# facebookresearch/PoseDiffusion

Measured on AMD Instinct MI355X. Metric: sequences/sec (20-frame, GGS on), higher is better.
Workload: dtype f32 (GGS, attention, LayerNorm, DDPM update, every accumulation); the encoder GEMMs multiply fp16 hi + lo operand pairs (22 bits, static power-of-two scales) with fp32 accumulation -- `exact_mode` is the same pipe with them on the exact-fp32 matrix instruction

## Files before the change

include/pd_engine.h:

```cpp
#ifndef PD_ENGINE_H
#define PD_ENGINE_H

#include <stdint.h>

#ifdef __cplusplus
extern "C" {
#endif

#define PD_OK 0
#define PD_ERR_INVALID_ARG (-1)
#define PD_ERR_UNSUPPORTED (-2)
#define PD_ERR_HIP (-3)
#define PD_ERR_STATE (-4)

#define PD_MAX_LAYERS 16
#define PD_POSE_DIM 9

typedef struct pd_engine pd_engine;

typedef struct pd_layer_weights {
    const float *norm1_w, *norm1_b;
    const float *in_proj_w, *in_proj_b;
    const float *out_proj_w, *out_proj_b;
    const float *norm2_w, *norm2_b;
    const float *linear1_w, *linear1_b;
    const float *linear2_w, *linear2_b;
} pd_layer_weights;

typedef struct pd_weights {
    int32_t d_model;
    int32_t nhead;
    int32_t dim_ff;
    int32_t num_layers;
    int32_t z_dim;
    int32_t n_harmonic;
    int32_t t_emb_dim;
    int32_t mlp_hidden;
    int32_t timesteps;
    int32_t reserved;
    const float *time_w0, *time_b0;
    const float *time_w2, *time_b2;
    const float *first_w, *first_b;
    pd_layer_weights layers[PD_MAX_LAYERS];
    const float *last0_w, *last0_b;
    const float *last_ln_w, *last_ln_b;
    const float *last3_w, *last3_b;
    const float *sqrt_recip_alphas_cumprod;
    const float *sqrt_recipm1_alphas_cumprod;
    const float *posterior_mean_coef1;
    const float *posterior_mean_coef2;
    const float *posterior_log_variance_clipped;
} pd_weights;

#define PD_WEIGHTS_PRED_X0 1
#define PD_WEIGHTS_POST_NORM 2
#define PD_WEIGHTS_NO_PIVOT 4
#define PD_WEIGHTS_GENERIC 8

typedef struct pd_ggs_cfg {
    float alpha;
    float learning_rate;
    int32_t iter_num;
    float sampson_max;
    int32_t min_matches;
    float momentum;
    int32_t wgs_per_seq;
    int32_t reserved;
} pd_ggs_cfg;
#define PD_GGS_CFG_FORCE_ONE_HOP 1
#define PD_GGS_CFG_NO_LDS_STAGING 2
#define PD_GGS_CFG_WAVES8 4
#define PD_GGS_CFG_LANE_ITEMS 8
#define PD_GGS_CFG_NO_LANE_ITEMS 16
#define PD_GGS_CFG_XCHG_SPREAD 32
#define PD_GGS_CFG_LONG_FRAMES 64


int pd_engine_create(const pd_weights *w, int max_B, int max_N, pd_engine **out);
void pd_engine_destroy(pd_engine *eng);
const char *pd_last_error(void);
const char *pd_version(void);


int pd_denoise_step(pd_engine *eng, const float *x, const float *z, int t, int B, int N,
                    float *eps_out, void *stream);

int pd_p_mean(pd_engine *eng, const float *x, const float *z, int t, int B, int N,
              float *mean_out, float *x0_out, void *stream);

int pd_p_finish(pd_engine *eng, const float *mean, const float *noise, int t, int B, int N,
                float *x_out, void *stream);


int pd_engine_set_q_tables(pd_engine *eng, const float *sqrt_alphas_cumprod, const float *sqrt_one_minus_alphas_cumprod);

int pd_denoise_step_t(pd_engine *eng, const float *x, const float *z, const int64_t *t_seq, int B, int N, float *out, void *stream);

int pd_p_losses(pd_engine *eng, const float *x_start, const float *z, const int64_t *t_seq, const float *noise, int B, int N,
                int loss_type, float *loss_out, float *x0_pred_out, float *xt_out, float *model_out, void *stream);

int pd_engine_set_frame_counts(pd_engine *eng, int B, const int32_t *n_frames, void *stream);


int pd_ggs_set_matches(pd_engine *eng, int seq, const double *kp1, const double *kp2,
                       const int64_t *i12, int64_t M, int n_frames, int height, int width);

#define PD_MATCH_HINT_ONE_ORDER (1 << 30)
typedef struct pd_match_hints {
    int32_t max_pairs;
    int32_t max_matches_per_pair;
} pd_match_hints;
int pd_ggs_set_matches_csr_async(pd_engine *eng, int seq_first, int n_seqs, const int64_t *seq_offsets, const double *kp1,
                                 const double *kp2, const int64_t *i12, int n_frames, int height, int width,
                                 const pd_match_hints *hints, void *stream);


int pd_ggs_guide(pd_engine *eng, float *model_mean, int B, int N, int t, const pd_ggs_cfg *cfg,
                 float *stats_out, void *stream);

int pd_ggs_stage_iters(const pd_ggs_cfg *cfg, int *iters_out5);

int pd_ggs_optimize(pd_engine *eng, float *model_mean, int B, int N, int update_R, int update_T,
                    int update_FL, const pd_ggs_cfg *cfg, float *stats_out, float *trace_out,
                    void *stream);

int pd_ggs_loss_grad(pd_engine *eng, const float *x, int B, int N, int update_R, int update_T,
                     int update_FL, const pd_ggs_cfg *cfg, float *loss_out, float *grad_out,
                     void *stream);


#define PD_OPT_DENOISER_SPLIT 2
#define PD_OPT_DENOISER_FUSED_ATTN 5
#define PD_OPT_DENOISER_LONG_ATTN 6
#define PD_OPT_GGS_MAX_FRAMES 7
#define PD_OPT_GGS_LONG_PAIR_ITEMS 8
int pd_engine_set_option(pd_engine *eng, int option, int value);
#define PD_OPT_WEIGHTS_NON_FINITE 4
int pd_engine_get_option(pd_engine *eng, int option, int *value_out);

int pd_sample(pd_engine *eng, const float *z, const float *noise, int B, int N, int cond_start_step,
              const pd_ggs_cfg *ggs, float *pose_out, float *process_out, float *stats_out,
              int use_graph, void *stream);

#define PD_PHASE_ALL 0
#define PD_PHASE_UNGUIDED 1
#define PD_PHASE_GUIDED 2
int pd_sample_phase(pd_engine *eng, const float *z, const float *noise, int B, int N, int cond_start_step,
                    const pd_ggs_cfg *ggs, int phase, float *pose_out, float *process_out, float *stats_out,
                    int use_graph, void *stream);

int pd_pose_to_camera(pd_engine *eng, const float *enc, int n_cameras, float *R_out, float *T_out,
                      float *focal_out, void *stream);
int pd_pose_to_camera_ex(pd_engine *eng, const float *enc, int n_cameras, float *R_out, float *T_out,
                         float *focal_out, float log_focal_length_bias, float min_focal_length, float max_focal_length,
                         void *stream);

int pd_camera_to_pose(const float *R, const float *T, const float *focal, int n, float log_focal_length_bias,
                      float min_focal_length, float max_focal_length, float *enc_out, void *stream);


int pd_time_embedding(const float *w0, const float *b0, const float *w2, const float *b2, const float *timesteps, int n,
                      float *out, void *stream);

int pd_pose_embedding(const float *x, long long rows, int dim, float *out, void *stream);


int pd_metrics_rel_pose_errors(const float *R_pred, const float *T_pred, const float *R_gt, const float *T_gt, int B, int N,
                               float *rel_r_deg, float *rel_t_deg, void *stream);

int pd_metrics_summary(const float *rel_r_deg, const float *rel_t_deg, int n, int max_threshold, float *out7, void *stream);

int pd_metrics_are(const float *R_a, const float *R_b, int n, float *err_deg, void *stream);

int pd_align_cameras(const float *R_src, const float *T_src, const float *R_tgt, const float *T_tgt, int n, int estimate_scale,
                     float eps, float *R_out, float *T_out, float *s_R_T_out, void *stream);


int pd_preprocess_image(const unsigned char *rgb_hwc, int height, int width, int image_size, float *out_chw, void *stream);


typedef struct pd_vit_layer_weights {
    const float *norm1_w, *norm1_b, *qkv_w, *qkv_b, *proj_w, *proj_b, *norm2_w, *norm2_b, *fc1_w, *fc1_b, *fc2_w, *fc2_b;
} pd_vit_layer_weights;
typedef struct pd_vit_weights {
    int32_t dim, depth, num_heads, mlp_hidden, patch_size, pos_grid, reserved0, reserved1;
    const float *patch_w, *patch_b, *cls_token, *pos_embed, *norm_w, *norm_b;
    pd_vit_layer_weights layers[16];
} pd_vit_weights;
typedef struct pd_vit pd_vit;
int pd_vit_create(const pd_vit_weights *w, pd_vit **out);
void pd_vit_destroy(pd_vit *v);
#define PD_VIT_OPT_EXACT_FP32 1
int pd_vit_set_option(pd_vit *v, int option, int value);

int pd_vit_forward_scale(pd_vit *v, const float *images, int n_img, int H, int W, double scale_factor, const float *pos_scaled,
                         float weight, int accumulate, float *z_out, void *stream);


int pd_ggs_launch_stamps(pd_engine *eng, long long *dst, int n, int *clock_khz_out, void *stream);

int pd_time_kernel(pd_engine *eng, int what, int B, int N, const pd_ggs_cfg *cfg, int reps,
                   float *ms_out, void *stream);

int pd_check_async_error(pd_engine *eng);

int pd_debug_ggs_prof(pd_engine *eng, int enable, long long *out6);
int pd_debug_ggs_plan(pd_engine *eng, int B, int N, const pd_ggs_cfg *cfg, int *out8);
int pd_debug_lane_tables(pd_engine *eng, int seq, int *out, int n_out);
int pd_debug_mfma_f16_subnormal(float *out4_host, void *stream);
int pd_debug_vit_tokens(pd_vit *v, float *dst, long long n_floats, void *stream);

#ifdef __cplusplus
}
#endif
#endif
```

posediffusion_amd/_lib.py:

```python
from __future__ import annotations

import ctypes as C
import os
import subprocess

_HERE = os.path.dirname(os.path.abspath(__file__))
LIB_PATH = os.environ.get("PD_ENGINE_LIB") or os.path.join(_HERE, "lib", "libpd_engine.so")
CSRC_DIR = os.path.join(_HERE, "csrc")
HEADER_PATH = os.path.normpath(os.path.join(_HERE, "..", "include", "pd_engine.h"))

PD_MAX_LAYERS = 16

c_float_p = C.POINTER(C.c_float)


class pd_layer_weights(C.Structure):
    _fields_ = [(n, C.c_void_p) for n in (
        "norm1_w", "norm1_b", "in_proj_w", "in_proj_b", "out_proj_w", "out_proj_b",
        "norm2_w", "norm2_b", "linear1_w", "linear1_b", "linear2_w", "linear2_b")]


class pd_weights(C.Structure):
    _fields_ = (
        [(n, C.c_int32) for n in ("d_model", "nhead", "dim_ff", "num_layers", "z_dim", "n_harmonic",
                                  "t_emb_dim", "mlp_hidden", "timesteps", "reserved")]
        + [(n, C.c_void_p) for n in ("time_w0", "time_b0", "time_w2", "time_b2", "first_w", "first_b")]
        + [("layers", pd_layer_weights * PD_MAX_LAYERS)]
        + [(n, C.c_void_p) for n in ("last0_w", "last0_b", "last_ln_w", "last_ln_b", "last3_w", "last3_b",
                                     "sqrt_recip_alphas_cumprod", "sqrt_recipm1_alphas_cumprod",
                                     "posterior_mean_coef1", "posterior_mean_coef2",
                                     "posterior_log_variance_clipped")]
    )


class pd_layer_grads(C.Structure):
    _fields_ = list(pd_layer_weights._fields_)


class pd_weight_grads(C.Structure):
    _fields_ = (
        [(n, C.c_void_p) for n in ("time_w0", "time_b0", "time_w2", "time_b2", "first_w", "first_b")]
        + [("layers", pd_layer_grads * PD_MAX_LAYERS)]
        + [(n, C.c_void_p) for n in ("last0_w", "last0_b", "last_ln_w", "last_ln_b", "last3_w", "last3_b")]
    )


class pd_vit_layer_weights(C.Structure):
    _fields_ = [(n, C.c_void_p) for n in ("norm1_w", "norm1_b", "qkv_w", "qkv_b", "proj_w", "proj_b", "norm2_w", "norm2_b",
                                          "fc1_w", "fc1_b", "fc2_w", "fc2_b")]


class pd_vit_weights(C.Structure):
    _fields_ = ([(n, C.c_int32) for n in ("dim", "depth", "num_heads", "mlp_hidden", "patch_size", "pos_grid", "reserved0", "reserved1")]
                + [(n, C.c_void_p) for n in ("patch_w", "patch_b", "cls_token", "pos_embed", "norm_w", "norm_b")]
                + [("layers", pd_vit_layer_weights * 16)])


class pd_vit_layer_grads(C.Structure):
    _fields_ = list(pd_vit_layer_weights._fields_)


class pd_vit_weight_grads(C.Structure):
    _fields_ = ([(n, C.c_void_p) for n in ("patch_w", "patch_b", "cls_token", "pos_embed", "norm_w", "norm_b")]
                + [("layers", pd_vit_layer_grads * 16)])


PD_VIT_TRAIN_MAX_TOKENS, PD_VIT_TRAIN_MAX_SCALES = 256, 8

PD_GGS_CFG_FORCE_ONE_HOP = 1
PD_GGS_CFG_NO_LDS_STAGING = 2
PD_GGS_CFG_WAVES8 = 4
PD_WEIGHTS_PRED_X0 = 1
PD_WEIGHTS_POST_NORM = 2
PD_WEIGHTS_NO_PIVOT = 4
PD_WEIGHTS_GENERIC = 8
PD_GGS_CFG_LANE_ITEMS = 8
PD_GGS_CFG_NO_LANE_ITEMS = 16
PD_GGS_CFG_XCHG_SPREAD = 32
PD_GGS_CFG_LONG_FRAMES = 64
PD_OPT_DENOISER_SPLIT = 2
PD_OPT_WEIGHTS_NON_FINITE = 4
PD_OPT_DENOISER_FUSED_ATTN = 5
PD_OPT_DENOISER_LONG_ATTN = 6
PD_OPT_GGS_MAX_FRAMES = 7
PD_OPT_GGS_LONG_PAIR_ITEMS = 8
PD_DROP_ATTN, PD_DROP_RESID1, PD_DROP_FF, PD_DROP_RESID2, PD_DROP_ALL = 1, 2, 4, 8, 15
PD_TR_OPT_MAX_FRAMES, PD_TR_OPT_LONG_ATTN = 1, 2
PD_MATCH_HINT_ONE_ORDER = 1 << 30


class pd_ggs_cfg(C.Structure):
    _fields_ = [("alpha", C.c_float), ("learning_rate", C.c_float), ("iter_num", C.c_int32),
                ("sampson_max", C.c_float), ("min_matches", C.c_int32), ("momentum", C.c_float),
                ("wgs_per_seq", C.c_int32), ("reserved", C.c_int32)]


class pd_match_hints(C.Structure):
    _fields_ = [("max_pairs", C.c_int32), ("max_matches_per_pair", C.c_int32)]


_vp, _i, _i64 = C.c_void_p, C.c_int, C.c_int64
SIGNATURES = {
    "pd_engine_create": (_i, [C.POINTER(pd_weights), _i, _i, C.POINTER(_vp)]),
    "pd_engine_destroy": (None, [_vp]),
    "pd_last_error": (C.c_char_p, []),
    "pd_version": (C.c_char_p, []),
    "pd_denoise_step": (_i, [_vp, _vp, _vp, _i, _i, _i, _vp, _vp]),
    "pd_engine_set_q_tables": (_i, [_vp, _vp, _vp]),
    "pd_engine_set_frame_counts": (_i, [_vp, _i, C.POINTER(C.c_int32), _vp]),
    "pd_denoise_step_t": (_i, [_vp, _vp, _vp, _vp, _i, _i, _vp, _vp]),
    "pd_p_losses": (_i, [_vp, _vp, _vp, _vp, _vp, _i, _i, _i, _vp, _vp, _vp, _vp, _vp]),
    "pd_camera_to_pose": (_i, [_vp, _vp, _vp, _i, C.c_float, C.c_float, C.c_float, _vp, _vp]),
    "pd_p_mean": (_i, [_vp, _vp, _vp, _i, _i, _i, _vp, _vp, _vp]),
    "pd_p_finish": (_i, [_vp, _vp, _vp, _i, _i, _i, _vp, _vp]),
    "pd_ggs_set_matches": (_i, [_vp, _i, _vp, _vp, _vp, _i64, _i, _i, _i]),
    "pd_ggs_set_matches_csr_async": (_i, [_vp, _i, _i, C.POINTER(_i64), _vp, _vp, _vp, _i, _i, _i, C.POINTER(pd_match_hints), _vp]),
    "pd_ggs_guide": (_i, [_vp, _vp, _i, _i, _i, C.POINTER(pd_ggs_cfg), _vp, _vp]),
    "pd_ggs_optimize": (_i, [_vp, _vp, _i, _i, _i, _i, _i, C.POINTER(pd_ggs_cfg), _vp, _vp, _vp]),
    "pd_ggs_loss_grad": (_i, [_vp, _vp, _i, _i, _i, _i, _i, C.POINTER(pd_ggs_cfg), _vp, _vp, _vp]),
    "pd_engine_set_option": (_i, [_vp, _i, _i]),
    "pd_engine_get_option": (_i, [_vp, _i, C.POINTER(_i)]),
    "pd_time_embedding": (_i, [_vp, _vp, _vp, _vp, _vp, _i, _vp, _vp]),
    "pd_pose_embedding": (_i, [_vp, C.c_longlong, _i, _vp, _vp]),
    "pd_metrics_rel_pose_errors": (_i, [_vp, _vp, _vp, _vp, _i, _i, _vp, _vp, _vp]),
    "pd_metrics_summary": (_i, [_vp, _vp, _i, _i, _vp, _vp]),
    "pd_metrics_are": (_i, [_vp, _vp, _i, _vp, _vp]),
    "pd_vit_create": (_i, [C.POINTER(pd_vit_weights), C.POINTER(_vp)]),
    "pd_vit_destroy": (None, [_vp]),
    "pd_vit_set_option": (_i, [_vp, _i, _i]),
    "pd_vit_forward_scale": (_i, [_vp, _vp, _i, _i, _i, C.c_double, _vp, C.c_float, _i, _vp, _vp]),
    "pd_preprocess_image": (_i, [_vp, _i, _i, _i, _vp, _vp]),
    "pd_align_cameras": (_i, [_vp, _vp, _vp, _vp, _i, _i, C.c_float, _vp, _vp, _vp, _vp]),
    "pd_sample": (_i, [_vp, _vp, _vp, _i, _i, _i, C.POINTER(pd_ggs_cfg), _vp, _vp, _vp, _i, _vp]),
    "pd_sample_phase": (_i, [_vp, _vp, _vp, _i, _i, _i, C.POINTER(pd_ggs_cfg), _i, _vp, _vp, _vp, _i, _vp]),
    "pd_pose_to_camera": (_i, [_vp, _vp, _i, _vp, _vp, _vp, _vp]),
    "pd_debug_lane_tables": (_i, [_vp, _i, C.POINTER(C.c_int), _i]),
    "pd_ggs_launch_stamps": (_i, [_vp, _vp, _i, C.POINTER(C.c_int), _vp]),
    "pd_ggs_stage_iters": (_i, [C.POINTER(pd_ggs_cfg), C.POINTER(C.c_int)]),
    "pd_pose_to_camera_ex": (_i, [_vp, _vp, _i, _vp, _vp, _vp, C.c_float, C.c_float, C.c_float, _vp]),
    "pd_time_kernel": (_i, [_vp, _i, _i, _i, C.POINTER(pd_ggs_cfg), _i, C.POINTER(C.c_float), _vp]),
    "pd_check_async_error": (_i, [_vp]),
    "pd_debug_ggs_prof": (_i, [_vp, _i, C.POINTER(C.c_longlong)]),
    "pd_debug_ggs_plan": (_i, [_vp, _i, _i, C.POINTER(pd_ggs_cfg), C.POINTER(C.c_int)]),
    "pd_debug_mfma_f16_subnormal": (_i, [C.POINTER(C.c_float), _vp]),
    "pd_debug_vit_tokens": (_i, [_vp, _vp, C.c_longlong, _vp]),
}
EXT_SIGNATURES = {
    "pd_ggs_set_matches_csr_async_nf": (_i, [_vp, _i, _i, C.POINTER(_i64), _vp, _vp, _vp, C.POINTER(_i), _i, _i, C.POINTER(pd_match_hints), _vp]),
}
TRAIN_SIGNATURES = {
    "pd_trainer_create": (_i, [C.POINTER(pd_weights), _vp, _vp, _i, _i, C.POINTER(_vp)]),
    "pd_trainer_destroy": (None, [_vp]),
    "pd_trainer_set_option": (_i, [_vp, _i, _i]),
    "pd_trainer_get_option": (_i, [_vp, _i, C.POINTER(_i)]),
    "pd_train_forward": (_i, [_vp, C.POINTER(pd_weights), _vp, _vp, _vp, _vp, _i, _i, _i, _vp, _vp, _vp, _vp, _vp]),
    "pd_train_forward_dropout": (_i, [_vp, C.POINTER(pd_weights), _vp, _vp, _vp, _vp, _i, _i, _i, C.c_float, C.c_uint, C.c_uint64, C.c_uint32,
                                      _vp, _vp, _vp, _vp, _vp]),
    "pd_train_backward": (_i, [_vp, C.POINTER(pd_weights), _vp, C.POINTER(pd_weight_grads), _vp, _vp]),
    "pd_train_debug_relu": (_i, [_vp, _i, _vp, C.c_longlong, _vp]),
    "pd_trainer_check_async": (_i, [_vp]),
}
VIT_TRAIN_SIGNATURES = {
    "pd_vit_trainer_create": (_i, [C.POINTER(pd_vit_weights), _i, _i, _i, C.POINTER(_vp)]),
    "pd_vit_trainer_destroy": (None, [_vp]),
    "pd_vit_train_forward": (_i, [_vp, C.POINTER(pd_vit_weights), _vp, _i, _i, _i, C.POINTER(C.c_double), _i, C.POINTER(_vp), _vp, _vp]),
    "pd_vit_train_backward": (_i, [_vp, C.POINTER(pd_vit_weights), _vp, C.POINTER(pd_vit_weight_grads), _vp]),
}

_lib = None


def build(verbose: bool = False) -> str:
    cmd = ["make", "-C", CSRC_DIR, "-j4"]
    res = subprocess.run(cmd, stdout=subprocess.PIPE, stderr=subprocess.STDOUT, text=True)
    if verbose or res.returncode != 0:
        print(res.stdout)
    if res.returncode != 0 or not os.path.isfile(LIB_PATH):
        raise RuntimeError("building libpd_engine.so failed:\n" + res.stdout[-4000:])
    return LIB_PATH


def load():
    global _lib
    if _lib is not None:
        return _lib
    if not os.path.isfile(LIB_PATH):
        raise RuntimeError(
            f"posediffusion_amd: HIP engine library not found at {LIB_PATH}. Build it with "
            "`python -c 'import __graft_entry__ as g; g.build()'` (or `make -C posediffusion_amd/csrc`). "
            "There is no CPU fallback.")
    import torch
    lib = C.CDLL(LIB_PATH, mode=C.RTLD_GLOBAL)
    for name, (res, args) in {**SIGNATURES, **EXT_SIGNATURES, **TRAIN_SIGNATURES, **VIT_TRAIN_SIGNATURES}.items():
        if os.environ.get("PD_ENGINE_LIB") and not hasattr(lib, name):
            continue
        fn = getattr(lib, name)
        fn.restype = res
        fn.argtypes = args
    _lib = lib
    return lib


def last_error() -> str:
    return (load().pd_last_error() or b"").decode("utf-8", "replace")


def check(rc: int, what: str = "pd_engine"):
    if rc != 0:
        raise RuntimeError(f"{what} failed (code {rc}): {last_error()}")
```

posediffusion_amd/csrc/pd_denoiser.hip:

```cpp
#include "pd_denoiser_dev.h"
#include "pd_gemm_stream.h"
#include "pd_gemm_split.h"
#include "pd_qkv_attn.h"
#include "pd_gemm_small.h"
#include "pd_attn.h"
#include "pd_attn_long.h"
#include "pd_denoiser_kernels.h"
#include "pd_denoiser_plan.h"

#include <algorithm>
#include <math.h>
#include <stdlib.h>
#include <string.h>

int pd_time_table(const pd_weights *w, float *table) {
    if (!w->time_w0 || !w->time_b0 || !w->time_w2 || !w->time_b2) {
        pd_set_error("pd_engine_create: a weight pointer is NULL");
        return PD_ERR_INVALID_ARG;
    }
    hipLaunchKernelGGL(pd_time_table_kernel, dim3(w->timesteps), dim3(128), 0, 0, w->time_w0, w->time_b0, w->time_w2, w->time_b2, table);
    PD_HIP_CHECK(hipGetLastError());
    return PD_OK;
}

// ... 128 lines not shown

bool pd_denoiser_has_streamed_path(const pd_engine *eng) { return eng->den && eng->den->hn; }
bool pd_denoiser_weights_non_finite(const pd_engine *eng) { return eng->den && eng->den->non_finite; }

int pd_denoiser_build_split(pd_engine *eng, int mode) {
    if (eng->gden) {
        pd_set_error("split-precision denoiser: this engine runs the shape-generic denoiser path (a non-default configuration or "
                     "PD_WEIGHTS_GENERIC), which has only the exact-fp32 kernels: PD_OPT_DENOISER_SPLIT stays 0");
        return PD_ERR_UNSUPPORTED;
    }
    PdDenoiserDev *d = eng->den;
    if (!d->hn) {
        pd_set_error("split-precision denoiser: the engine was created for fewer than %d token rows (max_B x max_N); the mode "
                     "applies to the streamed large-batch path only", PD_STREAM_MIN_ROWS);
        return PD_ERR_UNSUPPORTED;
    }
    const bool f16 = mode == 2;
    bool &ready = f16 ? d->split_h_ready : d->split_ready;
    if (ready) return PD_OK;
    PdPlaneExps e[PD_MAX_LAYERS] = {};
    for (int l = 0; f16 && l < d->num_layers; ++l) {
        PdLayerDev &L = d->layers[l];
        bool finite = true;
        PD_TRY(pd_plane_exponents(L.qkv_wf, L.qkv_b, L.out_wf, L.ff1_wf, L.ff1_b, L.ff2_wf, DM, DFF, &e[l], &finite));
        if (!finite) {
            d->non_finite = true;
            pd_set_error("denoiser: encoder layer %d holds non-finite weights or biases: no static operand bound exists, the fp16-plane "
                         "mode (PD_OPT_DENOISER_SPLIT = 2) is not available for these weights", l);
            return PD_ERR_INVALID_ARG;
        }
    }
    const int e_ln = 9;
    for (int l = 0; l < d->num_layers; ++l) {
        PdLayerDev &L = d->layers[l];
        PD_TRY(d->mem.planes(f16 ? &L.qkv_wh : &L.qkv_ws, L.qkv_wf, 3 * DM, DM, nullptr, f16, e[l].qkv));
        PD_TRY(d->mem.planes(f16 ? &L.out_wh : &L.out_ws, L.out_wf, DM, DM, nullptr, f16, e[l].out));
        PD_TRY(d->mem.planes(f16 ? &L.ff1_wh : &L.ff1_ws, L.ff1_wf, DFF, DM, nullptr, f16, e[l].ff1));
        PD_TRY(d->mem.planes(f16 ? &L.ff2_wh : &L.ff2_ws, L.ff2_wf, DM, DFF, nullptr, f16, e[l].ff2));
        if (!f16) continue;
        L.qkv_cs = ldexpf(1.0f, -(e_ln + e[l].qkv));
        L.out_cs = ldexpf(1.0f, -(e[l].ctx + e[l].out));
        L.ff1_cs = ldexpf(1.0f, -(e_ln + e[l].ff1));
        L.ff2_cs = ldexpf(1.0f, -(e[l].hid + e[l].ff2));
        L.ctx_scale = ldexpf(1.0f, e[l].ctx);
        L.ff_scale = ldexpf(1.0f, e[l].hid);
    }
    PD_HIP_CHECK(hipDeviceSynchronize());
    ready = true;
    return PD_OK;
}

void pd_denoiser_destroy(pd_engine *eng) {
    pd_denoiser_generic_destroy(eng);
    delete eng->den;
    eng->den = nullptr;
}

int pd_denoiser_prepare(pd_engine *eng, const float *z, int B, int N, hipStream_t s) {
    PdDenoiserDev *d = eng->den;
    if (eng->gden) d = nullptr;
    if (!z || B <= 0 || N <= 0 || B > eng->max_B || N > eng->max_N) {
        pd_set_error("denoiser: invalid arguments (B=%d N=%d; max_B=%d max_N=%d)", B, N, eng->max_B, eng->max_N);
        return PD_ERR_INVALID_ARG;
    }
    if (!d) return PD_OK;
    const int M = B * N;
    if (M >= PD_STREAM_MIN_ROWS && d->hn) pd_gemm_dma<0>(z, ZD, d->first_zf, ZD, d->first_b, d->zproj, M, DM, s);
    PD_HIP_CHECK(hipGetLastError());
    return PD_OK;
}

static void den_first_small(const pd_engine *eng, const PdDenoiserDev *d, GemmArgs &g, const float *x, const float *z, int t, int N, int MT, hipStream_t s) {
    g.bias = d->first_b; g.C = d->h; g.Nout = DM;
    g.x = x; g.z = z; g.temb = d->t_table + (size_t)t * 128; g.n_frames = N;
    launch_gemm<KFIRST_PAD, 2, 0>(g, d->first_wp, MT, eng->gemm_wide_min_tiles, s);
}
static void den_first_streamed(const PdDenoiserDev *d, const float *x, int t, int N, int M, hipStream_t s) {
    hipLaunchKernelGGL(pd_embed_rows_kernel, dim3((M + 3) / 4), dim3(256), 0, s, x, N, M, d->emb);
    pd_gemm_dma<4>(d->emb, KFIRST_D, d->first_df, KFIRST_D, d->ttab + (size_t)t * DM, d->h, M, DM, s, nullptr, d->zproj);
}

static void den_first_small_t(const pd_engine *eng, const PdDenoiserDev *d, GemmArgs &g, const float *x, const float *z, const int *t_row, int N, int MT,
                              hipStream_t s) {
    g.bias = d->first_b; g.C = d->h; g.Nout = DM;
    g.x = x; g.z = z; g.temb = d->t_table; g.t_row = t_row; g.n_frames = N;
    launch_gemm<KFIRST_PAD, 3, 0>(g, d->first_wp, MT, eng->gemm_wide_min_tiles, s);
}
static void den_first_streamed_t(const PdDenoiserDev *d, const float *x, const int *t_row, int N, int M, hipStream_t s) {
    hipLaunchKernelGGL(pd_embed_rows_kernel, dim3((M + 3) / 4), dim3(256), 0, s, x, N, M, d->emb);
    pd_den_first_gemm_t(d, t_row, M, s);
}

template <int SPLIT_OUT>
static void den_attn_long(const PdDenoiserDev *d, int B, int N, float out_scale, const int *nf, hipStream_t s) {
    static_assert(PD_MAX_DENOISER_FRAMES == PD_ATTN_LONG_TILE * PD_ATTN_LONG_MAX_TILES, "a lane holds one score per 64-key tile");
    hipLaunchKernelGGL(pd_attn_long_kernel<SPLIT_OUT>, dim3(B * NH, (N + PD_ATTN_LONG_ROWS - 1) / PD_ATTN_LONG_ROWS), dim3(256), pd_attn_long_lds(N, DH), s,
                       d->qkv, d->ctx, N, out_scale, nf);
}

static void den_layer_small(const pd_engine *eng, const PdDenoiserDev *d, const PdLayerDev &L, GemmArgs &g, bool long_attn, const int *nf, int B, int N, int MT,
                            hipStream_t s) {
    g.A = d->h; g.bias = L.qkv_b; g.C = d->qkv; g.Nout = 3 * DM;
    launch_gemm<DM, 1, 0>(g, L.qkv_wp, MT, eng->gemm_wide_min_tiles, s);
    if (long_attn) {
        den_attn_long<0>(d, B, N, 1.0f, nf, s);
    } else {
#ifdef PD_DEN_STAMPS
        hipLaunchKernelGGL(pd_attn_kernel<false>, dim3(B * NH, (N + 3) / 4), dim3(256), attn_lds(N), s, d->qkv, d->ctx, N, next_stamp_slot());
#else
        hipLaunchKernelGGL(pd_attn_kernel<false>, dim3(B * NH, (N + 3) / 4), dim3(256), attn_lds(N), s, d->qkv, d->ctx, N);
#endif
    }
    g.A = d->ctx; g.bias = L.out_b; g.C = d->h; g.Nout = DM;
    launch_gemm<DM, 0, 2>(g, L.out_wp, MT, eng->gemm_wide_min_tiles, s);
    g.A = d->h; g.bias = L.ff1_b; g.C = d->ff; g.Nout = DFF;
    launch_gemm<DM, 1, 1>(g, L.ff1_wp, MT, eng->gemm_wide_min_tiles, s);
    g.A = d->ff; g.bias = L.ff2_b; g.C = d->h; g.Nout = DM;
    launch_gemm<DFF, 0, 2>(g, L.ff2_wp, MT, eng->gemm_wide_min_tiles, s);
}
static void den_layer_streamed(const PdDenoiserDev *d, const PdLayerDev &L, bool long_attn, const int *nf, int B, int N, int M, hipStream_t s) {
    float2 *stats = (float2 *)d->hn;
    hipLaunchKernelGGL(pd_ln_stats_kernel<DM>, dim3((M + 3) / 4), dim3(256), 0, s, d->h, stats, M, 1e-5f);
    pd_gemm_dma<0, true>(d->h, DM, L.qkv_wf, DM, L.qkv_b, d->qkv, M, 3 * DM, s, stats);
    if (long_attn) den_attn_long<0>(d, B, N, 1.0f, nf, s);
    else hipLaunchKernelGGL(pd_attn_seq_kernel<0>, dim3(B * NH), dim3(256), attn_seq_lds(N), s, d->qkv, d->ctx, N, 1.0f);
    pd_gemm_dma<2>(d->ctx, DM, L.out_wf, DM, L.out_b, d->h, M, DM, s);
    hipLaunchKernelGGL(pd_ln_stats_kernel<DM>, dim3((M + 3) / 4), dim3(256), 0, s, d->h, stats, M, 1e-5f);
    pd_gemm_dma<1, true>(d->h, DM, L.ff1_wf, DM, L.ff1_b, d->ff, M, DFF, s, stats);
    pd_gemm_dma<2>(d->ff, DFF, L.ff2_wf, DFF, L.ff2_b, d->h, M, DM, s);
}
static void den_layer_bf16(const PdDenoiserDev *d, const PdLayerDev &L, bool long_attn, const int *nf, int B, int N, int M, hipStream_t s) {
    hipLaunchKernelGGL((pd_ln_rows_kernel<DM, 1>), dim3((M + 3) / 4), dim3(256), 0, s, d->h, d->hn, M, 1e-5f, 1.0f);
    pd_gemm_split<0, 1, 2>((const unsigned *)d->hn, DM, L.qkv_ws, DM, L.qkv_b, d->qkv, M, 3 * DM, s);
    if (long_attn) den_attn_long<1>(d, B, N, 1.0f, nf, s);
    else hipLaunchKernelGGL(pd_attn_seq_kernel<1>, dim3(B * NH), dim3(256), attn_seq_lds(N), s, d->qkv, d->ctx, N, 1.0f);
    pd_gemm_split<2, 1, 1>((const unsigned *)d->ctx, DM, L.out_ws, DM, L.out_b, d->h, M, DM, s);
    hipLaunchKernelGGL((pd_ln_rows_kernel<DM, 1>), dim3((M + 3) / 4), dim3(256), 0, s, d->h, d->hn, M, 1e-5f, 1.0f);
    pd_gemm_split<4, 1, 2>((const unsigned *)d->hn, DM, L.ff1_ws, DM, L.ff1_b, d->ff, M, DFF, s);
    pd_gemm_split<2, 1, 1>((const unsigned *)d->ff, DFF, L.ff2_ws, DFF, L.ff2_b, d->h, M, DM, s);
}
template <int EPI>
static void den_gemm_f16(int rt, const float *A, int K, const unsigned *W, const float *bias, float *C, int M, int Nout, hipStream_t s, float c_scale,
                         float out_scale = 1.0f) {
    const unsigned *Aw = (const unsigned *)A;
    if constexpr (PD_STRIP_RT1 != 0 && (EPI == 2 || (EPI == 4 && PD_STRIP_RT1 == 2)))
        if (rt == 1) return pd_gemm_strip<EPI, 1, true, 1, PD_STRIP_K64>(Aw, K, W, K, bias, C, M, Nout, s, c_scale, out_scale);
    if constexpr (EPI != 0)
        if (rt == 3) return pd_gemm_strip<EPI, 3, true, 1, PD_STRIP_K64>(Aw, K, W, K, bias, C, M, Nout, s, c_scale, out_scale);
    if (rt == 2) return pd_gemm_strip<EPI, 2, true, 1, PD_STRIP_K64>(Aw, K, W, K, bias, C, M, Nout, s, c_scale, out_scale);
    pd_gemm_split<EPI, 1, EPI == 2 ? 1 : 2, true>(Aw, K, W, K, bias, C, M, Nout, s, c_scale, out_scale);
}
static void den_layer_f16(const PdDenoiserDev *d, const PdLayerDev &L, const PdDenStepPlan &p, const int *nf, int B, int N, hipStream_t s) {
    const int M = p.M;
    hipLaunchKernelGGL((pd_ln_rows_kernel<DM, 2>), dim3((M + 3) / 4), dim3(256), 0, s, d->h, d->hn, M, 1e-5f, 512.0f);
    if (p.fused_attn) {
        pd_qkv_attn((const unsigned *)d->hn, L.qkv_wh, L.qkv_b, (unsigned *)d->ctx, B, N, L.qkv_cs, L.ctx_scale, s);
    } else {
        den_gemm_f16<0>(p.strip & 1 ? 2 : 0, d->hn, DM, L.qkv_wh, L.qkv_b, d->qkv, M, 3 * DM, s, L.qkv_cs);
        if (p.long_attn) den_attn_long<2>(d, B, N, L.ctx_scale, nf, s);
        else if (p.attn_mma) hipLaunchKernelGGL(pd_attn_mma_kernel<2>, dim3(B * NH), dim3(256), attn_mma_lds(N), s, d->qkv, d->ctx, N, L.ctx_scale);
        else hipLaunchKernelGGL(pd_attn_seq_kernel<2>, dim3(B * NH), dim3(256), attn_seq_lds(N), s, d->qkv, d->ctx, N, L.ctx_scale);
    }
    den_gemm_f16<2>(p.strip & 2 ? p.rt_res : 0, d->ctx, DM, L.out_wh, L.out_b, d->h, M, DM, s, L.out_cs);
    hipLaunchKernelGGL((pd_ln_rows_kernel<DM, 2>), dim3((M + 3) / 4), dim3(256), 0, s, d->h, d->hn, M, 1e-5f, 512.0f);
    den_gemm_f16<4>(p.strip & 4 ? p.rt_ff1 : 0, d->hn, DM, L.ff1_wh, L.ff1_b, d->ff, M, DFF, s, L.ff1_cs, L.ff_scale);
    den_gemm_f16<2>(p.strip & 8 ? p.rt_res : 0, d->ff, DFF, L.ff2_wh, L.ff2_b, d->h, M, DM, s, L.ff2_cs);
}
static void den_tail(const pd_engine *eng, const PdDenoiserDev *d, const float *x, int t, int M, float *eps_out, float *mean_out, float *x0_out,
                     const float *noise, float *x_next_out, bool stamped, const int *nf, int N, hipStream_t s) {
    HeadArgs ha;
    memset(&ha, 0, sizeof(ha));
    ha.hid = d->hid; ha.lnw = d->last_ln_w; ha.lnb = d->last_ln_b;
    ha.w3 = d->last3_w; ha.b3 = d->last3_b; ha.x = x; ha.noise = noise;
    ha.eps_out = eps_out; ha.mean_out = mean_out; ha.x0_out = x0_out; ha.xnext_out = x_next_out;
    ha.c_recip = eng->c_recip[t]; ha.c_recipm1 = eng->c_recipm1[t]; ha.coef1 = eng->coef1[t]; ha.coef2 = eng->coef2[t];
    ha.sigma = expf(0.5f * eng->logvar[t]);
    ha.M = M;
    ha.pred_x0 = eng->pred_x0;
    ha.nf = nf; ha.n_frames = N;
#ifdef PD_DEN_STAMPS
    ha.stamps = stamped ? next_stamp_slot() : nullptr;
#endif
    hipLaunchKernelGGL(pd_tail_kernel, dim3((M + 3) / 4), dim3(256), 0, s, ha);
}

static void den_tail_t(const pd_engine *eng, const PdDenoiserDev *d, const float *x, int M, const PdTSeq &ts, float *eps_out, float *x0_out, hipStream_t s) {
    HeadArgsT a;
    memset(&a, 0, sizeof(a));
    a.h.hid = d->hid; a.h.lnw = d->last_ln_w; a.h.lnb = d->last_ln_b;
    a.h.w3 = d->last3_w; a.h.b3 = d->last3_b; a.h.x = x;
    a.h.eps_out = eps_out; a.h.x0_out = x0_out;
    a.h.M = M;
    a.h.pred_x0 = eng->pred_x0;
    a.t_row = ts.t_row; a.c_recip = eng->d_c_recip; a.c_recipm1 = eng->d_c_recipm1;
    a.target = ts.target; a.loss_out = ts.loss_out; a.loss_type = ts.loss_type;
    hipLaunchKernelGGL(pd_tail_t_kernel, dim3((M + 3) / 4), dim3(256), 0, s, a);
}

int pd_denoiser_t_rows(pd_engine *eng, const int64_t *t_seq, int B, int N, hipStream_t s) {
    const int M = B * N;
    hipLaunchKernelGGL(pd_t_rows_kernel, dim3((M + 255) / 256), dim3(256), 0, s, t_seq, M, N, eng->timesteps, eng->d_t_row, eng->d_err);
    PD_HIP_CHECK(hipGetLastError());
    return PD_OK;
}
int pd_denoiser_q_sample(pd_engine *eng, const float *x_start, const float *noise, const int64_t *t_seq, int B, int N, float *xt, hipStream_t s) {
    const int M = B * N;
    hipLaunchKernelGGL(pd_q_sample_kernel, dim3((M * 9 + 255) / 256), dim3(256), 0, s, x_start, noise, t_seq, eng->d_q_a, eng->d_q_b, M, N, eng->timesteps,
                       xt, eng->d_t_row, eng->d_err);
    PD_HIP_CHECK(hipGetLastError());
    return PD_OK;
}

int pd_denoiser_launch(pd_engine *eng, const float *x, const float *z, int t, int B, int N, float *eps_out,
                       float *mean_out, float *x0_out, const float *noise, float *x_next_out, hipStream_t s, bool z_prepared, const PdTSeq *ts) {
    if (eng->gden) return pd_denoiser_generic_launch(eng, x, z, t, B, N, eps_out, mean_out, x0_out, noise, x_next_out, s, ts);
    PdDenoiserDev *d = eng->den;
    if (!x || !z || B <= 0 || N <= 0 || B > eng->max_B || N > eng->max_N || N > PD_MAX_DENOISER_FRAMES || t < 0 || t >= d->timesteps) {
        pd_set_error("denoiser: invalid arguments (B=%d N=%d t=%d; max_B=%d max_N=%d, N <= %d, 0 <= t < %d)", B, N, t,
                     eng->max_B, eng->max_N, PD_MAX_DENOISER_FRAMES, d->timesteps);
        return PD_ERR_INVALID_ARG;
    }
    const int *nf = nullptr;
    if (!ts) PD_TRY(pd_frame_counts(eng, B, N, "denoiser", &nf));
    if (!z_prepared) {
        int rc = pd_denoiser_prepare(eng, z, B, N, s);
        if (rc) return rc;
    }
    static const int knob_strip = pd_dev_knob("PD_DEN_STRIP", 15), knob_attn_mma = pd_dev_knob("PD_DEN_ATTN_MMA", 1);
    const PdDenStepPlan p = pd_den_step_plan(B, N, eng->den_split, eng->den_fused_attn, eng->num_cus, d->hn != nullptr, d->split_ready,
                                             d->split_h_ready, knob_strip, knob_attn_mma, eng->den_long_attn, nf != nullptr);
    const bool small = p.path == PD_DEN_SMALL;
    const int M = p.M;
    GemmArgs g;
    memset(&g, 0, sizeof(g));
    g.M = M;
    if (small && ts) den_first_small_t(eng, d, g, x, z, ts->t_row, N, p.MT, s);
    else if (small) den_first_small(eng, d, g, x, z, t, N, p.MT, s);
    else if (ts) den_first_streamed_t(d, x, ts->t_row, N, M, s);
    else den_first_streamed(d, x, t, N, M, s);
    for (int l = 0; l < d->num_layers; ++l) {
        const PdLayerDev &L = d->layers[l];
        switch (p.path) {
        case PD_DEN_SMALL: den_layer_small(eng, d, L, g, p.long_attn, nf, B, N, p.MT, s); break;
        case PD_DEN_STREAMED: den_layer_streamed(d, L, p.long_attn, nf, B, N, M, s); break;
        case PD_DEN_BF16_PLANES: den_layer_bf16(d, L, p.long_attn, nf, B, N, M, s); break;
        case PD_DEN_F16_PLANES: den_layer_f16(d, L, p, nf, B, N, s); break;
        }
    }
    if (small) {
        g.A = d->h; g.bias = d->last0_b; g.C = d->hid; g.Nout = HID;
        launch_gemm<DM, 0, 0>(g, d->last0_wp, p.MT, eng->gemm_wide_min_tiles, s);
    } else {
        pd_gemm_dma<0>(d->h, DM, d->last0_wf, DM, d->last0_b, d->hid, M, HID, s);
    }
    if (ts) den_tail_t(eng, d, x, M, *ts, eps_out, x0_out, s);
    else den_tail(eng, d, x, t, M, eps_out, mean_out, x0_out, noise, x_next_out, small, nf, N, s);
    PD_HIP_CHECK(hipGetLastError());
    return PD_OK;
}


extern "C" int pd_time_embedding(const float *w0, const float *b0, const float *w2, const float *b2, const float *timesteps, int n,
                                 float *out, void *stream) {
    if (n == 0) return PD_OK;
    if (!w0 || !b0 || !w2 || !b2 || !timesteps || !out || n < 0) {
        pd_set_error("pd_time_embedding: invalid arguments (n=%d)", n);
        return PD_ERR_INVALID_ARG;
    }
    hipLaunchKernelGGL(pd_time_embed_kernel, dim3(n), dim3(128), 0, (hipStream_t)stream, timesteps, w0, b0, w2, b2, out);
    PD_HIP_CHECK(hipGetLastError());
    return PD_OK;
}
extern "C" int pd_pose_embedding(const float *x, long long rows, int dim, float *out, void *stream) {
    if (rows == 0 && dim >= 1) return PD_OK;
    if (!x || !out || rows < 0 || dim < 1 || dim > 4096) {
        pd_set_error("pd_pose_embedding: invalid arguments (rows=%lld dim=%d)", rows, dim);
        return PD_ERR_INVALID_ARG;
    }
    const long long total = rows * 21 * dim;
    const int blocks = (int)((total + 255) / 256 < 65536 ? (total + 255) / 256 : 65536);
    hipLaunchKernelGGL(pd_harmonic_rows_kernel, dim3(blocks), dim3(256), 0, (hipStream_t)stream, x, rows, dim, out);
    PD_HIP_CHECK(hipGetLastError());
    return PD_OK;
}

static int mfma_f16_subnormal(bool shape16, const char *who, float *out4_host, void *stream) {
    if (!out4_host) return PD_ERR_INVALID_ARG;
    float *d = nullptr;
    PD_HIP_CHECK(hipMalloc((void **)&d, 8 * sizeof(float)));
    hipStream_t s = (hipStream_t)stream;
    if (shape16) hipLaunchKernelGGL(pd_mfma16_f16_subnormal_kernel, dim3(1), dim3(64), 0, s, d);
    else hipLaunchKernelGGL(pd_mfma_f16_subnormal_kernel, dim3(1), dim3(64), 0, s, d);
    float h[8];
    hipError_t e = hipMemcpyAsync(h, d, sizeof(h), hipMemcpyDeviceToHost, s);
    if (e == hipSuccess) e = hipStreamSynchronize(s);
    (void)hipFree(d);
    if (e != hipSuccess) {
        pd_set_error("%s: %s", who, hipGetErrorString(e));
        return PD_ERR_HIP;
    }
    for (int i = 0; i < 4; ++i) out4_host[i] = h[i];
    if (h[4] == 0.0f) out4_host[0] = -1.0f;
    return PD_OK;
}
extern "C" int pd_debug_mfma_f16_subnormal(float *out4_host, void *stream) {
    return mfma_f16_subnormal(out4_host && out4_host[0] == 32.0f, "pd_debug_mfma_f16_subnormal", out4_host, stream);
}
```

posediffusion_amd/csrc/pd_denoiser_plan.h:

```cpp
#pragma once
#include "pd_qkv_attn.h"

#ifndef PD_STRIP_RT3
#define PD_STRIP_RT3 1
#endif
#ifndef PD_STRIP_RT1
#define PD_STRIP_RT1 0
#endif
#ifndef PD_STRIP_RT3_FF1
#define PD_STRIP_RT3_FF1 0
#endif
#ifndef PD_STRIP_K64
#define PD_STRIP_K64 true
#endif

enum PdDenPath {
    PD_DEN_SMALL,
    PD_DEN_STREAMED,
    PD_DEN_BF16_PLANES,
    PD_DEN_F16_PLANES
};

struct PdDenStepPlan {
    PdDenPath path;
    int M, MT;
    bool long_attn;
    bool fused_attn;
    bool attn_mma;
    int rt_res, rt_ff1;
    int strip;
};

static inline PdDenStepPlan pd_den_step_plan(int B, int N, int split, int fused_attn, int num_cus, bool has_streamed, bool split_ready,
                                             bool split_h_ready, int knob_strip, int knob_attn_mma, int long_attn = 0, bool ragged = false) {
    PdDenStepPlan p = {};
    p.M = B * N;
    p.MT = (p.M + 31) / 32;
    p.long_attn = N > 64 || long_attn != 0 || ragged;
    if (p.M < PD_STREAM_MIN_ROWS || !has_streamed) p.path = PD_DEN_SMALL;
    else if (split == 2 && split_h_ready) p.path = PD_DEN_F16_PLANES;
    else if (split == 1 && split_ready) p.path = PD_DEN_BF16_PLANES;
    else p.path = PD_DEN_STREAMED;
    if (p.path != PD_DEN_F16_PLANES) return p;
    const int cus = num_cus > 0 ? num_cus : 256;
    const int qa_wgs = pd_qkv_attn_wgs(B, N);
    const bool qa_fills = 4 * qa_wgs >= 3 * ((qa_wgs + cus - 1) / cus) * cus;
    p.fused_attn = qa_wgs > 0 && !p.long_attn && (fused_attn == 1 ? qa_fills : fused_attn == 2);
    p.attn_mma = N <= 32 && knob_attn_mma && !p.long_attn;
    const bool rt3 = PD_STRIP_RT3 && (((p.M + 63) / 64) * (DM / 128)) > cus && (((p.M + 95) / 96) * (DM / 128)) <= cus;
    p.rt_res = !rt3 ? 2 : PD_STRIP_RT1 ? 1 : 3;
    p.rt_ff1 = !rt3 ? 2 : PD_STRIP_RT1 == 2 ? 1 : PD_STRIP_RT3_FF1 ? 3 : 2;
    p.strip = knob_strip;
    return p;
}
```

posediffusion_amd/csrc/pd_engine.hip:

```cpp
#include "pd_internal.h"

#include <algorithm>

#include <math.h>
#include <stdarg.h>
#include <string.h>

static thread_local char g_err[1024] = "";

void pd_set_error(const char *fmt, ...) {
    va_list ap;
    va_start(ap, fmt);
    vsnprintf(g_err, sizeof(g_err), fmt, ap);
    va_end(ap);
}

extern "C" const char *pd_last_error(void) { return g_err; }
extern "C" const char *pd_version(void) { return "pd_engine 0.1 gfx950"; }

__global__ void pd_finish_kernel(const float *__restrict__ mean, const float *__restrict__ noise, float sigma, int n,
                                 float *__restrict__ out, const int *__restrict__ nf, int n_frames) {
    const int i = blockIdx.x * blockDim.x + threadIdx.x;
    if (i >= n) return;
    if (nf) {
// ... 436 lines not shown
    return pd_pose_to_camera_ex(eng, enc, n_cameras, R_out, T_out, focal_out, 1.8f, 0.1f, 20.0f, stream);
}

int pd_ggs_frames_unsupported(const pd_engine *eng, int N, const char *who) {
    if (!eng || N <= eng->ggs_max_frames || N > eng->max_N) return PD_OK;
    pd_set_error("%s: geometry-guided sampling (GGS) is limited to %d frames (N=%d); the denoiser and unguided sampling take up to %d "
                 "frames: sample without GGS", who, eng->ggs_max_frames, N, PD_MAX_DENOISER_FRAMES);
    return PD_ERR_UNSUPPORTED;
}
static void guide_stages(const pd_ggs_cfg *cfg, PdGgsStage *st) {
    const int it = cfg->iter_num;
    st[0] = {1, 1, 1, 2 * it};
    st[1] = {0, 0, 1, it};
    st[2] = {1, 0, 0, it};
    st[3] = {0, 1, 0, it};
    st[4] = {1, 1, 1, 2 * it};
}

extern "C" int pd_ggs_stage_iters(const pd_ggs_cfg *cfg, int *iters_out5) {
    if (!cfg || !iters_out5 || cfg->iter_num < 0) {
        pd_set_error("pd_ggs_stage_iters: invalid arguments");
        return PD_ERR_INVALID_ARG;
    }
    PdGgsStage st[PD_GGS_MAX_STAGES];
    guide_stages(cfg, st);
    for (int i = 0; i < 5; ++i) iters_out5[i] = st[i].iters;
    return PD_OK;
}

static int check_cfg(const pd_ggs_cfg *cfg, const char *who) {
    if (!cfg || cfg->iter_num < 0 || !(cfg->learning_rate > 0.0f)) {
        pd_set_error("%s: invalid pd_ggs_cfg", who);
        return PD_ERR_INVALID_ARG;
    }
    return PD_OK;
}

extern "C" int pd_ggs_guide(pd_engine *eng, float *model_mean, int B, int N, int t, const pd_ggs_cfg *cfg,
                            float *stats_out, void *stream) {
    (void)t;
    int rc = check_cfg(cfg, "pd_ggs_guide");
    if (rc) return rc;
    PdGgsStage st[5];
    guide_stages(cfg, st);
    return pd_ggs_launch(eng, model_mean, B, N, st, 5, cfg, 0, stats_out, nullptr, 0, nullptr, nullptr, (hipStream_t)stream);
}

extern "C" int pd_ggs_optimize(pd_engine *eng, float *model_mean, int B, int N, int update_R, int update_T, int update_FL,
                               const pd_ggs_cfg *cfg, float *stats_out, float *trace_out, void *stream) {
    int rc = check_cfg(cfg, "pd_ggs_optimize");
    if (rc) return rc;
    PdGgsStage st = {update_R ? 1 : 0, update_T ? 1 : 0, update_FL ? 1 : 0, cfg->iter_num};
    if (update_R && update_T && update_FL) st.iters *= 2;
    return pd_ggs_launch(eng, model_mean, B, N, &st, 1, cfg, 0, stats_out, trace_out, st.iters, nullptr, nullptr,
                         (hipStream_t)stream);
}

extern "C" int pd_ggs_loss_grad(pd_engine *eng, const float *x, int B, int N, int update_R, int update_T, int update_FL,
                                const pd_ggs_cfg *cfg, float *loss_out, float *grad_out, void *stream) {
    int rc = check_cfg(cfg, "pd_ggs_loss_grad");
    if (rc) return rc;
    if (!loss_out || !grad_out) {
        pd_set_error("pd_ggs_loss_grad: NULL output");
        return PD_ERR_INVALID_ARG;
    }
    PdGgsStage st = {update_R ? 1 : 0, update_T ? 1 : 0, update_FL ? 1 : 0, 1};
    return pd_ggs_launch(eng, const_cast<float *>(x), B, N, &st, 1, cfg, 1, nullptr, nullptr, 0, loss_out, grad_out,
                         (hipStream_t)stream);
}

static int issue_loop(pd_engine *eng, int B, int N, int cond_start, const pd_ggs_cfg *ggs, bool want_stats, int step_begin,
                      int step_end, hipStream_t s) {
    const int T = eng->timesteps;
    const size_t bn9 = (size_t)B * N * 9;
    float *proc = eng->d_process;
    int rc0 = pd_denoiser_prepare(eng, eng->d_z, B, N, s);
    if (rc0) return rc0;
    for (int step = step_begin; step < step_end; ++step) {
        const int t = T - 1 - step;
        const float *x = proc + (size_t)step * bn9;
        float *xn = proc + (size_t)(step + 1) * bn9;
        const bool guided = ggs && t < cond_start;
        int rc;
        if (guided) {
            rc = pd_denoiser_launch(eng, x, eng->d_z, t, B, N, nullptr, nullptr, nullptr, nullptr, xn, s, true);
            if (rc) return rc;
            float *st = want_stats ? eng->d_stats + (size_t)(cond_start - 1 - t) * B * 5 * 4 : nullptr;
            eng->stamp_slot = (cond_start - 1 - t) % PD_STAMP_SLOTS;
            rc = pd_ggs_guide(eng, xn, B, N, t, ggs, st, s);
            eng->stamp_slot = 0;
        } else {
            const float *nz = (t > 0) ? eng->d_noise + (size_t)(step + 1) * bn9 : nullptr;
            rc = pd_denoiser_launch(eng, x, eng->d_z, t, B, N, nullptr, nullptr, nullptr, nz, xn, s, true);
        }
        if (rc) return rc;
    }
    return PD_OK;
}

static bool same_cfg(const pd_ggs_cfg &a, const pd_ggs_cfg &b) { return memcmp(&a, &b, sizeof(a)) == 0; }

extern "C" int pd_sample_phase(pd_engine *eng, const float *z, const float *noise, int B, int N, int cond_start_step,
                               const pd_ggs_cfg *ggs, int phase, float *pose_out, float *process_out, float *stats_out,
                               int use_graph, void *stream) {
    if (!eng || !z || !noise || !pose_out || B <= 0 || B > eng->max_B || N <= 0 || N > eng->max_N ||
        cond_start_step < 0 || cond_start_step > eng->timesteps || phase < PD_PHASE_ALL || phase > PD_PHASE_GUIDED) {
        pd_set_error("pd_sample: invalid arguments (B=%d N=%d cond_start_step=%d phase=%d)", B, N, cond_start_step, phase);
        return PD_ERR_INVALID_ARG;
    }
    if (ggs) {
        int rc = check_cfg(ggs, "pd_sample");
        if (rc) return rc;
        if (cond_start_step > 0) {
            PD_TRY(pd_ggs_frames_unsupported(eng, N, "pd_sample"));
            for (int b = 0; b < B; ++b)
                if (!eng->seqs[b].blob) {
                    pd_set_error("pd_sample: GGS requested but sequence slot %d has no matches", b);
                    return PD_ERR_STATE;
                }
        }
    }
    const int *nf = nullptr;
    PD_TRY(pd_frame_counts(eng, B, N, "pd_sample", &nf));
    hipStream_t s = (hipStream_t)stream;
    const int T = eng->timesteps;
    const size_t bn9 = (size_t)B * N * 9;
    const bool has_ggs = ggs && cond_start_step > 0;
    const bool want_stats = has_ggs && stats_out;
    const int split = has_ggs ? T - cond_start_step : T;
    const int step_begin = phase == PD_PHASE_GUIDED ? split : 0;
    const int step_end = phase == PD_PHASE_UNGUIDED ? split : T;
    if (phase != PD_PHASE_GUIDED) {
        PD_HIP_CHECK(hipMemcpyAsync(eng->d_z, z, sizeof(float) * B * N * eng->z_dim, hipMemcpyDeviceToDevice, s));
        PD_HIP_CHECK(hipMemcpyAsync(eng->d_noise, noise, sizeof(float) * (T + 1) * bn9, hipMemcpyDeviceToDevice, s));
        PD_HIP_CHECK(hipMemcpyAsync(eng->d_process, noise, sizeof(float) * bn9, hipMemcpyDeviceToDevice, s));
        if (nf) hipLaunchKernelGGL(pd_zero_padding_kernel, dim3(((int)bn9 + 255) / 256), dim3(256), 0, s, eng->d_process, (int)bn9, nf, N);
    }
    if (has_ggs && phase != PD_PHASE_UNGUIDED) {
        int rc = pd_wait_uploads(eng, s);
        if (rc) return rc;
    }
    if (step_begin == step_end) {
    } else if (!use_graph) {
        int rc = issue_loop(eng, B, N, cond_start_step, has_ggs ? ggs : nullptr, true, step_begin, step_end, s);
        if (rc) return rc;
    } else {
        pd_engine::GraphKey key;
        memset(&key, 0, sizeof(key));
        key.B = B;
        key.N = N;
        key.cond_start = has_ggs ? cond_start_step : 0;
        key.has_ggs = has_ggs;
        key.phase = phase;
        key.den_split = eng->den_split | (eng->den_fused_attn << 8) | (eng->den_long_attn << 16) | ((nf ? 1 : 0) << 24);
        if (has_ggs) {
            key.cfg = *ggs;
            if (phase != PD_PHASE_UNGUIDED) {
                int rc = pd_ggs_plan(eng, B, N, ggs, &key.plan);
                if (rc) return rc;
            }
        }
        hipGraphExec_t exec = nullptr;
        for (size_t gi = 0; gi < eng->graphs.size(); ++gi) {
            auto &g = eng->graphs[gi];
            if (g.first.B == B && g.first.N == N && g.first.cond_start == key.cond_start && g.first.has_ggs == key.has_ggs &&
                g.first.phase == phase && g.first.den_split == key.den_split && same_cfg(g.first.cfg, key.cfg) &&
                memcmp(&g.first.plan, &key.plan, sizeof(PdGgsPlan)) == 0) {
                exec = g.second;
                std::rotate(eng->graphs.begin() + gi, eng->graphs.begin() + gi + 1, eng->graphs.end());
                break;
            }
        }
        if (!exec) {
            if (!eng->own_stream) PD_HIP_CHECK(hipStreamCreateWithFlags(&eng->own_stream, hipStreamNonBlocking));
            hipGraph_t graph = nullptr;
            PD_HIP_CHECK(hipStreamBeginCapture(eng->own_stream, hipStreamCaptureModeThreadLocal));
            int rc = issue_loop(eng, B, N, cond_start_step, has_ggs ? ggs : nullptr, true, step_begin, step_end, eng->own_stream);
            hipError_t ce = hipStreamEndCapture(eng->own_stream, &graph);
            if (rc) {
                if (graph) (void)hipGraphDestroy(graph);
                return rc;
            }
            PD_HIP_CHECK(ce);
            PD_HIP_CHECK(hipGraphInstantiate(&exec, graph, nullptr, nullptr, 0));
            PD_HIP_CHECK(hipGraphDestroy(graph));
            if (eng->graphs.size() >= PD_GRAPH_CACHE_MAX) {
                PD_HIP_CHECK(hipDeviceSynchronize());
                (void)hipGraphExecDestroy(eng->graphs.front().second);
                eng->graphs.erase(eng->graphs.begin());
            }
            eng->graphs.push_back({key, exec});
        }
        PD_HIP_CHECK(hipGraphLaunch(exec, s));
        if (has_ggs) {
            int rc = pd_mark_use(eng, s);
            if (rc) return rc;
        }
    }
    if (phase == PD_PHASE_UNGUIDED) return PD_OK;
    PD_HIP_CHECK(hipMemcpyAsync(pose_out, eng->d_process + (size_t)T * bn9, sizeof(float) * bn9, hipMemcpyDeviceToDevice, s));
    if (process_out)
        PD_HIP_CHECK(hipMemcpyAsync(process_out, eng->d_process, sizeof(float) * (T + 1) * bn9, hipMemcpyDeviceToDevice, s));
    if (want_stats)
        PD_HIP_CHECK(hipMemcpyAsync(stats_out, eng->d_stats, sizeof(float) * (size_t)cond_start_step * B * 5 * 4,
                                    hipMemcpyDeviceToDevice, s));
    return PD_OK;
}

extern "C" int pd_sample(pd_engine *eng, const float *z, const float *noise, int B, int N, int cond_start_step,
                         const pd_ggs_cfg *ggs, float *pose_out, float *process_out, float *stats_out, int use_graph,
                         void *stream) {
    return pd_sample_phase(eng, z, noise, B, N, cond_start_step, ggs, PD_PHASE_ALL, pose_out, process_out, stats_out, use_graph,
                           stream);
}

extern "C" int pd_engine_set_option(pd_engine *eng, int option, int value) {
    if (!eng) {
        pd_set_error("pd_engine_set_option: NULL engine");
        return PD_ERR_INVALID_ARG;
    }
    switch (option) {
    case PD_OPT_DENOISER_SPLIT:
        if (value < 0 || value > 2) {
            pd_set_error("pd_engine_set_option: PD_OPT_DENOISER_SPLIT takes 0, 1 or 2 (got %d)", value);
            return PD_ERR_INVALID_ARG;
        }
        if (value) {
            PD_HIP_CHECK(hipSetDevice(eng->device));
            int rc = pd_denoiser_build_split(eng, value);
            if (rc) return rc;
        }
        eng->den_split = value;
        break;
    case PD_OPT_DENOISER_FUSED_ATTN:
        if (value < 0 || value > 2) {
            pd_set_error("pd_engine_set_option: PD_OPT_DENOISER_FUSED_ATTN takes 0, 1 or 2 (got %d)", value);
            return PD_ERR_INVALID_ARG;
        }
        eng->den_fused_attn = value;
        break;
    case PD_OPT_DENOISER_LONG_ATTN:
        if (value < 0 || value > 1) {
            pd_set_error("pd_engine_set_option: PD_OPT_DENOISER_LONG_ATTN takes 0 or 1 (got %d)", value);
            return PD_ERR_INVALID_ARG;
        }
        eng->den_long_attn = value;
        break;
    case PD_OPT_GGS_MAX_FRAMES: {
        if (value != PD_MAX_FRAMES && !(value > PD_MAX_FRAMES && value <= eng->max_N && value <= PD_GGS_LONG_MAX_FRAMES)) {
            pd_set_error("pd_engine_set_option: PD_OPT_GGS_MAX_FRAMES takes %d (the default) or a value in (%d, max_N=%d] with max_N <= %d (got %d)",
                         PD_MAX_FRAMES, PD_MAX_FRAMES, eng->max_N, PD_GGS_LONG_MAX_FRAMES, value);
            return PD_ERR_INVALID_ARG;
        }
        PD_HIP_CHECK(hipSetDevice(eng->device));
        PD_HIP_CHECK(hipDeviceSynchronize());
        const size_t granules = xchg_granules_for(std::min(value, eng->max_N));
        if (granules != eng->xchg_granules) {
            unsigned long long *fresh = nullptr;
            if (hipMalloc((void **)&fresh, sizeof(unsigned long long) * 2 * granules * eng->max_B) != hipSuccess) {
                (void)hipGetLastError();
                pd_set_error("pd_engine_set_option: PD_OPT_GGS_MAX_FRAMES = %d: hipMalloc of %zu B for the exchange region failed; the limit stays %d",
                             value, sizeof(unsigned long long) * 2 * granules * eng->max_B, eng->ggs_max_frames);
                return PD_ERR_HIP;
            }
            (void)hipFree(eng->d_xchg);
            eng->d_xchg = fresh;
            eng->xchg_granules = granules;
        }
        for (auto &g : eng->graphs) (void)hipGraphExecDestroy(g.second);
        eng->graphs.clear();
        eng->ggs_max_frames = value;
        break;
    }
    case PD_OPT_GGS_LONG_PAIR_ITEMS:
        if (value < 0 || value > 1) {
            pd_set_error("pd_engine_set_option: PD_OPT_GGS_LONG_PAIR_ITEMS takes 0 or 1 (got %d)", value);
            return PD_ERR_INVALID_ARG;
        }
        eng->ggs_long_pair_items = value;
        break;
    case 3:
        if (value == 0) break;
        pd_set_error("pd_engine_set_option: option 3 (the persistent small-batch denoiser launch of round 3) is no longer built: it measured "
                     "2.4 x slower than the multi-launch path (profiles/round3_small_persistent.txt; source parked under tools/parked/)");
        return PD_ERR_UNSUPPORTED;
    default:
        pd_set_error("pd_engine_set_option: unknown option %d", option);
        return PD_ERR_INVALID_ARG;
    }
    return PD_OK;
}

extern "C" int pd_engine_get_option(pd_engine *eng, int option, int *value_out) {
    if (!eng || !value_out) {
        pd_set_error("pd_engine_get_option: NULL argument");
        return PD_ERR_INVALID_ARG;
    }
    switch (option) {
    case PD_OPT_DENOISER_SPLIT: *value_out = eng->den_split; break;
    case PD_OPT_DENOISER_FUSED_ATTN: *value_out = eng->den_fused_attn; break;
    case PD_OPT_DENOISER_LONG_ATTN: *value_out = eng->den_long_attn; break;
    case PD_OPT_GGS_MAX_FRAMES: *value_out = eng->ggs_max_frames; break;
    case PD_OPT_GGS_LONG_PAIR_ITEMS: *value_out = eng->ggs_long_pair_items; break;
    case PD_OPT_WEIGHTS_NON_FINITE: *value_out = pd_denoiser_weights_non_finite(eng) ? 1 : 0; break;
    default:
        pd_set_error("pd_engine_get_option: unknown option %d", option);
        return PD_ERR_INVALID_ARG;
    }
    return PD_OK;
}

extern "C" int pd_time_kernel(pd_engine *eng, int what, int B, int N, const pd_ggs_cfg *cfg, int reps, float *ms_out,
                              void *stream) {
    if (!eng || !ms_out || reps <= 0 || B <= 0 || B > eng->max_B || N <= 0 || N > eng->max_N) {
        pd_set_error("pd_time_kernel: invalid arguments");
        return PD_ERR_INVALID_ARG;
    }
    if (what != 0) {
        PD_TRY(check_cfg(cfg, "pd_time_kernel"));
        PD_TRY(pd_ggs_frames_unsupported(eng, N, "pd_time_kernel"));
    }
    hipStream_t s = (hipStream_t)stream;
    struct CountsOff {
        pd_engine *e;
        int B;
        explicit CountsOff(pd_engine *e_) : e(e_), B(e_->nf_B) { e->nf_B = 0; }
        ~CountsOff() { e->nf_B = B; }
    } counts_off(eng);
    hipEvent_t e0, e1;
    PD_HIP_CHECK(hipEventCreate(&e0));
    PD_HIP_CHECK(hipEventCreate(&e1));
    const size_t bn9 = (size_t)B * N * 9;
    int rc = PD_OK;
    if (what == 0) {
        rc = pd_denoiser_launch(eng, eng->d_process, eng->d_z, 50, B, N, nullptr, eng->d_mean, nullptr, nullptr, nullptr, s, false);
        PD_HIP_CHECK(hipEventRecord(e0, s));
        for (int i = 0; i < reps && !rc; ++i)
            rc = pd_denoiser_launch(eng, eng->d_process, eng->d_z, 50, B, N, nullptr, eng->d_mean, nullptr, nullptr, nullptr, s, true);
        PD_HIP_CHECK(hipEventRecord(e1, s));
    } else {
        PD_HIP_CHECK(hipEventRecord(e0, s));
        for (int i = 0; i < reps && !rc; ++i) {
            PD_HIP_CHECK(hipMemcpyAsync(eng->d_mean, eng->d_process + (size_t)eng->timesteps * bn9, sizeof(float) * bn9,
                                        hipMemcpyDeviceToDevice, s));
            rc = pd_ggs_guide(eng, eng->d_mean, B, N, 0, cfg, nullptr, s);
        }
        PD_HIP_CHECK(hipEventRecord(e1, s));
    }
    if (rc) return rc;
    PD_HIP_CHECK(hipEventSynchronize(e1));
    float ms = 0.0f;
    PD_HIP_CHECK(hipEventElapsedTime(&ms, e0, e1));
    *ms_out = ms / (float)reps;
    (void)hipEventDestroy(e0);
    (void)hipEventDestroy(e1);
    return PD_OK;
}

extern "C" int pd_check_async_error(pd_engine *eng) {
    if (!eng) return PD_ERR_INVALID_ARG;
    unsigned int v = 0;
    PD_HIP_CHECK(hipDeviceSynchronize());
    PD_HIP_CHECK(hipMemcpy(&v, eng->d_err, sizeof(v), hipMemcpyDeviceToHost));
    if (v) {
        pd_set_error("asynchronous error (flag=%u):%s%s%s%s", v,
                     (v & 1u) ? " a cross-workgroup exchange spin timed out (co-resident workgroups lost?);" : "",
                     (v & 2u) ? " pd_ggs_set_matches_csr_async met a frame index outside [0, n_frames);" : "",
                     (v & 4u) ? " pd_ggs_set_matches_csr_async: pd_match_hints violated (more pairs / matches per pair than declared): the slot was emptied;" : "",
                     (v & 8u) ? " pd_denoise_step_t / pd_p_losses met a timestep outside [0, timesteps): it was clamped;" : "");
        (void)hipMemset(eng->d_err, 0, sizeof(v));
        return PD_ERR_STATE;
    }
    return PD_OK;
}

extern "C" int pd_debug_ggs_prof(pd_engine *eng, int enable, long long *out6) {
    if (!eng) return PD_ERR_INVALID_ARG;
    eng->ggs_prof_on = enable;
    if (out6) {
        PD_HIP_CHECK(hipDeviceSynchronize());
        PD_HIP_CHECK(hipMemcpy(out6, eng->d_err + 2, sizeof(long long) * 16, hipMemcpyDeviceToHost));
    }
    return PD_OK;
}

__global__ void pd_copy_stamps_kernel(const unsigned long long *__restrict__ src, long long *__restrict__ dst, int n2) {
    const int i = threadIdx.x;
    if (i < n2) dst[i] = (long long)src[i];
}
extern "C" int pd_ggs_launch_stamps(pd_engine *eng, long long *dst, int n, int *clock_khz_out, void *stream) {
    if (!eng || !dst || n <= 0 || n > PD_STAMP_SLOTS) {
        pd_set_error("pd_ggs_launch_stamps: invalid arguments (n=%d, at most %d slots)", n, PD_STAMP_SLOTS);
        return PD_ERR_INVALID_ARG;
    }
    if (clock_khz_out) {
        static int khz = 0;
        if (khz == 0) PD_HIP_CHECK(hipDeviceGetAttribute(&khz, hipDeviceAttributeWallClockRate, eng->device));
        *clock_khz_out = khz;
    }
    hipLaunchKernelGGL(pd_copy_stamps_kernel, dim3(1), dim3(2 * PD_STAMP_SLOTS), 0, (hipStream_t)stream, eng->d_stamps, dst, 2 * n);
    PD_HIP_CHECK(hipGetLastError());
    return PD_OK;
}

extern "C" int pd_debug_lane_tables(pd_engine *eng, int seq, int *out, int n_out) {
    if (!eng || !out || seq < 0 || seq >= eng->max_B || n_out < 4) {
        pd_set_error("pd_debug_lane_tables: invalid arguments (seq=%d n_out=%d)", seq, n_out);
        return PD_ERR_INVALID_ARG;
    }
    PD_HIP_CHECK(hipDeviceSynchronize());
    PdSeqDesc D;
    PD_HIP_CHECK(hipMemcpy(&D, eng->d_seqs + seq, sizeof(D), hipMemcpyDeviceToHost));
    for (int i = 0; i < n_out; ++i) out[i] = 0;
    out[0] = D.n_litems;
    out[1] = D.n_lwaves;
    out[2] = D.l_item_len;
    out[3] = D.l_max_steps;
    if (D.n_lwaves > 0 && D.lwave) {
        int2 lw[PD_LANE_WAVES];
        const int nw = D.n_lwaves < PD_LANE_WAVES ? D.n_lwaves : PD_LANE_WAVES;
        PD_HIP_CHECK(hipMemcpy(lw, D.lwave, sizeof(int2) * nw, hipMemcpyDeviceToHost));
        for (int w = 0; w < nw && 4 + w < n_out; ++w) out[4 + w] = lw[w].y;
    }
    return PD_OK;
}

extern "C" int pd_debug_ggs_plan(pd_engine *eng, int B, int N, const pd_ggs_cfg *cfg, int *out8) {
    if (!eng || !cfg || !out8) return PD_ERR_INVALID_ARG;
    PD_TRY(pd_ggs_frames_unsupported(eng, N, "pd_debug_ggs_plan"));
    PdGgsPlan plan;
    int rc = pd_ggs_plan(eng, B, N, cfg, &plan);
    if (rc) return rc;
    const int v[8] = {plan.k, plan.n_slots, plan.lds, plan.long_frames ? 1 + plan.long_frames : plan.two_hop, plan.waves, plan.stage_p, plan.lane, plan.lane_rl};
    for (int i = 0; i < 8; ++i) out8[i] = v[i];
    return PD_OK;
}
```

posediffusion_amd/csrc/pd_gemm_split.h:

```cpp
#pragma once
#include "pd_gemm_stream.h"

__device__ __forceinline__ float vit_gelu_fast(float v) {
    const float x = fabsf(v) * 0.70710678118654752f;
    const float t = __builtin_amdgcn_rcpf(fmaf(0.3275911f, x, 1.0f));
    float p = fmaf(1.061405429f, t, -1.453152027f);
    p = fmaf(p, t, 1.421413741f);
    p = fmaf(p, t, -0.284496736f);
    p = fmaf(p, t, 0.254829592f);
    const float q = 0.5f * p * t * __expf(-x * x);
    return v * (v >= 0.0f ? 1.0f - q : q);
}

struct VitSplitArgs {
    const unsigned *A, *W;
    const float *bias;
    void *C;
    int M, Nout, K, lda;
    float c_scale, out_scale;
#ifdef PD_STRIP_LEGS
    long long *legs;
#endif
};
#ifndef PD_STRIP_PIPE
// ... 31 lines not shown
            mtile = grp * GROUP + r % GROUP;
        } else {
            const int r = b - full, rest = MT % GROUP;
            ntile = r / rest;
            mtile = (MT / GROUP) * GROUP + r % rest;
        }
    }
    const int m0 = mtile * TM, n0 = ntile * TN;
    const int sr = tid >> 2, sg = tid & 3, st = sr * LR + 8 * sg;
    const int KS = g.K / 16;
#define VP_EACH(X) X(0) X(1)
#define VP_DECL(j)                                                                                                            \
    const uint4 *ap##j = (const uint4 *)(g.A + (size_t)min(m0 + sr + 64 * (j < WM ? j : 0), g.M - 1) * g.lda) + 2 * sg;        \
    const uint4 *wq##j = (const uint4 *)g.W + (size_t)(n0 / 32 + wn * WN + (j < WN ? j : 0)) * KS * 128 + lane;                 \
    uint4 ra##j##a, ra##j##b, cw##j##0h, cw##j##0l, cw##j##1h, cw##j##1l, nw##j##0h, nw##j##0l, nw##j##1h, nw##j##1l;
#define VP_LOAD(j)                                  \
    if constexpr (j < WM) {                         \
        ra##j##a = ap##j[nx];                       \
        ra##j##b = ap##j[nx + 1];                   \
    }                                               \
    if constexpr (j < WN) {                         \
        nw##j##0h = wq##j[(size_t)(nc * 4 + 0) * 64]; \
        nw##j##0l = wq##j[(size_t)(nc * 4 + 1) * 64]; \
        nw##j##1h = wq##j[(size_t)(nc * 4 + 2) * 64]; \
        nw##j##1l = wq##j[(size_t)(nc * 4 + 3) * 64]; \
    }
#define VP_LOAD_A(j)                                \
    if constexpr (j < WM) {                         \
        ra##j##a = ap##j[nx];                       \
        ra##j##b = ap##j[nx + 1];                   \
    }
#define VP_LOAD_W(j)                                \
    if constexpr (j < WN) {                         \
        nw##j##0h = wq##j[(size_t)(nc * 4 + 0) * 64]; \
        nw##j##0l = wq##j[(size_t)(nc * 4 + 1) * 64]; \
        nw##j##1h = wq##j[(size_t)(nc * 4 + 2) * 64]; \
        nw##j##1l = wq##j[(size_t)(nc * 4 + 3) * 64]; \
    }
#define VP_ROLL(j)             \
    if constexpr (j < WN) {    \
        cw##j##0h = nw##j##0h; \
        cw##j##0l = nw##j##0l; \
        cw##j##1h = nw##j##1h; \
        cw##j##1l = nw##j##1l; \
    }
#define VP_STORE(j)                                                                                       \
    if constexpr (j < WM) {                                                                               \
        uint4 h, l;                                                                                       \
        h.x = __builtin_amdgcn_perm(ra##j##a.y, ra##j##a.x, 0x05040100u);                                 \
        l.x = __builtin_amdgcn_perm(ra##j##a.y, ra##j##a.x, 0x07060302u);                                 \
        h.y = __builtin_amdgcn_perm(ra##j##a.w, ra##j##a.z, 0x05040100u);                                 \
        l.y = __builtin_amdgcn_perm(ra##j##a.w, ra##j##a.z, 0x07060302u);                                 \
        h.z = __builtin_amdgcn_perm(ra##j##b.y, ra##j##b.x, 0x05040100u);                                 \
        l.z = __builtin_amdgcn_perm(ra##j##b.y, ra##j##b.x, 0x07060302u);                                 \
        h.w = __builtin_amdgcn_perm(ra##j##b.w, ra##j##b.z, 0x05040100u);                                 \
        l.w = __builtin_amdgcn_perm(ra##j##b.w, ra##j##b.z, 0x07060302u);                                 \
        *(uint4 *)(da + st + j * 64 * LR) = h;                                                            \
        *(uint4 *)(da + st + j * 64 * LR + 4) = l;                                                        \
    }
#define VP_MMA(j, s)                                                                                                         \
    if constexpr (j < WN) {                                                                                                  \
        _Pragma("unroll") for (int mi = 0; mi < WM; ++mi) {                                                                  \
            acc[mi][j < WN ? j : 0] = mma(al##s[mi], cw##j##s##h, acc[mi][j < WN ? j : 0]);                                    \
            acc[mi][j < WN ? j : 0] = mma(ah##s[mi], cw##j##s##l, acc[mi][j < WN ? j : 0]);                                    \
            acc[mi][j < WN ? j : 0] = mma(ah##s[mi], cw##j##s##h, acc[mi][j < WN ? j : 0]);                                    \
        }                                                                                                                    \
    }
    auto mma = [](const uint4 &a, const uint4 &b, const f32x16 &c) {
        if constexpr (F16) return __builtin_amdgcn_mfma_f32_32x32x16_f16(__builtin_bit_cast(f16x8, a), __builtin_bit_cast(f16x8, b), c, 0, 0, 0);
        else return __builtin_amdgcn_mfma_f32_32x32x16_bf16(__builtin_bit_cast(bf16x8, a), __builtin_bit_cast(bf16x8, b), c, 0, 0, 0);
    };
    VP_EACH(VP_DECL)
    {
        const int nx = 0, nc = 0;
        unsigned *da = As;
        VP_EACH(VP_LOAD)
        VP_EACH(VP_STORE)
        VP_EACH(VP_ROLL)
    }
    __syncthreads();
    f32x16 acc[WM][WN];
#pragma unroll
    for (int mi = 0; mi < WM; ++mi)
#pragma unroll
        for (int ni = 0; ni < WN; ++ni)
#pragma unroll
            for (int i = 0; i < 16; ++i) acc[mi][ni][i] = 0.0f;
    const int nk = g.K / KC;
    const int aoff = (wm * 32 * WM + l31) * LR + 8 * hi;
    for (int kc = 0; kc < nk; ++kc) {
        const int nc = min(kc + 1, nk - 1), nx = nc * (KC / 4);
        if constexpr (BARE == 0 || BARE == 5) { VP_EACH(VP_LOAD) }
        else if constexpr (BARE == 1) { VP_EACH(VP_LOAD_A) }
        else if constexpr (BARE == 2) { VP_EACH(VP_LOAD_W) }
        __builtin_amdgcn_sched_barrier(0);
        const unsigned *a = As + (kc & 1) * TM * LR + aoff;
        uint4 ah0[WM], al0[WM], ah1[WM], al1[WM];
#pragma unroll
        for (int mi = 0; mi < WM; ++mi) {
            ah0[mi] = *(const uint4 *)(a + mi * 32 * LR);
            al0[mi] = *(const uint4 *)(a + mi * 32 * LR + 4);
            ah1[mi] = *(const uint4 *)(a + mi * 32 * LR + 16);
            al1[mi] = *(const uint4 *)(a + mi * 32 * LR + 20);
        }
        if constexpr (BARE != 5) {
            VP_MMA(0, 0)
            VP_MMA(1, 0)
            VP_MMA(0, 1)
            VP_MMA(1, 1)
        }
        __builtin_amdgcn_sched_barrier(0);
        unsigned *da = As + ((kc + 1) & 1) * TM * LR;
        if constexpr (BARE == 0 || BARE == 1 || BARE == 5) { VP_EACH(VP_STORE) }
        if constexpr (BARE == 0 || BARE == 2 || BARE == 5) { VP_EACH(VP_ROLL) }
        if constexpr (BARE != 4) __syncthreads();
    }
#undef VP_DECL
#undef VP_LOAD
#undef VP_LOAD_A
#undef VP_LOAD_W
#undef VP_ROLL
#undef VP_STORE
#undef VP_MMA
#pragma unroll
    for (int mi = 0; mi < WM; ++mi)
#pragma unroll
        for (int ni = 0; ni < WN; ++ni) {
            const int col = n0 + (wn * WN + ni) * 32 + l31, r0 = m0 + (wm * WM + mi) * 32 + 4 * hi;
            const float bias = g.bias[col];
            float res[16];
            if constexpr (EPI == 2) {
#pragma unroll
                for (int i = 0; i < 16; ++i) res[i] = ((const float *)g.C)[(size_t)min(r0 + (i & 3) + 8 * (i >> 2), g.M - 1) * g.Nout + col];
            }
#pragma unroll
            for (int i = 0; i < 16; ++i) {
                const int row = r0 + (i & 3) + 8 * (i >> 2);
                float v = F16 ? fmaf(acc[mi][ni][i], g.c_scale, bias) : acc[mi][ni][i] + bias;
                if constexpr (EPI == 3) v = vit_gelu_fast(v);
                if constexpr (EPI == 4) v = pd_relu(v);
                if constexpr (EPI == 2) v += res[i];
                if (row < g.M) {
                    if constexpr (EPI == 3 || EPI == 4)
                        ((unsigned *)g.C)[(size_t)row * g.Nout + col] = pd_split_word_as<F16 ? 2 : 1>(v, g.out_scale);
                    else
                        ((float *)g.C)[(size_t)row * g.Nout + col] = v;
                }
            }
        }
}

template <bool M16>
__device__ __forceinline__ int pd_strip_swz(int r) { return M16 ? ((r >> 1) & 1) | ((r >> 1) & 4) : (r >> 1) & 7; }
static constexpr size_t PD_STRIP_PATCH_BYTES = (size_t)4 * 32 * 36 * sizeof(float);
template <int RT, bool K64>
static constexpr size_t pd_gemm_strip_lds() {
    const size_t stage = (size_t)(K64 ? 4 : 2) * 32 * RT * 32 * sizeof(unsigned);
    return K64 && PD_STRIP_WIDE_EPI && stage < PD_STRIP_PATCH_BYTES ? PD_STRIP_PATCH_BYTES : stage;
}
template <int EPI, int RT, bool F16, int CT = 1, int BARE = 0, bool K64 = false>
__global__ __launch_bounds__(256) __attribute__((amdgpu_waves_per_eu((K64 && PD_STRIP_MFMA16 && RT >= 2) ? (RT == 3 ? 3 : 4) - (EPI == 2 ? 1 : 0) : 1)))
void pd_gemm_strip_kernel(VitSplitArgs g) {
    constexpr bool M16 = K64 && PD_STRIP_MFMA16 != 0;
    static_assert(!M16 || PD_STRIP_WIDE_EPI, "the 16x16 accumulator layout is written out by the wide epilogue only");
    constexpr int KC = 32, TM = 32 * RT, TN = 128 * CT, GROUP = RT == 3 ? 24 : (RT == 1 ? 32 : 2048 / TM), CHA = TM * KC;
    static_assert(RT >= 1 && RT <= 4 && (CT == 1 || CT == 2), "pieces of 8 rows, RT per wave and chunk");
    extern __shared__ __attribute__((aligned(1024))) unsigned strip_lds[];
    PD_LEG(0, wall_clock64());
    PD_LEG(2, __builtin_amdgcn_s_memtime());
    const int tid = threadIdx.x, lane = tid & 63, l31 = lane & 31, hi = lane >> 5, l15 = lane & 15, kg = lane >> 4;
    const int wave = __builtin_amdgcn_readfirstlane(tid >> 6);
    const int MT = (g.M + TM - 1) / TM, NT = g.Nout / TN;
    int mtile, ntile;
    {
        const int b = blockIdx.x, full = (MT / GROUP) * GROUP * NT;
        if (b < full) {
            const int grp = b / (NT * GROUP), r = b - grp * (NT * GROUP);
            ntile = r / GROUP;
            mtile = grp * GROUP + r % GROUP;
        } else {
            const int r = b - full, rest = MT % GROUP;
            ntile = r / rest;
            mtile = (MT / GROUP) * GROUP + r % rest;
        }
    }
    const int m0 = mtile * TM, n0 = ntile * TN;
    const int prow = lane >> 3, pslot = lane & 7;
    unsigned oa[RT];
#pragma unroll
    for (int j = 0; j < RT; ++j) {
        const int r = 8 * (RT * wave + j) + prow;
        oa[j] = (unsigned)(((size_t)min(m0 + r, g.M - 1) * g.lda + 4 * (pslot ^ pd_strip_swz<M16>(r))) * sizeof(unsigned));
    }
    const unsigned lds_a = (unsigned)(size_t)(strip_lds + RT * wave * 256);
    auto stage = [&](int kc, int buf) {
        const float *ab = (const float *)(g.A + kc * KC);
        const unsigned da = __builtin_amdgcn_readfirstlane(lds_a + buf * CHA * 4);
#pragma unroll
        for (int j = 0; j < RT; ++j) pd_dma_piece(ab, oa[j], da + j * 1024);
    };
    const int KS = g.K / 16;
    const uint4 *wq = (const uint4 *)g.W + (size_t)(n0 / 32 + CT * wave) * KS * 128 + (M16 ? (kg >> 1) * 128 + (kg & 1) * 32 + l15 : lane);
    uint4 cw[CT][2][2], nw[CT][2][2];
    auto mma = [](const uint4 &a, const uint4 &b, const f32x16 &c) {
        if constexpr (F16) return __builtin_amdgcn_mfma_f32_32x32x16_f16(__builtin_bit_cast(f16x8, a), __builtin_bit_cast(f16x8, b), c, 0, 0, 0);
        else return __builtin_amdgcn_mfma_f32_32x32x16_bf16(__builtin_bit_cast(bf16x8, a), __builtin_bit_cast(bf16x8, b), c, 0, 0, 0);
    };
    f32x16 acc[RT][CT];
    typedef float acc_v4 __attribute__((ext_vector_type(4)));
    acc_v4 acc4[M16 ? 2 * RT : 1][2];
    typedef unsigned res_v4 __attribute__((ext_vector_type(4)));
    res_v4 resid[(EPI == 2 && K64) ? RT : 1][4];
    if constexpr (K64) {
        static_assert(CT == 1 && BARE == 0, "the 64-k form exists for one column tile per wave");
        typedef unsigned wv4 __attribute__((ext_vector_type(4)));
#pragma unroll
        for (int mi = 0; mi < RT; ++mi)
#pragma unroll
            for (int i = 0; i < 16; ++i) acc[mi][0][i] = 0.0f;
#pragma unroll
        for (int t = 0; t < (M16 ? 2 * RT : 1); ++t) acc4[t][0] = acc4[t][1] = acc_v4{0.0f, 0.0f, 0.0f, 0.0f};
        auto mmaw = [](const uint4 &a, const wv4 &b, const f32x16 &c) {
            if constexpr (F16) return __builtin_amdgcn_mfma_f32_32x32x16_f16(__builtin_bit_cast(f16x8, a), __builtin_bit_cast(f16x8, b), c, 0, 0, 0);
            else return __builtin_amdgcn_mfma_f32_32x32x16_bf16(__builtin_bit_cast(bf16x8, a), __builtin_bit_cast(bf16x8, b), c, 0, 0, 0);
        };
        auto mma16 = [](const uint4 &a, const wv4 &b, const acc_v4 &c) {
            if constexpr (F16) return __builtin_amdgcn_mfma_f32_16x16x32_f16(__builtin_bit_cast(f16x8, a), __builtin_bit_cast(f16x8, b), c, 0, 0, 0);
            else return __builtin_amdgcn_mfma_f32_16x16x32_bf16(__builtin_bit_cast(bf16x8, a), __builtin_bit_cast(bf16x8, b), c, 0, 0, 0);
        };
#define PD_STRIP_WLOAD(w0, w1, w2, w3, b)                                                                                            \
    do {                                                                                                                             \
        const uint4 *wp_ = wq + (size_t)(b) * 256;                                                                                   \
        if constexpr (M16)                                                                                                           \
            asm volatile("global_load_dwordx4 %0, %4, off\n\tglobal_load_dwordx4 %1, %4, off offset:1024\n\t"                       \
                         "global_load_dwordx4 %2, %4, off offset:256\n\tglobal_load_dwordx4 %3, %4, off offset:1280"                 \
                         : "=&v"(w0), "=&v"(w1), "=&v"(w2), "=&v"(w3) : "v"(wp_) : "memory");                                        \
        else                                                                                                                         \
            asm volatile("global_load_dwordx4 %0, %4, off\n\tglobal_load_dwordx4 %1, %4, off offset:1024\n\t"                       \
                         "global_load_dwordx4 %2, %4, off offset:2048\n\tglobal_load_dwordx4 %3, %4, off offset:3072"                \
                         : "=&v"(w0), "=&v"(w1), "=&v"(w2), "=&v"(w3) : "v"(wp_) : "memory");                                        \
    } while (0)
#define PD_STRIP_WAIT(n, w0, w1, w2, w3) asm volatile("s_waitcnt vmcnt(" #n ")" : "+v"(w0), "+v"(w1), "+v"(w2), "+v"(w3) : : "memory")
#define PD_STRIP_WAITN(n, w0, w1, w2, w3) asm volatile("s_waitcnt vmcnt(%4)" : "+v"(w0), "+v"(w1), "+v"(w2), "+v"(w3) : "n"(n) : "memory")
        auto stage64 = [&](int c, int buf) {
            const unsigned da = __builtin_amdgcn_readfirstlane(lds_a + buf * 2 * CHA * 4);
#pragma unroll
            for (int h = 0; h < 2; ++h) {
                const float *ab = (const float *)(g.A + (2 * c + h) * KC);
#pragma unroll
                for (int j = 0; j < RT; ++j) pd_dma_piece(ab, oa[j], da + h * CHA * 4 + j * 1024);
            }
        };
        auto block = [&](const unsigned *a, const wv4 &w0, const wv4 &w1, const wv4 &w2, const wv4 &w3) {
            uint4 ah[RT], al[RT];
            if constexpr (M16) {
                const int sz = pd_strip_swz<true>(l15);
#pragma unroll
                for (int st = 0; st < 2; ++st)
#pragma unroll
                    for (int mi = 0; mi < RT; ++mi) {
                        const uint4 p = *(const uint4 *)(a + (mi * 32 + st * 16) * KC + 4 * ((2 * kg) ^ sz));
                        const uint4 q = *(const uint4 *)(a + (mi * 32 + st * 16) * KC + 4 * ((2 * kg + 1) ^ sz));
                        const uint4 h8 = make_uint4(__builtin_amdgcn_perm(p.y, p.x, 0x05040100u), __builtin_amdgcn_perm(p.w, p.z, 0x05040100u),
                                                    __builtin_amdgcn_perm(q.y, q.x, 0x05040100u), __builtin_amdgcn_perm(q.w, q.z, 0x05040100u));
                        const uint4 l8 = make_uint4(__builtin_amdgcn_perm(p.y, p.x, 0x07060302u), __builtin_amdgcn_perm(p.w, p.z, 0x07060302u),
                                                    __builtin_amdgcn_perm(q.y, q.x, 0x07060302u), __builtin_amdgcn_perm(q.w, q.z, 0x07060302u));
                        acc_v4 &c0 = acc4[M16 ? 2 * mi + st : 0][0], &c1 = acc4[M16 ? 2 * mi + st : 0][1];
                        c0 = mma16(l8, w0, c0); c1 = mma16(l8, w2, c1);
                        c0 = mma16(h8, w1, c0); c1 = mma16(h8, w3, c1);
                        c0 = mma16(h8, w0, c0); c1 = mma16(h8, w2, c1);
                    }
            } else
#pragma unroll
            for (int st = 0; st < 2; ++st) {
#pragma unroll
                for (int mi = 0; mi < RT; ++mi) {
                    const uint4 p = *(const uint4 *)(a + mi * 32 * KC + 4 * ((4 * st + 2 * hi) ^ ((l31 >> 1) & 7)));
                    const uint4 q = *(const uint4 *)(a + mi * 32 * KC + 4 * ((4 * st + 2 * hi + 1) ^ ((l31 >> 1) & 7)));
                    ah[mi] = make_uint4(__builtin_amdgcn_perm(p.y, p.x, 0x05040100u), __builtin_amdgcn_perm(p.w, p.z, 0x05040100u),
                                        __builtin_amdgcn_perm(q.y, q.x, 0x05040100u), __builtin_amdgcn_perm(q.w, q.z, 0x05040100u));
                    al[mi] = make_uint4(__builtin_amdgcn_perm(p.y, p.x, 0x07060302u), __builtin_amdgcn_perm(p.w, p.z, 0x07060302u),
                                        __builtin_amdgcn_perm(q.y, q.x, 0x07060302u), __builtin_amdgcn_perm(q.w, q.z, 0x07060302u));
                }
                const wv4 &wh = st ? w2 : w0, &wl = st ? w3 : w1;
#pragma unroll
                for (int mi = 0; mi < RT; ++mi) acc[mi][0] = mmaw(al[mi], wh, acc[mi][0]);
#pragma unroll
                for (int mi = 0; mi < RT; ++mi) acc[mi][0] = mmaw(ah[mi], wl, acc[mi][0]);
#pragma unroll
                for (int mi = 0; mi < RT; ++mi) acc[mi][0] = mmaw(ah[mi], wh, acc[mi][0]);
            }
        };
#if PD_STRIP_PIPE
        wv4 raw[2][RT][2];
        const int swz = M16 ? pd_strip_swz<true>(l15) : (l31 >> 1) & 7;
        auto read_mi = [&](int rb, const unsigned *a, int st, int mi) {
            const unsigned p_ = (unsigned)(size_t)(M16 ? a + (mi * 32 + st * 16) * KC + 4 * ((2 * kg) ^ swz) : a + mi * 32 * KC + 4 * ((4 * st + 2 * hi) ^ swz));
            const unsigned q_ = (unsigned)(size_t)(M16 ? a + (mi * 32 + st * 16) * KC + 4 * ((2 * kg + 1) ^ swz) : a + mi * 32 * KC + 4 * ((4 * st + 2 * hi + 1) ^ swz));
            asm volatile("ds_read_b128 %0, %2\n\tds_read_b128 %1, %3" : "=&v"(raw[rb][mi][0]), "=&v"(raw[rb][mi][1]) : "v"(p_), "v"(q_) : "memory");
        };
        auto wait_reads = [&](int rb) {
#pragma unroll
            for (int mi = 0; mi < RT; ++mi) asm volatile("s_waitcnt lgkmcnt(0)" : "+v"(raw[rb][mi][0]), "+v"(raw[rb][mi][1]) : : "memory");
        };
        int dma_cn = 0, dma_nb = 0;
        auto dma_piece_at = [&](int p) {
            const unsigned da = __builtin_amdgcn_readfirstlane(lds_a + dma_nb * 2 * CHA * 4);
            const int h = p / RT, j = p % RT;
            pd_dma_piece((const float *)(g.A + (2 * dma_cn + h) * KC), oa[j], da + h * CHA * 4 + j * 1024);
        };
        auto step = [&](int rb, const wv4 &wh, const wv4 &wl, bool has_next, int nrb, const unsigned *na, int nst, int dma_step) {
            uint4 ah[RT], al[RT];
#pragma unroll
            for (int mi = 0; mi < RT; ++mi) {
                const wv4 p = raw[rb][mi][0], q = raw[rb][mi][1];
#ifdef PD_STRIP_NOPERM
                al[mi] = make_uint4(q.x, q.y, q.z, q.w);
#else
                al[mi] = make_uint4(__builtin_amdgcn_perm(p.y, p.x, 0x07060302u), __builtin_amdgcn_perm(p.w, p.z, 0x07060302u),
                                    __builtin_amdgcn_perm(q.y, q.x, 0x07060302u), __builtin_amdgcn_perm(q.w, q.z, 0x07060302u));
#endif
                __builtin_amdgcn_sched_barrier(0);
                acc[mi][0] = mmaw(al[mi], wh, acc[mi][0]);
                __builtin_amdgcn_sched_barrier(0);
            }
#pragma unroll
            for (int mi = 0; mi < RT; ++mi) {
                const wv4 p = raw[rb][mi][0], q = raw[rb][mi][1];
#ifdef PD_STRIP_NOPERM
                ah[mi] = make_uint4(p.x, p.y, p.z, p.w);
#else
                ah[mi] = make_uint4(__builtin_amdgcn_perm(p.y, p.x, 0x05040100u), __builtin_amdgcn_perm(p.w, p.z, 0x05040100u),
                                    __builtin_amdgcn_perm(q.y, q.x, 0x05040100u), __builtin_amdgcn_perm(q.w, q.z, 0x05040100u));
#endif
                if (has_next) read_mi(nrb, na, nst, mi);
                __builtin_amdgcn_sched_barrier(0);
                acc[mi][0] = mmaw(ah[mi], wl, acc[mi][0]);
                __builtin_amdgcn_sched_barrier(0);
            }
#pragma unroll
            for (int mi = 0; mi < RT; ++mi) {
                if (dma_step >= 0) dma_piece_at(dma_step * RT + mi);
                __builtin_amdgcn_sched_barrier(0);
                acc[mi][0] = mmaw(ah[mi], wh, acc[mi][0]);
                __builtin_amdgcn_sched_barrier(0);
            }
        };
        auto step16 = [&](int rb, int h, const wv4 &w0, const wv4 &w1, const wv4 &w2, const wv4 &w3, bool has_next, int nrb, const unsigned *na, int nst,
                          int dma_step) {
            uint4 ah[RT], al[RT];
#pragma unroll
            for (int mi = 0; mi < RT; ++mi) {
                const wv4 p = raw[rb][mi][0], q = raw[rb][mi][1];
                const int t = M16 ? 2 * mi + h : 0;
                al[mi] = make_uint4(__builtin_amdgcn_perm(p.y, p.x, 0x07060302u), __builtin_amdgcn_perm(p.w, p.z, 0x07060302u),
                                    __builtin_amdgcn_perm(q.y, q.x, 0x07060302u), __builtin_amdgcn_perm(q.w, q.z, 0x07060302u));
                __builtin_amdgcn_sched_barrier(0);
                acc4[t][0] = mma16(al[mi], w0, acc4[t][0]);
                acc4[t][1] = mma16(al[mi], w2, acc4[t][1]);
                __builtin_amdgcn_sched_barrier(0);
            }
#pragma unroll
            for (int mi = 0; mi < RT; ++mi) {
                const wv4 p = raw[rb][mi][0], q = raw[rb][mi][1];
                const int t = M16 ? 2 * mi + h : 0;
                ah[mi] = make_uint4(__builtin_amdgcn_perm(p.y, p.x, 0x05040100u), __builtin_amdgcn_perm(p.w, p.z, 0x05040100u),
                                    __builtin_amdgcn_perm(q.y, q.x, 0x05040100u), __builtin_amdgcn_perm(q.w, q.z, 0x05040100u));
                if (has_next) read_mi(nrb, na, nst, mi);
                __builtin_amdgcn_sched_barrier(0);
                acc4[t][0] = mma16(ah[mi], w1, acc4[t][0]);
                acc4[t][1] = mma16(ah[mi], w3, acc4[t][1]);
                __builtin_amdgcn_sched_barrier(0);
            }
#pragma unroll
            for (int mi = 0; mi < RT; ++mi) {
                const int t = M16 ? 2 * mi + h : 0;
                if (dma_step >= 0) dma_piece_at(dma_step * RT + mi);
                __builtin_amdgcn_sched_barrier(0);
                acc4[t][0] = mma16(ah[mi], w0, acc4[t][0]);
                acc4[t][1] = mma16(ah[mi], w2, acc4[t][1]);
                __builtin_amdgcn_sched_barrier(0);
            }
        };
#endif
        wv4 a0, a1, a2, a3, b0, b1, b2, b3;
        const int nk64 = g.K / 64;
        auto resid_load = [&]() {
            const int pr_ = lane >> 3, colb_ = n0 + wave * 32 + (lane & 7) * 4;
#pragma unroll
            for (int mi = 0; mi < RT; ++mi)
#pragma unroll
                for (int q = 0; q < 4; ++q) {
                    const float *rp_ = (const float *)g.C + (size_t)min(m0 + mi * 32 + 8 * q + pr_, g.M - 1) * g.Nout + colb_;
                    asm volatile("global_load_dwordx4 %0, %1, off" : "=&v"(resid[mi][q]) : "v"(rp_) : "memory");
                }
        };
        auto resid_wait = [&]() {
#pragma unroll
            for (int mi = 0; mi < ((EPI == 2) ? RT : 1); ++mi)
                asm volatile("s_waitcnt vmcnt(0)" : "+v"(resid[mi][0]), "+v"(resid[mi][1]), "+v"(resid[mi][2]), "+v"(resid[mi][3]) : : "memory");
        };
        stage64(0, 0);
        PD_STRIP_WLOAD(a0, a1, a2, a3, 0);
        PD_STRIP_WLOAD(b0, b1, b2, b3, 1);
        PD_STRIP_WAIT(0, a0, a1, a2, a3);
        PD_STRIP_WAIT(0, b0, b1, b2, b3);
        __syncthreads();
        PD_LEG(3, __builtin_amdgcn_s_memtime());
#ifdef PD_STRIP_LEGS
        long long leg_t0 = 0, leg_wb = 0, leg_wa = 0, leg_bar = 0, leg_s0 = 0, leg_s1 = 0, leg_s2 = 0, leg_s3 = 0;
#define PD_LEG_T0() leg_t0 = __builtin_amdgcn_s_memtime()
#define PD_LEG_ACC(v) v += __builtin_amdgcn_s_memtime() - leg_t0
#else
#define PD_LEG_T0() do { } while (0)
#define PD_LEG_ACC(v) do { } while (0)
#endif
        constexpr int RESN = (PD_STRIP_RES_AHEAD && EPI == 2) ? 4 * RT : 0;
        auto chunk = [&](int c, auto mode_) {
            constexpr int MODE = decltype(mode_)::value;
            const int cn = c + 1;
            const unsigned *a = strip_lds + (c & 1) * 2 * CHA + (M16 ? l15 : l31) * KC;
#if PD_STRIP_PIPE
            dma_cn = cn;
            dma_nb = (c + 1) & 1;
#pragma unroll
            for (int mi = 0; mi < RT; ++mi) read_mi(0, a, 0, mi);
            wait_reads(0);
            PD_LEG_T0();
            if constexpr (M16) step16(0, 0, a0, a1, a2, a3, true, 1, a, 1, MODE == 2 ? -1 : 0);
            else step(0, a0, a1, true, 1, a, 1, MODE == 2 ? -1 : 0);
            PD_LEG_ACC(leg_s0);
            wait_reads(1);
            PD_LEG_T0();
            if constexpr (M16) step16(1, 1, a0, a1, a2, a3, true, 0, a + CHA, 0, MODE == 2 ? -1 : 1);
            else step(1, a2, a3, true, 0, a + CHA, 0, MODE == 2 ? -1 : 1);
            PD_LEG_ACC(leg_s1);
#else
            if constexpr (MODE != 2) stage64(cn, (c + 1) & 1);
            block(a, a0, a1, a2, a3);
#endif
            if constexpr (MODE != 2) PD_STRIP_WLOAD(a0, a1, a2, a3, 2 * cn);
            PD_LEG_T0();
            PD_STRIP_WAITN((MODE == 2 ? RESN : 2 * RT + 4), b0, b1, b2, b3);
            PD_LEG_ACC(leg_wb);
#if PD_STRIP_PIPE
            wait_reads(0);
            PD_LEG_T0();
            if constexpr (M16) step16(0, 0, b0, b1, b2, b3, true, 1, a + CHA, 1, -1);
            else step(0, b0, b1, true, 1, a + CHA, 1, -1);
            PD_LEG_ACC(leg_s2);
            wait_reads(1);
            PD_LEG_T0();
            if constexpr (M16) step16(1, 1, b0, b1, b2, b3, false, 0, a, 0, -1);
            else step(1, b2, b3, false, 0, a, 0, -1);
            PD_LEG_ACC(leg_s3);
#else
            block(a + CHA, b0, b1, b2, b3);
#endif
            if constexpr (MODE != 2) {
                PD_STRIP_WLOAD(b0, b1, b2, b3, 2 * cn + 1);
                if constexpr (MODE == 1 && RESN > 0) resid_load();
                PD_LEG_T0();
                PD_STRIP_WAITN((MODE == 1 ? 4 + RESN : 4), a0, a1, a2, a3);
                PD_LEG_ACC(leg_wa);
                PD_LEG_T0();
                __syncthreads();
                PD_LEG_ACC(leg_bar);
            }
        };
        if constexpr (RESN > 0) {
            if (nk64 < 2) {
                resid_load();
                resid_wait();
            }
        }
        for (int c = 0; c < nk64 - 2; ++c) chunk(c, std::integral_constant<int, 0>());
        if (nk64 >= 2) chunk(nk64 - 2, std::integral_constant<int, 1>());
        chunk(nk64 - 1, std::integral_constant<int, 2>());
        PD_STRIP_WAIT(0, b0, b1, b2, b3);
#if PD_STRIP_RES_AHEAD
        if constexpr (EPI == 2) {
            resid_wait();
        }
#endif
        PD_LEG(4, __builtin_amdgcn_s_memtime());
#ifdef PD_STRIP_LEGS
        PD_LEG(6, (leg_wb << 32) | (leg_wa & 0xffffffffll));
        PD_LEG(7, leg_bar);
#ifdef PD_STRIP_STEP_CLOCKS
        PD_LEG(0, (leg_s0 << 32) | (leg_s1 & 0xffffffffll));
        PD_LEG(1, (leg_s2 << 32) | (leg_s3 & 0xffffffffll));
#endif
#endif
#undef PD_STRIP_WLOAD
#undef PD_STRIP_WAIT
#undef PD_STRIP_WAITN
    } else {
#pragma unroll
    for (int c = 0; c < CT; ++c)
#pragma unroll
        for (int st = 0; st < 2; ++st)
#pragma unroll
            for (int pl = 0; pl < 2; ++pl) cw[c][st][pl] = wq[(size_t)c * KS * 128 + (size_t)(st * 2 + pl) * 64];
    stage(0, 0);
    asm volatile("s_waitcnt vmcnt(0)" ::: "memory");
    __syncthreads();
#pragma unroll
    for (int mi = 0; mi < RT; ++mi)
#pragma unroll
        for (int c = 0; c < CT; ++c)
#pragma unroll
            for (int i = 0; i < 16; ++i) acc[mi][c][i] = 0.0f;
    const int nk = g.K / KC, sw = (l31 >> 1) & 7;
    for (int kc = 0; kc < nk; ++kc) {
        const int nc = min(kc + 1, nk - 1);
        if constexpr (BARE == 0 || BARE == 2 || BARE >= 5) {
#pragma unroll
            for (int c = 0; c < CT; ++c)
#pragma unroll
                for (int st = 0; st < 2; ++st)
#pragma unroll
                    for (int pl = 0; pl < 2; ++pl) nw[c][st][pl] = wq[(size_t)c * KS * 128 + (size_t)(nc * 4 + st * 2 + pl) * 64];
        }
        if constexpr (BARE == 0 || BARE == 1 || BARE >= 5) stage(nc, (kc + 1) & 1);
        const unsigned *a = strip_lds + (BARE == 6 ? 0 : (kc & 1)) * CHA + l31 * KC;
        uint4 ah[RT], al[RT];
#pragma unroll
        for (int st = 0; st < 2; ++st) {
            if (BARE != 6 || kc == 0)
#pragma unroll
            for (int mi = 0; mi < RT; ++mi) {
                const uint4 p = *(const uint4 *)(a + mi * 32 * KC + 4 * ((4 * st + 2 * hi) ^ sw));
                const uint4 q = *(const uint4 *)(a + mi * 32 * KC + 4 * ((4 * st + 2 * hi + 1) ^ sw));
                ah[mi] = make_uint4(__builtin_amdgcn_perm(p.y, p.x, 0x05040100u), __builtin_amdgcn_perm(p.w, p.z, 0x05040100u),
                                    __builtin_amdgcn_perm(q.y, q.x, 0x05040100u), __builtin_amdgcn_perm(q.w, q.z, 0x05040100u));
                al[mi] = make_uint4(__builtin_amdgcn_perm(p.y, p.x, 0x07060302u), __builtin_amdgcn_perm(p.w, p.z, 0x07060302u),
                                    __builtin_amdgcn_perm(q.y, q.x, 0x07060302u), __builtin_amdgcn_perm(q.w, q.z, 0x07060302u));
            }
            if constexpr (BARE != 5) {
#pragma unroll
                for (int mi = 0; mi < RT; ++mi)
#pragma unroll
                    for (int c = 0; c < CT; ++c) acc[mi][c] = mma(al[mi], cw[c][st][0], acc[mi][c]);
#pragma unroll
                for (int mi = 0; mi < RT; ++mi)
#pragma unroll
                    for (int c = 0; c < CT; ++c) acc[mi][c] = mma(ah[mi], cw[c][st][1], acc[mi][c]);
#pragma unroll
                for (int mi = 0; mi < RT; ++mi)
#pragma unroll
                    for (int c = 0; c < CT; ++c) acc[mi][c] = mma(ah[mi], cw[c][st][0], acc[mi][c]);
            } else {
#pragma unroll
                for (int mi = 0; mi < RT; ++mi) acc[mi][0][st] += __uint_as_float(al[mi].x ^ ah[mi].w ^ cw[0][st][0].y ^ cw[0][st][1].z);
            }
        }
        if constexpr (BARE == 0 || BARE == 2 || BARE >= 5) {
#pragma unroll
            for (int c = 0; c < CT; ++c)
#pragma unroll
                for (int st = 0; st < 2; ++st)
#pragma unroll
                    for (int pl = 0; pl < 2; ++pl) cw[c][st][pl] = nw[c][st][pl];
        }
        if constexpr (BARE != 4) {
            asm volatile("s_waitcnt vmcnt(0)" ::: "memory");
            __syncthreads();
        }
    }
    }
#if PD_STRIP_WIDE_EPI
    if constexpr (BARE == 0 && K64) {
        static_assert(PD_STRIP_PATCH_BYTES <= pd_gemm_strip_lds<RT, K64>(), "the four waves' patches live in the launch's dynamic LDS");
        __syncthreads();
        float *patch = (float *)strip_lds + wave * (32 * 36);
        const int pr = lane >> 3, pc = (lane & 7) * 4;
#pragma unroll
        for (int c = 0; c < CT; ++c) {
            const int colb = n0 + (CT * wave + c) * 32 + pc;
            const float4 bias4 = *(const float4 *)(g.bias + colb);
#pragma unroll
            for (int mi = 0; mi < RT; ++mi) {
                if constexpr (M16) {
#pragma unroll
                    for (int h = 0; h < 2; ++h)
#pragma unroll
                        for (int ct = 0; ct < 2; ++ct)
#pragma unroll
                            for (int i = 0; i < 4; ++i) patch[(16 * h + 4 * kg + i) * 36 + 16 * ct + l15] = acc4[M16 ? 2 * mi + h : 0][ct][i];
                } else
#pragma unroll
                for (int i = 0; i < 16; ++i) patch[((i & 3) + 8 * (i >> 2) + 4 * hi) * 36 + l31] = acc[mi][c][i];
                float4 res4[4];
                if constexpr (EPI == 2) {
#pragma unroll
                    for (int q = 0; q < 4; ++q) {
#if PD_STRIP_RES_AHEAD
                        res4[q] = __builtin_bit_cast(float4, resid[mi][q]);
#else
                        res4[q] = *(const float4 *)((const float *)g.C + (size_t)min(m0 + mi * 32 + 8 * q + pr, g.M - 1) * g.Nout + colb);
#endif
                    }
                }
#pragma unroll
                for (int q = 0; q < 4; ++q) {
                    const int row = m0 + mi * 32 + 8 * q + pr;
                    const float4 a4 = *(const float4 *)(patch + (8 * q + pr) * 36 + pc);
                    float v[4] = {a4.x, a4.y, a4.z, a4.w};
                    const float b4[4] = {bias4.x, bias4.y, bias4.z, bias4.w};
                    const float r4[4] = {EPI == 2 ? res4[q].x : 0.0f, EPI == 2 ? res4[q].y : 0.0f, EPI == 2 ? res4[q].z : 0.0f, EPI == 2 ? res4[q].w : 0.0f};
                    unsigned o[4];
#pragma unroll
                    for (int e = 0; e < 4; ++e) {
                        float t = F16 ? fmaf(v[e], g.c_scale, b4[e]) : v[e] + b4[e];
                        if constexpr (EPI == 3) t = F16 ? 0.5f * t * (1.0f + erff(t * 0.70710678118654752f)) : vit_gelu_fast(t);
                        if constexpr (EPI == 4) t = pd_relu(t);
                        if constexpr (EPI == 2) t += r4[e];
                        if constexpr (EPI == 3 || EPI == 4) o[e] = pd_split_word_as<F16 ? 2 : 1>(t, g.out_scale);
                        else o[e] = __float_as_uint(t);
                    }
                    if (row < g.M) *(uint4 *)((unsigned *)g.C + (size_t)row * g.Nout + colb) = make_uint4(o[0], o[1], o[2], o[3]);
                }
            }
        }
    } else
#endif
#pragma unroll
    for (int c = 0; c < CT; ++c) {
        const int col = n0 + (CT * wave + c) * 32 + l31;
        const float bias = g.bias[col];
#pragma unroll
        for (int mi = 0; mi < RT; ++mi) {
            const int r0 = m0 + mi * 32 + 4 * hi;
            float res[16];
            if constexpr (EPI == 2) {
#pragma unroll
                for (int i = 0; i < 16; ++i) res[i] = ((const float *)g.C)[(size_t)min(r0 + (i & 3) + 8 * (i >> 2), g.M - 1) * g.Nout + col];
            }
#pragma unroll
            for (int i = 0; i < 16; ++i) {
                const int row = r0 + (i & 3) + 8 * (i >> 2);
                float v = F16 ? fmaf(acc[mi][c][i], g.c_scale, bias) : acc[mi][c][i] + bias;
                if constexpr (EPI == 3) v = F16 ? 0.5f * v * (1.0f + erff(v * 0.70710678118654752f)) : vit_gelu_fast(v);
                if constexpr (EPI == 4) v = pd_relu(v);
                if constexpr (EPI == 2) v += res[i];
                if (row < g.M) {
                    if constexpr (EPI == 3 || EPI == 4)
                        ((unsigned *)g.C)[(size_t)row * g.Nout + col] = pd_split_word_as<F16 ? 2 : 1>(v, g.out_scale);
                    else
                        ((float *)g.C)[(size_t)row * g.Nout + col] = v;
                }
            }
        }
    }
#ifdef PD_STRIP_LEGS
    asm volatile("s_waitcnt vmcnt(0)" ::: "memory");
    PD_LEG(5, __builtin_amdgcn_s_memtime());
#ifndef PD_STRIP_STEP_CLOCKS
    PD_LEG(1, wall_clock64());
#endif
#endif
}
template <int EPI, int RT, bool F16, int CT = 1, bool K64 = false>
static inline void pd_gemm_strip(const unsigned *A, int lda, const unsigned *W, int K, const float *bias, void *C, int M, int Nout, hipStream_t s,
                                 float c_scale = 1.0f, float out_scale = 1.0f) {
    VitSplitArgs g{A, W, bias, C, M, Nout, K, lda, c_scale, out_scale};
    constexpr int TM = 32 * RT;
    hipLaunchKernelGGL((pd_gemm_strip_kernel<EPI, RT, F16, CT, 0, K64>), dim3(((M + TM - 1) / TM) * (Nout / (128 * CT))), dim3(256),
                       (pd_gemm_strip_lds<RT, K64>()), s, g);
}

static constexpr size_t pd_split_lds(int WM) { return (size_t)2 * 64 * WM * PD_STREAM_LR * sizeof(float); }
template <int EPI, int WM, int WN, bool F16 = false>
static inline void pd_gemm_split(const unsigned *A, int lda, const unsigned *W, int K, const float *bias, void *C, int M, int Nout, hipStream_t s,
                                 float c_scale = 1.0f, float out_scale = 1.0f) {
    VitSplitArgs g{A, W, bias, C, M, Nout, K, lda, c_scale, out_scale};
    constexpr int TM = 64 * WM, TN = 64 * WN;
    hipLaunchKernelGGL((vit_gemm_split_kernel<EPI, WM, WN, F16>), dim3(((M + TM - 1) / TM) * (Nout / TN)), dim3(256), pd_split_lds(WM), s, g);
}
```

posediffusion_amd/csrc/pd_gemm_stream.h:

```cpp
#pragma once
#include "pd_internal.h"

typedef float f32x16 __attribute__((ext_vector_type(16)));
typedef __bf16 bf16x8 __attribute__((ext_vector_type(8)));
typedef _Float16 f16x8 __attribute__((ext_vector_type(8)));

__device__ __forceinline__ unsigned pd_split_word(float v) {
    const __bf16 h = (__bf16)v;
    const __bf16 l = (__bf16)(v - (float)h);
    return (unsigned)__builtin_bit_cast(unsigned short, h) | ((unsigned)__builtin_bit_cast(unsigned short, l) << 16);
}

__device__ __forceinline__ unsigned pd_split_word_h(float v) {
    const _Float16 h = (_Float16)v;
    const _Float16 l = (_Float16)(v - (float)h);
    return (unsigned)__builtin_bit_cast(unsigned short, h) | ((unsigned)__builtin_bit_cast(unsigned short, l) << 16);
}
template <int SPLIT>
__device__ __forceinline__ unsigned pd_split_word_as(float v, float scale) {
    if constexpr (SPLIT == 2) return pd_split_word_h(v * scale);
    return pd_split_word(v);
}

template <int CTRL>
__device__ __forceinline__ float pd_stream_dpp_add(float v) {
    return v + __int_as_float(__builtin_amdgcn_update_dpp(0, __float_as_int(v), CTRL, 0xf, 0xf, false));
}
__device__ __forceinline__ float pd_stream_sum8(float v) {
    v = pd_stream_dpp_add<0xB1>(v);
    v = pd_stream_dpp_add<0x4E>(v);
    return pd_stream_dpp_add<0x141>(v);
}

template <int D, int SPLIT>
__global__ __launch_bounds__(256) void pd_ln_rows_kernel(const float *__restrict__ x, float *__restrict__ xn, int M, float eps, float scale) {
    constexpr int PER = D / 64;
    static_assert(D % 64 == 0, "one wave per row");
    const int row = blockIdx.x * 4 + (threadIdx.x >> 6), lane = threadIdx.x & 63;
    if (row >= M) return;
    const float *src = x + (size_t)row * D;
    float v[PER], s = 0.0f;
#pragma unroll
    for (int i = 0; i < PER; ++i) {
        v[i] = src[lane + 64 * i];
        s += v[i];
    }
#pragma unroll
    for (int off = 32; off >= 1; off >>= 1) s += __shfl_xor(s, off, 64);
    const float mean = s * (1.0f / D);
    float q = 0.0f;
#pragma unroll
    for (int i = 0; i < PER; ++i) q += (v[i] - mean) * (v[i] - mean);
#pragma unroll
    for (int off = 32; off >= 1; off >>= 1) q += __shfl_xor(q, off, 64);
    const float rstd = 1.0f / sqrtf(q * (1.0f / D) + eps);
#pragma unroll
    for (int i = 0; i < PER; ++i) {
        const float o = (v[i] - mean) * rstd;
        if constexpr (SPLIT != 0)
            ((unsigned *)xn)[(size_t)row * D + lane + 64 * i] = pd_split_word_as<SPLIT>(o, scale);
        else
            xn[(size_t)row * D + lane + 64 * i] = o;
    }
}
template <int D>
__global__ __launch_bounds__(256) void pd_ln_stats_kernel(const float *__restrict__ x, float2 *__restrict__ stats, int M, float eps) {
    constexpr int PER = D / 64;
    static_assert(D % 256 == 0, "one wave per row, float4 per lane");
    const int row = blockIdx.x * 4 + (threadIdx.x >> 6), lane = threadIdx.x & 63;
    if (row >= M) return;
    const float4 *src = (const float4 *)(x + (size_t)row * D) + lane;
    float4 v[PER / 4];
    float s = 0.0f;
#pragma unroll
    for (int i = 0; i < PER / 4; ++i) {
        v[i] = src[64 * i];
        s += (v[i].x + v[i].y) + (v[i].z + v[i].w);
    }
#pragma unroll
    for (int off = 32; off >= 1; off >>= 1) s += __shfl_xor(s, off, 64);
    const float mean = s * (1.0f / D);
    float q = 0.0f;
#pragma unroll
    for (int i = 0; i < PER / 4; ++i)
        q += ((v[i].x - mean) * (v[i].x - mean) + (v[i].y - mean) * (v[i].y - mean)) + ((v[i].z - mean) * (v[i].z - mean) + (v[i].w - mean) * (v[i].w - mean));
#pragma unroll
    for (int off = 32; off >= 1; off >>= 1) q += __shfl_xor(q, off, 64);
    if (lane == 0) stats[row] = make_float2(mean, 1.0f / sqrtf(q * (1.0f / D) + eps));
}

struct PdStreamArgs {
    const float *A, *W, *bias;
    float *C;
    int M, Nout, K, lda, ldw;
    const float2 *ln_stats;
    const float *R;
    const int *t_row;
};
#define PD_STREAM_KC 32
#define PD_STREAM_LR (PD_STREAM_KC + 4)
#define VS_EACH(X) X(0) X(1) X(2) X(3)

template <int EPI, int WM, int WN, bool ALN = false, int BARE = 0>
__global__ __launch_bounds__(256) void pd_gemm_stream_kernel(PdStreamArgs g) {
    constexpr int KC = PD_STREAM_KC, LR = PD_STREAM_LR, TM = 64 * WM, TN = 64 * WN, PA = 2 * WM, PW = 2 * WN, GROUP = 2048 / TM;
    static_assert(KC == 32 && PA <= 4 && PW <= 4, "staging: 8 float4 per row, passes of 32 rows");
    extern __shared__ __attribute__((aligned(16))) float lds[];
    float *As = lds, *Ws = lds + 2 * TM * LR;
    const int tid = threadIdx.x, lane = tid & 63, wave = tid >> 6, l31 = lane & 31, hi = lane >> 5, wm = wave & 1, wn = wave >> 1;
    const int MT = (g.M + TM - 1) / TM, NT = g.Nout / TN;
    int mtile, ntile;
    {
        const int b = blockIdx.x, full = (MT / GROUP) * GROUP * NT;
        if (b < full) {
            const int grp = b / (NT * GROUP), r = b - grp * (NT * GROUP);
            ntile = r / GROUP;
            mtile = grp * GROUP + r % GROUP;
        } else {
            const int r = b - full, rest = MT % GROUP;
            ntile = r / rest;
            mtile = (MT / GROUP) * GROUP + r % rest;
        }
    }
    const int m0 = mtile * TM, n0 = ntile * TN;
    const int sr = tid >> 3, sc = tid & 7, st = sr * LR + 4 * sc;
#define VS_DECL(j)                                                                                                        \
    const float4 *ap##j = (const float4 *)(g.A + (size_t)min(m0 + sr + 32 * (j < PA ? j : 0), g.M - 1) * g.lda) + sc;       \
    const float4 *wp##j = (const float4 *)(g.W + (size_t)(n0 + sr + 32 * (j < PW ? j : 0)) * g.ldw) + sc;                   \
    float4 ra##j, rw##j;
#define VS_LOAD(j)                       \
    if constexpr (j < PA) ra##j = ap##j[nx]; \
    if constexpr (j < PW) rw##j = wp##j[nx];
#define VS_STORE(j)                                                                                          \
    if constexpr (j < PA) {                                                                                   \
        float4 t_ = ra##j;                                                                                    \
        if constexpr (ALN) {                                                                                  \
            t_.x = (t_.x - ln_mu[j < PA ? j : 0]) * ln_rs[j < PA ? j : 0];                                    \
            t_.y = (t_.y - ln_mu[j < PA ? j : 0]) * ln_rs[j < PA ? j : 0];                                    \
            t_.z = (t_.z - ln_mu[j < PA ? j : 0]) * ln_rs[j < PA ? j : 0];                                    \
            t_.w = (t_.w - ln_mu[j < PA ? j : 0]) * ln_rs[j < PA ? j : 0];                                    \
        }                                                                                                     \
        *(float4 *)(da + st + j * 32 * LR) = t_;                                                              \
    }                                                                                                         \
    if constexpr (j < PW) *(float4 *)(dw + st + j * 32 * LR) = rw##j;
    VS_EACH(VS_DECL)
    float ln_mu[PA], ln_rs[PA];
    if constexpr (ALN) {
#pragma unroll
        for (int j = 0; j < PA; ++j) {
            const float2 st2 = g.ln_stats[min(m0 + sr + 32 * j, g.M - 1)];
            ln_mu[j] = st2.x;
            ln_rs[j] = st2.y;
        }
    }
    {
        const int nx = 0;
        float *da = As, *dw = Ws;
        VS_EACH(VS_LOAD)
        VS_EACH(VS_STORE)
    }
    __syncthreads();
    f32x16 acc[WM][WN];
#pragma unroll
    for (int mi = 0; mi < WM; ++mi)
#pragma unroll
        for (int ni = 0; ni < WN; ++ni)
#pragma unroll
            for (int i = 0; i < 16; ++i) acc[mi][ni][i] = 0.0f;
    const int nk = g.K / KC;
    const int aoff = (wm * 32 * WM + l31) * LR + 4 * hi, boff = (wn * 32 * WN + l31) * LR + 4 * hi;
    auto mma_chunk = [&](int buf) {
        const float *a = As + buf * TM * LR + aoff, *b = Ws + buf * TN * LR + boff;
#pragma unroll
        for (int kk = 0; kk < KC / 8; ++kk) {
            float4 af[WM], bf[WN];
#pragma unroll
            for (int mi = 0; mi < WM; ++mi) af[mi] = (BARE != 3) ? *(const float4 *)(a + mi * 32 * LR + kk * 8) : make_float4(1.f + kk, 2.f, 3.f, 4.f);
#pragma unroll
            for (int ni = 0; ni < WN; ++ni) bf[ni] = (BARE != 3) ? *(const float4 *)(b + ni * 32 * LR + kk * 8) : make_float4(1.f, 2.f + kk, 3.f, 4.f);
#pragma unroll
            for (int mi = 0; mi < WM; ++mi)
#pragma unroll
                for (int ni = 0; ni < WN; ++ni) {
                    acc[mi][ni] = __builtin_amdgcn_mfma_f32_32x32x2f32(af[mi].x, bf[ni].x, acc[mi][ni], 0, 0, 0);
                    acc[mi][ni] = __builtin_amdgcn_mfma_f32_32x32x2f32(af[mi].y, bf[ni].y, acc[mi][ni], 0, 0, 0);
                    acc[mi][ni] = __builtin_amdgcn_mfma_f32_32x32x2f32(af[mi].z, bf[ni].z, acc[mi][ni], 0, 0, 0);
                    acc[mi][ni] = __builtin_amdgcn_mfma_f32_32x32x2f32(af[mi].w, bf[ni].w, acc[mi][ni], 0, 0, 0);
                }
        }
    };
    for (int kc = 0; kc < nk; ++kc) {
        const int nx = min(kc + 1, nk - 1) * (KC / 4);
        if constexpr (BARE == 0 || BARE == 4) {
            VS_EACH(VS_LOAD)
        }
        __builtin_amdgcn_sched_barrier(0);
        mma_chunk(kc & 1);
        __builtin_amdgcn_sched_barrier(0);
        float *da = As + ((kc + 1) & 1) * TM * LR, *dw = Ws + ((kc + 1) & 1) * TN * LR;
        if constexpr (BARE == 0 || BARE == 5) {
            VS_EACH(VS_STORE)
        }
        if constexpr (BARE == 4) {
            asm volatile("" ::"v"(ra0.x), "v"(ra1.x), "v"(rw0.x), "v"(rw1.x));
        }
        if constexpr (BARE < 2 || BARE >= 4) __syncthreads();
    }
#undef VS_DECL
// ... 218 lines not shown
```

posediffusion_amd/csrc/pd_internal.h:

```cpp
#pragma once

#include <hip/hip_runtime.h>
#include <stdint.h>
#include <stdio.h>
#include <string>
#include <vector>

#include "../../include/pd_engine.h"

#define PD_WAVE 64
#define PD_MAX_FRAMES 64
#define PD_GGS_LONG_MAX_FRAMES 256
#define PD_MAX_DENOISER_FRAMES 256
#define PD_GGS_THREADS 512
#define PD_GGS_WAVES (PD_GGS_THREADS / PD_WAVE)
#define PD_GGS_PINC_ROWS (2 * PD_GGS_THREADS)
#define PD_GGS_MAX_PCHUNKS 8
#define PD_GGS_MAX_STAGES 5
#define PD_ITEM_MAX_MATCHES 512
#define PD_ITEM_VALS 12
#ifndef PD_LANE_WAVES
#define PD_LANE_WAVES 8
#endif
#define PD_LANE_THREADS (PD_LANE_WAVES * PD_WAVE)
// ... 55 lines not shown
struct PdGgsStage {
    int update_R, update_T, update_FL, iters;
};

struct PdGgsParams {
    const PdSeqDesc *seqs;
    float *x;
    int N, k;
    PdGgsStage stages[PD_GGS_MAX_STAGES];
    int n_stages;
    float alpha, lr, sampson_max, momentum;
    int min_matches;
    int eval_only;
    float *stats;
    float *trace;
    int trace_iters;
    float *loss_out;
    float *grad_out;
    unsigned long long *xchg;
    int xchg_stride;
    unsigned int *err_flag;
    long long *prof;
    int prof_wave;
    int n_seqs;
    unsigned long long *stamp;
    int xchg_local;
};

__host__ __device__ inline void pd_interleave_pair(const float4 a, const float4 b, float4 &q0, float4 &q1) {
    q0 = make_float4(a.x, b.x, a.y, b.y);
    q1 = make_float4(a.z, b.z, a.w, b.w);
}

struct PdGgsPlan {
    int k, n_slots, lds, two_hop, max_items;
    int pinc_rows, stage_p;
    int waves;
    int lane, lane_rl;
    int xchg_local;
    int long_frames;
};

__host__ __device__ inline int pd_lane_items_of(int m, int len) { return (m + len - 1) / len; }
__host__ __device__ inline int pd_cut_len(int m, int nch, int c) { return m / nch + (c < m % nch ? 1 : 0); }

struct PdBlobArrays {
    size_t pts, pij, pio, itm, ptb, pco, gps, gio, lit, lwv, lpt, lst;
};
inline size_t pd_al256(size_t v) { return (v + 255) & ~(size_t)255; }
inline size_t pd_blob_layout(const PdBlobArrays &n, PdBlobArrays &o) {
    o.pts = 0;
    o.pij = pd_al256(o.pts + sizeof(float4) * n.pts);
    o.pio = pd_al256(o.pij + sizeof(int2) * n.pij);
    o.itm = pd_al256(o.pio + sizeof(int) * n.pio);
    o.ptb = pd_al256(o.itm + sizeof(int4) * n.itm);
    o.pco = pd_al256(o.ptb + sizeof(int4) * n.ptb);
    o.gps = pd_al256(o.pco + sizeof(int) * n.pco);
    o.gio = pd_al256(o.gps + sizeof(int2) * n.gps);
    o.lit = pd_al256(o.gio + sizeof(int) * n.gio);
    o.lwv = pd_al256(o.lit + sizeof(int4) * n.lit);
    o.lpt = pd_al256(o.lwv + sizeof(int2) * n.lwv);
    o.lst = pd_al256(o.lpt + sizeof(int2) * n.lpt);
    return pd_al256(o.lst + sizeof(float4) * n.lst);
}
inline void pd_desc_point_into(PdSeqDesc &d, char *base, const PdBlobArrays &o) {
    d.pts = (const float4 *)(base + o.pts);
    d.pair_ij = (const int2 *)(base + o.pij);
    d.pair_item_off = (const int *)(base + o.pio);
    d.items = (const int4 *)(base + o.itm);
    d.ptab = (const int4 *)(base + o.ptb);
    d.pchunk_off = (const int *)(base + o.pco);
    d.gpos = (const int2 *)(base + o.gps);
    d.ginc_off = (const int *)(base + o.gio);
    d.litems = (const int4 *)(base + o.lit);
    d.lwave = (const int2 *)(base + o.lwv);
    d.lptab = (const int2 *)(base + o.lpt);
    d.lstream = (const float4 *)(base + o.lst);
}
__host__ __device__ inline int pd_lane_rank(const int *val, const int *nch, int n, int p, bool by_steps) {
    const int vp = by_steps ? val[p] : pd_lane_items_of(val[p], nch[p]);
    int r = 0;
    for (int q = 0; q < n; ++q) {
        if (nch[q] == 0 || q == p) continue;
        const int vq = by_steps ? val[q] : pd_lane_items_of(val[q], nch[q]);
        if (vq > vp || (vq == vp && q < p)) r += by_steps ? nch[q] : 1;
    }
    return r;
}

#ifndef PD_LANE_MORE_MAX
#define PD_LANE_MORE_MAX 3
#endif
#ifndef PD_LANE_MORE_SLACK
#define PD_LANE_MORE_SLACK 16
#endif
__host__ __device__ inline int pd_lane_pass_cost(const int *T, const int *Tmin) {
    int c = 0;
    for (int s = 0; s < 4; ++s) {
        int t1 = 100 * T[s] + 15 * (T[s] - Tmin[s]), t2 = 0;
        for (int w = s + 4; w < PD_LANE_WAVES; w += 4) t2 += 100 * T[w] + 15 * (T[w] - Tmin[w]);
        const int a = t1, b = (45 * t1) / 100 + t2;
        c = c > a ? c : a;
        c = c > b ? c : b;
    }
    return c;
}

struct PdSeqHost {
    void *blob = nullptr;
    size_t blob_bytes = 0;
    PdSeqDesc desc{};
    int n_local_max_k1 = 0;
    int max_item_len = 0;
    int max_deg = 0;
    bool device_built = false;
};

struct PdSeqTables {
    std::vector<float4> pts, lstream;
    std::vector<int2> pair_ij, gpos, lwave, lptab;
    std::vector<int> pair_item_off, pchunk_off, ginc_off;
    std::vector<int4> items, ptab, litems;
    int n_pchunks = 0, single_item_pairs = 1, l_item_len = 0, l_max_steps = 0;
    int max_item_len = 0, max_deg = 0;
};

struct PdDenoiserDev;
struct PdGenericDen;

struct pd_engine {
    int device = 0;
    int num_cus = 0;
    int max_B = 0, max_N = 0;
    int d_model = 0, nhead = 0, dim_ff = 0, num_layers = 0, z_dim = 0, timesteps = 0;
    PdDenoiserDev *den = nullptr;
    PdGenericDen *gden = nullptr;
    std::vector<float> c_recip, c_recipm1, coef1, coef2, logvar;
    int pred_x0 = 0;
    float *d_c_recip = nullptr, *d_c_recipm1 = nullptr;
    float *d_q_a = nullptr, *d_q_b = nullptr;
    int *d_t_row = nullptr;
    float *d_xt = nullptr;
    int nf_B = 0;
    std::vector<int> nf_host;
    int *d_nf = nullptr;
    std::vector<PdSeqHost> seqs;
    PdSeqDesc *d_seqs = nullptr;
    unsigned long long *d_xchg = nullptr;
    size_t xchg_granules = 0;
    int ggs_max_frames = PD_MAX_FRAMES;
    int ggs_long_pair_items = 0;
    unsigned int *d_err = nullptr;
    int ggs_prof_on = 0;
    int den_fused_attn = 1;
    int den_long_attn = 0;
    int den_split = 0;
    int gemm_wide_min_tiles = 200;
    float *d_stats_scratch = nullptr;
    unsigned long long *d_stamps = nullptr;
    int stamp_slot = 0;
    float *d_z = nullptr, *d_noise = nullptr, *d_process = nullptr, *d_mean = nullptr, *d_stats = nullptr;
    struct GraphKey {
        int B, N, cond_start, has_ggs, phase, den_split;
        pd_ggs_cfg cfg;
        PdGgsPlan plan;
    };
    std::vector<std::pair<GraphKey, hipGraphExec_t>> graphs;
    hipStream_t own_stream = nullptr;
    struct StreamEvent {
        hipStream_t stream;
        hipEvent_t event;
    };
    std::vector<StreamEvent> uses, uploads;
    struct RetiredBlob {
        void *ptr;
        hipEvent_t done;
    };
    std::vector<RetiredBlob> retired_blobs;
};

int pd_denoiser_create(pd_engine *eng, const pd_weights *w);
void pd_denoiser_destroy(pd_engine *eng);
bool pd_denoiser_has_streamed_path(const pd_engine *eng);
bool pd_denoiser_weights_non_finite(const pd_engine *eng);
int pd_denoiser_build_split(pd_engine *eng, int mode);
struct PdTSeq {
    const int *t_row;
    const float *target;
    float *loss_out;
    int loss_type;
};
int pd_denoiser_launch(pd_engine *eng, const float *x, const float *z, int t, int B, int N, float *eps_out,
                       float *mean_out, float *x0_out, const float *noise, float *x_next_out, hipStream_t s, bool z_prepared = false,
                       const PdTSeq *ts = nullptr);
int pd_denoiser_t_rows(pd_engine *eng, const int64_t *t_seq, int B, int N, hipStream_t s);
int pd_denoiser_q_sample(pd_engine *eng, const float *x_start, const float *noise, const int64_t *t_seq, int B, int N, float *xt, hipStream_t s);
void pd_den_first_gemm_t(const PdDenoiserDev *d, const int *t_row, int M, hipStream_t s);
int pd_denoiser_prepare(pd_engine *eng, const float *z, int B, int N, hipStream_t s);

int pd_time_table(const pd_weights *w, float *table);
bool pd_denoiser_generic_shape_ok(const pd_weights *w, char *why, size_t why_len);
int pd_denoiser_generic_create(pd_engine *eng, const pd_weights *w);
void pd_denoiser_generic_destroy(pd_engine *eng);
int pd_denoiser_generic_launch(pd_engine *eng, const float *x, const float *z, int t, int B, int N, float *eps_out, float *mean_out,
                               float *x0_out, const float *noise, float *x_next_out, hipStream_t s, const PdTSeq *ts = nullptr);

int pd_ggs_init();
int pd_ggs_plan(pd_engine *eng, int B, int N, const pd_ggs_cfg *cfg, PdGgsPlan *out);
int pd_ggs_launch(pd_engine *eng, float *x, int B, int N, const PdGgsStage *stages, int n_stages,
                  const pd_ggs_cfg *cfg, int eval_only, float *stats, float *trace, int trace_iters,
                  float *loss_out, float *grad_out, hipStream_t s);
int pd_build_seq_tables(const double *kp1, const double *kp2, const int64_t *i12, int64_t M, int n_frames, PdSeqTables &out);
void pd_ggs_free_seq(PdSeqHost &h);
int pd_ggs_ingest_init();
int pd_ggs_frames_unsupported(const pd_engine *eng, int N, const char *who);
int pd_frame_counts(const pd_engine *eng, int B, int N, const char *who, const int **nf_dev);
bool pd_stream_capturing(hipStream_t s);
int pd_wait_uploads(pd_engine *eng, hipStream_t s);
int pd_mark_use(pd_engine *eng, hipStream_t s);
int pd_record_stream_event(std::vector<pd_engine::StreamEvent> &list, hipStream_t s);
int pd_wait_uses(pd_engine *eng, hipStream_t s, bool host);
void pd_free_retired_blobs(pd_engine *eng);
#define PD_GRAPH_CACHE_MAX 8
#define PD_STAMP_SLOTS 128
```

posediffusion_amd/csrc/pd_qkv_attn.h:

```cpp
#pragma once
#include "pd_gemm_split.h"

#ifndef PD_QA_XCD_MAP
#define PD_QA_XCD_MAP 1
#endif
#define PD_QA_WAVES 12
#define PD_QA_THREADS (PD_QA_WAVES * 64)
#define PD_QA_ROWS 96
#define PD_QA_LDR (3 * DH + 4)
#define PD_QA_LS 36
#ifndef PD_QA_DEEP_DEFAULT
#define PD_QA_DEEP_DEFAULT 0
#endif

struct PdQkvAttnArgs {
    const unsigned *A;
    const unsigned *W;
    const float *bias;
    unsigned *ctx;
    int B, N, G;
    float c_scale, out_scale;
};
static inline int pd_qkv_attn_group(int N) { return N >= 1 && N <= 32 ? (PD_QA_ROWS - 1) / N : 0; }
static inline int pd_qkv_attn_wgs(int B, int N) {
    const int G = pd_qkv_attn_group(N);
    return G ? ((B + G - 1) / G) * NH : 0;
}
static inline size_t pd_qkv_attn_lds(int N) {
    const int G = pd_qkv_attn_group(N);
    const size_t image = (size_t)(G * N + 1) * PD_QA_LDR * sizeof(float);
    const size_t stage = (size_t)4 * PD_QA_ROWS * 32 * sizeof(unsigned);
    return (image > stage ? image : stage) + (size_t)3 * 32 * PD_QA_LS * sizeof(float);
}

template <int BARE, bool DEEP = false>
__global__ __launch_bounds__(PD_QA_THREADS) void pd_qkv_attn_kernel(PdQkvAttnArgs g) {
    constexpr int KC = 32, RT = 3, TM = PD_QA_ROWS, CHA = TM * KC, LDR = PD_QA_LDR, LS = PD_QA_LS;
    constexpr bool M16 = PD_STRIP_MFMA16 != 0;
    extern __shared__ __attribute__((aligned(1024))) unsigned qa_lds[];
    const int tid = threadIdx.x, lane = tid & 63, l31 = lane & 31, hi = lane >> 5;
    const int wave = __builtin_amdgcn_readfirstlane(tid >> 6);
    int head = blockIdx.x & 3, grp = blockIdx.x >> 2;
#if PD_QA_XCD_MAP == 1
    {
        const int ngrp = gridDim.x >> 2, c = blockIdx.x >> 4, r = blockIdx.x & 15;
        if (4 * c + 4 <= ngrp) {
            head = 2 * ((r & 7) >> 2) + (r >> 3);
            grp = 4 * c + (r & 3);
        }
    }
#elif PD_QA_XCD_MAP == 2
    {
        const int ngrp = gridDim.x >> 2, c = blockIdx.x >> 5, r = blockIdx.x & 31;
        if (8 * c + 8 <= ngrp) {
            head = r >> 3;
            grp = 8 * c + (r & 7);
        }
    }
#endif
    const int N = g.N, G = g.G, M = g.B * N;
    const int seq0 = grp * G, nseq = min(G, g.B - seq0), m0 = seq0 * N, rows = nseq * N;
    const int nt16 = __builtin_amdgcn_readfirstlane((rows + 15) >> 4);
    const int stages = __builtin_amdgcn_readfirstlane(8 * wave < 16 * nt16 ? 1 : 0);
    const int prow = lane >> 3, pslot = lane & 7, l15 = lane & 15, kg = lane >> 4;
    unsigned oa;
    {
        const int r = 8 * wave + prow;
        oa = (unsigned)(((size_t)min(m0 + r, M - 1) * DM + 4 * (pslot ^ pd_strip_swz<M16>(r))) * sizeof(unsigned));
    }
    const unsigned lds_a = (unsigned)(size_t)(qa_lds + wave * 256);
    const int third = wave >> 2;
    const int ntile = third * (DM / 32) + head * (DH / 32) + (wave & 3);
    constexpr int KS = DM / 16;
    const uint4 *wq = (const uint4 *)g.W + (size_t)ntile * KS * 128 + (M16 ? (kg >> 1) * 128 + (kg & 1) * 32 + l15 : lane);
    typedef unsigned wv4 __attribute__((ext_vector_type(4)));
    f32x16 acc[M16 ? 1 : RT];
    f32x4 acc4[M16 ? 2 * RT : 1][2];
#pragma unroll
    for (int mi = 0; mi < (M16 ? 1 : RT); ++mi)
#pragma unroll
        for (int i = 0; i < 16; ++i) acc[mi][i] = 0.0f;
#pragma unroll
    for (int t = 0; t < (M16 ? 2 * RT : 1); ++t) acc4[t][0] = acc4[t][1] = f32x4{0.f, 0.f, 0.f, 0.f};
    auto mmaw = [](const uint4 &a, const wv4 &b, const f32x16 &c) {
        return __builtin_amdgcn_mfma_f32_32x32x16_f16(__builtin_bit_cast(f16x8, a), __builtin_bit_cast(f16x8, b), c, 0, 0, 0);
    };
    auto mma16 = [](const uint4 &a, const wv4 &b, const f32x4 &c) {
        return __builtin_amdgcn_mfma_f32_16x16x32_f16(__builtin_bit_cast(f16x8, a), __builtin_bit_cast(f16x8, b), c, 0, 0, 0);
    };
#define PD_QA_WLOAD(w0, w1, w2, w3, b)                                                                                               \
    do {                                                                                                                             \
        const uint4 *wp_ = wq + (size_t)(b) * 256;                                                                                   \
        if constexpr (M16)                                                                                                           \
            asm volatile("global_load_dwordx4 %0, %4, off\n\tglobal_load_dwordx4 %1, %4, off offset:1024\n\t"                       \
                         "global_load_dwordx4 %2, %4, off offset:256\n\tglobal_load_dwordx4 %3, %4, off offset:1280"                 \
                         : "=&v"(w0), "=&v"(w1), "=&v"(w2), "=&v"(w3) : "v"(wp_) : "memory");                                        \
        else                                                                                                                         \
            asm volatile("global_load_dwordx4 %0, %4, off\n\tglobal_load_dwordx4 %1, %4, off offset:1024\n\t"                       \
                         "global_load_dwordx4 %2, %4, off offset:2048\n\tglobal_load_dwordx4 %3, %4, off offset:3072"                \
                         : "=&v"(w0), "=&v"(w1), "=&v"(w2), "=&v"(w3) : "v"(wp_) : "memory");                                        \
    } while (0)
#define PD_QA_WAIT(n, w0, w1, w2, w3) asm volatile("s_waitcnt vmcnt(" #n ")" : "+v"(w0), "+v"(w1), "+v"(w2), "+v"(w3) : : "memory")
#define PD_QA_WAIT_STAGED(stg, w0, w1, w2, w3)                                                                                       \
    asm volatile("s_cmp_eq_u32 %4, 0\n\ts_cbranch_scc1 .Lqa_ns%=\n\ts_waitcnt vmcnt(6)\n\ts_branch .Lqa_done%=\n"                   \
                 ".Lqa_ns%=:\n\ts_waitcnt vmcnt(4)\n.Lqa_done%=:"                                                                   \
                 : "+v"(w0), "+v"(w1), "+v"(w2), "+v"(w3) : "s"(__builtin_amdgcn_readfirstlane(stg)) : "memory", "scc")
    auto stage64 = [&](int c, int buf) {
        if (!stages) return;
        const unsigned da = __builtin_amdgcn_readfirstlane(lds_a + buf * 2 * CHA * 4);
#pragma unroll
        for (int h = 0; h < 2; ++h) pd_dma_piece((const float *)(g.A + (2 * c + h) * KC), oa, da + h * CHA * 4);
    };
    auto block = [&](auto nt_, const unsigned *a, const wv4 &w0, const wv4 &w1, const wv4 &w2, const wv4 &w3) {
        constexpr int NT = decltype(nt_)::value;
        if constexpr (M16) {
            const int sz = pd_strip_swz<true>(l15);
#pragma unroll
            for (int t = 0; t < NT; ++t) {
                const uint4 p = *(const uint4 *)(a + t * 16 * KC + 4 * ((2 * kg) ^ sz));
                const uint4 q = *(const uint4 *)(a + t * 16 * KC + 4 * ((2 * kg + 1) ^ sz));
                const uint4 h8 = make_uint4(__builtin_amdgcn_perm(p.y, p.x, 0x05040100u), __builtin_amdgcn_perm(p.w, p.z, 0x05040100u),
                                            __builtin_amdgcn_perm(q.y, q.x, 0x05040100u), __builtin_amdgcn_perm(q.w, q.z, 0x05040100u));
                const uint4 l8 = make_uint4(__builtin_amdgcn_perm(p.y, p.x, 0x07060302u), __builtin_amdgcn_perm(p.w, p.z, 0x07060302u),
                                            __builtin_amdgcn_perm(q.y, q.x, 0x07060302u), __builtin_amdgcn_perm(q.w, q.z, 0x07060302u));
                f32x4 &c0 = acc4[M16 ? t : 0][0], &c1 = acc4[M16 ? t : 0][1];
                c0 = mma16(l8, w0, c0); c1 = mma16(l8, w2, c1);
                c0 = mma16(h8, w1, c0); c1 = mma16(h8, w3, c1);
                c0 = mma16(h8, w0, c0); c1 = mma16(h8, w2, c1);
            }
        } else {
        uint4 ah[RT], al[RT];
#pragma unroll
        for (int st = 0; st < 2; ++st) {
#pragma unroll
            for (int mi = 0; mi < RT; ++mi) {
                const uint4 p = *(const uint4 *)(a + mi * 32 * KC + 4 * ((4 * st + 2 * hi) ^ ((l31 >> 1) & 7)));
                const uint4 q = *(const uint4 *)(a + mi * 32 * KC + 4 * ((4 * st + 2 * hi + 1) ^ ((l31 >> 1) & 7)));
                ah[mi] = make_uint4(__builtin_amdgcn_perm(p.y, p.x, 0x05040100u), __builtin_amdgcn_perm(p.w, p.z, 0x05040100u),
                                    __builtin_amdgcn_perm(q.y, q.x, 0x05040100u), __builtin_amdgcn_perm(q.w, q.z, 0x05040100u));
                al[mi] = make_uint4(__builtin_amdgcn_perm(p.y, p.x, 0x07060302u), __builtin_amdgcn_perm(p.w, p.z, 0x07060302u),
                                    __builtin_amdgcn_perm(q.y, q.x, 0x07060302u), __builtin_amdgcn_perm(q.w, q.z, 0x07060302u));
            }
            const wv4 &wh = st ? w2 : w0, &wl = st ? w3 : w1;
#pragma unroll
            for (int mi = 0; mi < RT; ++mi) acc[M16 ? 0 : mi] = mmaw(al[mi], wh, acc[M16 ? 0 : mi]);
#pragma unroll
            for (int mi = 0; mi < RT; ++mi) acc[M16 ? 0 : mi] = mmaw(ah[mi], wl, acc[M16 ? 0 : mi]);
#pragma unroll
            for (int mi = 0; mi < RT; ++mi) acc[M16 ? 0 : mi] = mmaw(ah[mi], wh, acc[M16 ? 0 : mi]);
        }
        }
    };
    const int lrow = M16 ? l15 : l31;
    auto kloop = [&](auto nt_) {
        wv4 a0, a1, a2, a3, b0, b1, b2, b3;
        constexpr int nk64 = DM / 64;
        stage64(0, 0);
        PD_QA_WLOAD(a0, a1, a2, a3, 0);
        PD_QA_WLOAD(b0, b1, b2, b3, 1);
        PD_QA_WAIT(0, a0, a1, a2, a3);
        PD_QA_WAIT(0, b0, b1, b2, b3);
        __syncthreads();
        if constexpr (DEEP) {
            static_assert(!DEEP || BARE == 0, "the deep form has no development variants");
            wv4 c0, c1, c2, c3, d0, d1, d2, d3;
            for (int c = 0; c < nk64; c += 2) {
                {
                    const unsigned *a = qa_lds + 0 * 2 * CHA + lrow * KC;
                    stage64(c + 1, 1);
                    PD_QA_WLOAD(c0, c1, c2, c3, 2 * (c + 1));
                    PD_QA_WLOAD(d0, d1, d2, d3, 2 * (c + 1) + 1);
                    block(nt_, a, a0, a1, a2, a3);
                    block(nt_, a + CHA, b0, b1, b2, b3);
                    PD_QA_WAIT(0, c0, c1, c2, c3);
                    PD_QA_WAIT(0, d0, d1, d2, d3);
                    __syncthreads();
                }
                {
                    const int cn = min(c + 2, nk64 - 1);
                    const unsigned *a = qa_lds + 1 * 2 * CHA + lrow * KC;
                    stage64(cn, 0);
                    PD_QA_WLOAD(a0, a1, a2, a3, 2 * cn);
                    PD_QA_WLOAD(b0, b1, b2, b3, 2 * cn + 1);
                    block(nt_, a, c0, c1, c2, c3);
                    block(nt_, a + CHA, d0, d1, d2, d3);
                    PD_QA_WAIT(0, a0, a1, a2, a3);
                    PD_QA_WAIT(0, b0, b1, b2, b3);
                    __syncthreads();
                }
            }
        } else
        for (int c = 0; c < nk64; ++c) {
            const int cn = min(c + 1, nk64 - 1);
            const unsigned *a = qa_lds + (c & 1) * 2 * CHA + lrow * KC;
            if constexpr (BARE == 0) {
                if (c + 1 < nk64) {
                    stage64(cn, (c + 1) & 1);
                    block(nt_, a, a0, a1, a2, a3);
                    PD_QA_WLOAD(a0, a1, a2, a3, 2 * cn);
                    PD_QA_WAIT_STAGED(stages, b0, b1, b2, b3);
                    block(nt_, a + CHA, b0, b1, b2, b3);
                    PD_QA_WLOAD(b0, b1, b2, b3, 2 * cn + 1);
                    PD_QA_WAIT(4, a0, a1, a2, a3);
                } else {
                    block(nt_, a, a0, a1, a2, a3);
                    PD_QA_WAIT(0, b0, b1, b2, b3);
                    block(nt_, a + CHA, b0, b1, b2, b3);
                }
            } else {
                if constexpr (BARE != 2 && BARE != 3) stage64(cn, (c + 1) & 1);
                if constexpr (BARE != 4) block(nt_, a, a0, a1, a2, a3);
                if constexpr (BARE != 1 && BARE != 3) PD_QA_WLOAD(a0, a1, a2, a3, 2 * cn);
                if constexpr (BARE != 4) block(nt_, a + CHA, b0, b1, b2, b3);
                if constexpr (BARE != 1 && BARE != 3) PD_QA_WLOAD(b0, b1, b2, b3, 2 * cn + 1);
                PD_QA_WAIT(0, a0, a1, a2, a3);
                PD_QA_WAIT(0, b0, b1, b2, b3);
            }
            __syncthreads();
        }
        PD_QA_WAIT(0, b0, b1, b2, b3);
    };
    if constexpr (M16) {
        switch (nt16) {
        case 1: kloop(std::integral_constant<int, 1>()); break;
        case 2: kloop(std::integral_constant<int, 2>()); break;
        case 3: kloop(std::integral_constant<int, 3>()); break;
        case 4: kloop(std::integral_constant<int, 4>()); break;
        case 5: kloop(std::integral_constant<int, 5>()); break;
        default: kloop(std::integral_constant<int, 6>()); break;
        }
    } else {
        kloop(std::integral_constant<int, 6>());
    }
#undef PD_QA_WLOAD
#undef PD_QA_WAIT
#undef PD_QA_WAIT_STAGED
    if constexpr (BARE == 5) {
        if (acc[0][0] + acc4[0][0][0] == 123.456f) g.ctx[tid] = 1u;
        return;
    }
    float *img = (float *)qa_lds;
    float *Sall = img + (size_t)(G * N + 1) * LDR;
    {
        const float qscale = 0.08838834764831845f;
        if constexpr (M16) {
#pragma unroll
            for (int ct = 0; ct < 2; ++ct) {
                const float bias = g.bias[ntile * 32 + 16 * ct + l15];
                const int lcol = third * DH + (wave & 3) * 32 + 16 * ct + l15;
#pragma unroll
                for (int t = 0; t < 2 * RT; ++t)
#pragma unroll
                    for (int i = 0; i < 4; ++i) {
                        const int row = 16 * t + 4 * kg + i;
                        float v = fmaf(acc4[M16 ? t : 0][ct][i], g.c_scale, bias);
                        if (third == 0) v *= qscale;
                        if (row < rows) img[row * LDR + lcol] = v;
                    }
            }
        } else {
        const int col = ntile * 32 + l31;
        const float bias = g.bias[col];
        const int lcol = third * DH + (wave & 3) * 32 + l31;
#pragma unroll
        for (int mi = 0; mi < RT; ++mi)
#pragma unroll
            for (int i = 0; i < 16; ++i) {
                const int row = mi * 32 + 4 * hi + (i & 3) + 8 * (i >> 2);
                float v = fmaf(acc[M16 ? 0 : mi][i], g.c_scale, bias);
                if (third == 0) v *= qscale;
                if (row < rows) img[row * LDR + lcol] = v;
            }
        }
        for (int c = tid; c < LDR; c += PD_QA_THREADS) img[G * N * LDR + c] = 0.0f;
    }
    __syncthreads();
    const int team = wave >> 2, tw = wave & 3, ttid = tid & 255;
    float *S = Sall + team * 32 * LS;
    const int rounds = (G + 2) / 3;
    for (int rd = 0; rd < rounds; ++rd) {
        const int s = rd * 3 + team;
        const bool active = s < nseq;
        const float *base = img + (size_t)s * N * LDR;
        const float *zrow = img + (size_t)G * N * LDR;
        auto rowp = [&](int j) { return j < N ? base + j * LDR : zrow; };
        if (active) {
            const float *qa = rowp(16 * (tw >> 1) + (lane & 15)) + 4 * (lane >> 4);
            const float *kb = rowp(16 * (tw & 1) + (lane & 15)) + DH + 4 * (lane >> 4);
            f32x4 sc = {0.f, 0.f, 0.f, 0.f};
#pragma unroll
            for (int c = 0; c < DH / 16; ++c) {
                const float4 a = *(const float4 *)(qa + 16 * c), k = *(const float4 *)(kb + 16 * c);
                sc = __builtin_amdgcn_mfma_f32_16x16x4f32(a.x, k.x, sc, 0, 0, 0);
                sc = __builtin_amdgcn_mfma_f32_16x16x4f32(a.y, k.y, sc, 0, 0, 0);
                sc = __builtin_amdgcn_mfma_f32_16x16x4f32(a.z, k.z, sc, 0, 0, 0);
                sc = __builtin_amdgcn_mfma_f32_16x16x4f32(a.w, k.w, sc, 0, 0, 0);
            }
            const int j = 16 * (tw & 1) + (lane & 15);
#pragma unroll
            for (int e = 0; e < 4; ++e) S[(16 * (tw >> 1) + 4 * (lane >> 4) + e) * LS + j] = sc[e];
        }
        __syncthreads();
        if (active) {
            const int i = ttid >> 3, sub = ttid & 7;
            float4 sv = *(const float4 *)(S + i * LS + 4 * sub);
            const int j0 = 4 * sub;
            sv.x = j0 + 0 < N ? sv.x : -INFINITY;
            sv.y = j0 + 1 < N ? sv.y : -INFINITY;
            sv.z = j0 + 2 < N ? sv.z : -INFINITY;
            sv.w = j0 + 3 < N ? sv.w : -INFINITY;
            float mx = fmaxf(fmaxf(sv.x, sv.y), fmaxf(sv.z, sv.w));
            mx = fmaxf(mx, __shfl_xor(mx, 1, 64));
            mx = fmaxf(mx, __shfl_xor(mx, 2, 64));
            mx = fmaxf(mx, __shfl_xor(mx, 4, 64));
            float4 e;
            e.x = j0 + 0 < N ? expf(sv.x - mx) : 0.0f;
            e.y = j0 + 1 < N ? expf(sv.y - mx) : 0.0f;
            e.z = j0 + 2 < N ? expf(sv.z - mx) : 0.0f;
            e.w = j0 + 3 < N ? expf(sv.w - mx) : 0.0f;
            const float inv = 1.0f / pd_sum8((e.x + e.y) + (e.z + e.w));
            e.x *= inv; e.y *= inv; e.z *= inv; e.w *= inv;
            *(float4 *)(S + i * LS + 4 * sub) = e;
        }
        __syncthreads();
        if (active) {
            f32x4 o[2][2];
#pragma unroll
            for (int rt = 0; rt < 2; ++rt)
#pragma unroll
                for (int ct = 0; ct < 2; ++ct) o[rt][ct] = f32x4{0.f, 0.f, 0.f, 0.f};
            const float *pa = S + (lane & 15) * LS + 4 * (lane >> 4);
            const int vcol = 2 * DH + 32 * tw + (lane & 15);
            const int jg = 4 * (lane >> 4);
#pragma unroll
            for (int c = 0; c < 2; ++c) {
                const float4 p0 = *(const float4 *)(pa + 16 * c), p1 = *(const float4 *)(pa + 16 * LS + 16 * c);
                float v0[4], v1[4];
#pragma unroll
                for (int e = 0; e < 4; ++e) {
                    const float *vr = rowp(16 * c + jg + e) + vcol;
                    v0[e] = vr[0];
                    v1[e] = vr[16];
                }
                const float a0[4] = {p0.x, p0.y, p0.z, p0.w}, a1[4] = {p1.x, p1.y, p1.z, p1.w};
#pragma unroll
                for (int e = 0; e < 4; ++e) {
                    o[0][0] = __builtin_amdgcn_mfma_f32_16x16x4f32(a0[e], v0[e], o[0][0], 0, 0, 0);
                    o[0][1] = __builtin_amdgcn_mfma_f32_16x16x4f32(a0[e], v1[e], o[0][1], 0, 0, 0);
                    o[1][0] = __builtin_amdgcn_mfma_f32_16x16x4f32(a1[e], v0[e], o[1][0], 0, 0, 0);
                    o[1][1] = __builtin_amdgcn_mfma_f32_16x16x4f32(a1[e], v1[e], o[1][1], 0, 0, 0);
                }
            }
#pragma unroll
            for (int rt = 0; rt < 2; ++rt)
#pragma unroll
                for (int e = 0; e < 4; ++e) {
                    const int i = 16 * rt + 4 * (lane >> 4) + e;
                    if (i < N) {
                        unsigned *out = g.ctx + (size_t)((seq0 + s) * N + i) * DM + head * DH + 32 * tw + (lane & 15);
#pragma unroll
                        for (int ct = 0; ct < 2; ++ct) out[16 * ct] = pd_split_word_as<2>(o[rt][ct][e], g.out_scale);
                    }
                }
        }
        __syncthreads();
    }
}

static inline void pd_qkv_attn(const unsigned *hn, const unsigned *Wh, const float *bias, unsigned *ctx, int B, int N, float c_scale, float out_scale,
                               hipStream_t s) {
    PdQkvAttnArgs g{hn, Wh, bias, ctx, B, N, pd_qkv_attn_group(N), c_scale, out_scale};
    const dim3 grid(pd_qkv_attn_wgs(B, N)), blk(PD_QA_THREADS);
    const size_t lds = pd_qkv_attn_lds(N);
#ifdef PD_DEV_KNOBS
    static const int bare = pd_dev_knob("PD_QA_BARE", 0);
    static const int deep = pd_dev_knob("PD_QA_DEEP", PD_QA_DEEP_DEFAULT);
    if (bare == 0 && !deep) { hipLaunchKernelGGL((pd_qkv_attn_kernel<0, false>), grid, blk, lds, s, g); return; }
    switch (bare) {
    case 1: hipLaunchKernelGGL(pd_qkv_attn_kernel<1>, grid, blk, lds, s, g); return;
    case 2: hipLaunchKernelGGL(pd_qkv_attn_kernel<2>, grid, blk, lds, s, g); return;
    case 3: hipLaunchKernelGGL(pd_qkv_attn_kernel<3>, grid, blk, lds, s, g); return;
    case 4: hipLaunchKernelGGL(pd_qkv_attn_kernel<4>, grid, blk, lds, s, g); return;
    case 5: hipLaunchKernelGGL(pd_qkv_attn_kernel<5>, grid, blk, lds, s, g); return;
    default: break;
    }
#endif
    hipLaunchKernelGGL((pd_qkv_attn_kernel<0, PD_QA_DEEP_DEFAULT != 0>), grid, blk, lds, s, g);
}
```

Before: 1113.

## Store denoiser activations as separate fp16 hi/lo planes for strip GEMMs

```diff
diff --git a/include/pd_engine.h b/include/pd_engine.h
--- a/include/pd_engine.h
+++ b/include/pd_engine.h
@@ -134,6 +134,7 @@
 #define PD_OPT_DENOISER_LONG_ATTN 6
 #define PD_OPT_GGS_MAX_FRAMES 7
 #define PD_OPT_GGS_LONG_PAIR_ITEMS 8
+#define PD_OPT_DENOISER_ACT_PLANES 9
 int pd_engine_set_option(pd_engine *eng, int option, int value);
 #define PD_OPT_WEIGHTS_NON_FINITE 4
 int pd_engine_get_option(pd_engine *eng, int option, int *value_out);
diff --git a/posediffusion_amd/_lib.py b/posediffusion_amd/_lib.py
--- a/posediffusion_amd/_lib.py
+++ b/posediffusion_amd/_lib.py
@@ -83,6 +83,7 @@
 PD_OPT_DENOISER_FUSED_ATTN = 5
 PD_OPT_DENOISER_LONG_ATTN = 6
 PD_OPT_GGS_MAX_FRAMES = 7
+PD_OPT_DENOISER_ACT_PLANES = 9
 PD_OPT_GGS_LONG_PAIR_ITEMS = 8
 PD_DROP_ATTN, PD_DROP_RESID1, PD_DROP_FF, PD_DROP_RESID2, PD_DROP_ALL = 1, 2, 4, 8, 15
 PD_TR_OPT_MAX_FRAMES, PD_TR_OPT_LONG_ATTN = 1, 2
diff --git a/posediffusion_amd/csrc/pd_denoiser.hip b/posediffusion_amd/csrc/pd_denoiser.hip
--- a/posediffusion_amd/csrc/pd_denoiser.hip
+++ b/posediffusion_amd/csrc/pd_denoiser.hip
@@ -304,6 +304,7 @@
 }
 static void den_layer_f16(const PdDenoiserDev *d, const PdLayerDev &L, const PdDenStepPlan &p, const int *nf, int B, int N, hipStream_t s) {
     const int M = p.M;
+    if (p.act_planes) return pd_den_layer_f16_planes(d, L, B, N, p.rt_res == 3, p.rt_ff1 == 3, s);
     hipLaunchKernelGGL((pd_ln_rows_kernel<DM, 2>), dim3((M + 3) / 4), dim3(256), 0, s, d->h, d->hn, M, 1e-5f, 512.0f);
     if (p.fused_attn) {
         pd_qkv_attn((const unsigned *)d->hn, L.qkv_wh, L.qkv_b, (unsigned *)d->ctx, B, N, L.qkv_cs, L.ctx_scale, s);
@@ -380,7 +381,7 @@
     }
     static const int knob_strip = pd_dev_knob("PD_DEN_STRIP", 15), knob_attn_mma = pd_dev_knob("PD_DEN_ATTN_MMA", 1);
     const PdDenStepPlan p = pd_den_step_plan(B, N, eng->den_split, eng->den_fused_attn, eng->num_cus, d->hn != nullptr, d->split_ready,
-                                             d->split_h_ready, knob_strip, knob_attn_mma, eng->den_long_attn, nf != nullptr);
+                                             d->split_h_ready, knob_strip, knob_attn_mma, eng->den_long_attn, nf != nullptr, eng->den_act_planes);
     const bool small = p.path == PD_DEN_SMALL;
     const int M = p.M;
     GemmArgs g;
diff --git a/posediffusion_amd/csrc/pd_denoiser_plan.h b/posediffusion_amd/csrc/pd_denoiser_plan.h
--- a/posediffusion_amd/csrc/pd_denoiser_plan.h
+++ b/posediffusion_amd/csrc/pd_denoiser_plan.h
@@ -29,10 +29,11 @@
     bool attn_mma;
     int rt_res, rt_ff1;
     int strip;
+    bool act_planes;
 };
 
 static inline PdDenStepPlan pd_den_step_plan(int B, int N, int split, int fused_attn, int num_cus, bool has_streamed, bool split_ready,
-                                             bool split_h_ready, int knob_strip, int knob_attn_mma, int long_attn = 0, bool ragged = false) {
+                                             bool split_h_ready, int knob_strip, int knob_attn_mma, int long_attn = 0, bool ragged = false, int act_planes = 1) {
     PdDenStepPlan p = {};
     p.M = B * N;
     p.MT = (p.M + 31) / 32;
@@ -51,5 +52,6 @@
     p.rt_res = !rt3 ? 2 : PD_STRIP_RT1 ? 1 : 3;
     p.rt_ff1 = !rt3 ? 2 : PD_STRIP_RT1 == 2 ? 1 : PD_STRIP_RT3_FF1 ? 3 : 2;
     p.strip = knob_strip;
+    p.act_planes = act_planes != 0 && p.fused_attn && p.strip == 15 && PD_STRIP_RT1 == 0 && PD_STRIP_K64 && PD_STRIP_MFMA16 != 0 && PD_STRIP_WIDE_EPI != 0 && PD_STRIP_PIPE != 0;
     return p;
 }
diff --git a/posediffusion_amd/csrc/pd_denoiser_planes.hip b/posediffusion_amd/csrc/pd_denoiser_planes.hip
--- /dev/null
+++ b/posediffusion_amd/csrc/pd_denoiser_planes.hip
@@ -0,0 +1,22 @@
+#include "pd_denoiser_dev.h"
+#include "pd_gemm_stream.h"
+#include "pd_gemm_split.h"
+#include "pd_qkv_attn.h"
+#include "pd_denoiser_plan.h"
+
+template <int EPI>
+static void den_gemm_planes(bool rt3, const float *A, int K, const unsigned *W, const float *bias, float *C, int M, int Nout, hipStream_t s, float c_scale,
+                            float out_scale = 1.0f) {
+    if (rt3) pd_gemm_strip<EPI, 3, true, 1, PD_STRIP_K64, true>((const unsigned *)A, K, W, K, bias, C, M, Nout, s, c_scale, out_scale);
+    else pd_gemm_strip<EPI, 2, true, 1, PD_STRIP_K64, true>((const unsigned *)A, K, W, K, bias, C, M, Nout, s, c_scale, out_scale);
+}
+
+void pd_den_layer_f16_planes(const PdDenoiserDev *d, const PdLayerDev &L, int B, int N, bool rt3_res, bool rt3_ff1, hipStream_t s) {
+    const int M = B * N;
+    hipLaunchKernelGGL((pd_ln_rows_kernel<DM, 3>), dim3((M + 3) / 4), dim3(256), 0, s, d->h, d->hn, M, 1e-5f, 512.0f);
+    pd_qkv_attn<true>((const unsigned *)d->hn, L.qkv_wh, L.qkv_b, (unsigned *)d->ctx, B, N, L.qkv_cs, L.ctx_scale, s);
+    den_gemm_planes<2>(rt3_res, d->ctx, DM, L.out_wh, L.out_b, d->h, M, DM, s, L.out_cs);
+    hipLaunchKernelGGL((pd_ln_rows_kernel<DM, 3>), dim3((M + 3) / 4), dim3(256), 0, s, d->h, d->hn, M, 1e-5f, 512.0f);
+    den_gemm_planes<4>(rt3_ff1, d->hn, DM, L.ff1_wh, L.ff1_b, d->ff, M, DFF, s, L.ff1_cs, L.ff_scale);
+    den_gemm_planes<2>(rt3_res, d->ff, DFF, L.ff2_wh, L.ff2_b, d->h, M, DM, s, L.ff2_cs);
+}
diff --git a/posediffusion_amd/csrc/pd_engine.hip b/posediffusion_amd/csrc/pd_engine.hip
--- a/posediffusion_amd/csrc/pd_engine.hip
+++ b/posediffusion_amd/csrc/pd_engine.hip
@@ -612,7 +612,7 @@
         key.cond_start = has_ggs ? cond_start_step : 0;
         key.has_ggs = has_ggs;
         key.phase = phase;
-        key.den_split = eng->den_split | (eng->den_fused_attn << 8) | (eng->den_long_attn << 16) | ((nf ? 1 : 0) << 24);
+        key.den_split = eng->den_split | (eng->den_fused_attn << 8) | (eng->den_act_planes << 12) | (eng->den_long_attn << 16) | ((nf ? 1 : 0) << 24);
         if (has_ggs) {
             key.cfg = *ggs;
             if (phase != PD_PHASE_UNGUIDED) {
@@ -699,6 +699,13 @@
         }
         eng->den_fused_attn = value;
         break;
+    case PD_OPT_DENOISER_ACT_PLANES:
+        if (value < 0 || value > 1) {
+            pd_set_error("pd_engine_set_option: PD_OPT_DENOISER_ACT_PLANES takes 0 or 1 (got %d)", value);
+            return PD_ERR_INVALID_ARG;
+        }
+        eng->den_act_planes = value;
+        break;
     case PD_OPT_DENOISER_LONG_ATTN:
         if (value < 0 || value > 1) {
             pd_set_error("pd_engine_set_option: PD_OPT_DENOISER_LONG_ATTN takes 0 or 1 (got %d)", value);
@@ -759,6 +766,7 @@
     switch (option) {
     case PD_OPT_DENOISER_SPLIT: *value_out = eng->den_split; break;
     case PD_OPT_DENOISER_FUSED_ATTN: *value_out = eng->den_fused_attn; break;
+    case PD_OPT_DENOISER_ACT_PLANES: *value_out = eng->den_act_planes; break;
     case PD_OPT_DENOISER_LONG_ATTN: *value_out = eng->den_long_attn; break;
     case PD_OPT_GGS_MAX_FRAMES: *value_out = eng->ggs_max_frames; break;
     case PD_OPT_GGS_LONG_PAIR_ITEMS: *value_out = eng->ggs_long_pair_items; break;
diff --git a/posediffusion_amd/csrc/pd_gemm_split.h b/posediffusion_amd/csrc/pd_gemm_split.h
--- a/posediffusion_amd/csrc/pd_gemm_split.h
+++ b/posediffusion_amd/csrc/pd_gemm_split.h
@@ -207,16 +207,18 @@
 
 template <bool M16>
 __device__ __forceinline__ int pd_strip_swz(int r) { return M16 ? ((r >> 1) & 1) | ((r >> 1) & 4) : (r >> 1) & 7; }
+__device__ __forceinline__ int pd_strip_swz_planes(int r) { return (r & 2) | ((r >> 1) & 4); }
 static constexpr size_t PD_STRIP_PATCH_BYTES = (size_t)4 * 32 * 36 * sizeof(float);
 template <int RT, bool K64>
 static constexpr size_t pd_gemm_strip_lds() {
     const size_t stage = (size_t)(K64 ? 4 : 2) * 32 * RT * 32 * sizeof(unsigned);
     return K64 && PD_STRIP_WIDE_EPI && stage < PD_STRIP_PATCH_BYTES ? PD_STRIP_PATCH_BYTES : stage;
 }
-template <int EPI, int RT, bool F16, int CT = 1, int BARE = 0, bool K64 = false>
+template <int EPI, int RT, bool F16, int CT = 1, int BARE = 0, bool K64 = false, bool PLANES = false>
 __global__ __launch_bounds__(256) __attribute__((amdgpu_waves_per_eu((K64 && PD_STRIP_MFMA16 && RT >= 2) ? (RT == 3 ? 3 : 4) - (EPI == 2 ? 1 : 0) : 1)))
 void pd_gemm_strip_kernel(VitSplitArgs g) {
     constexpr bool M16 = K64 && PD_STRIP_MFMA16 != 0;
+    static_assert(!PLANES || (M16 && F16 && (EPI == 2 || EPI == 4)), "fp16 planes: the denoiser's 64-k 16x16x32 launches that read them (EPI 4 writes them too)");
     static_assert(!M16 || PD_STRIP_WIDE_EPI, "the 16x16 accumulator layout is written out by the wide epilogue only");
     constexpr int KC = 32, TM = 32 * RT, TN = 128 * CT, GROUP = RT == 3 ? 24 : (RT == 1 ? 32 : 2048 / TM), CHA = TM * KC;
     static_assert(RT >= 1 && RT <= 4 && (CT == 1 || CT == 2), "pieces of 8 rows, RT per wave and chunk");
@@ -245,8 +247,14 @@
 #pragma unroll
     for (int j = 0; j < RT; ++j) {
         const int r = 8 * (RT * wave + j) + prow;
-        oa[j] = (unsigned)(((size_t)min(m0 + r, g.M - 1) * g.lda + 4 * (pslot ^ pd_strip_swz<M16>(r))) * sizeof(unsigned));
-    }
+        if constexpr (PLANES) oa[j] = (unsigned)((size_t)min(m0 + r, g.M - 1) * g.lda * 2 + 16 * (pslot ^ pd_strip_swz_planes(r)));
+        else oa[j] = (unsigned)(((size_t)min(m0 + r, g.M - 1) * g.lda + 4 * (pslot ^ pd_strip_swz<M16>(r))) * sizeof(unsigned));
+    }
+    const size_t plane_bytes = (size_t)g.M * g.lda * 2;
+    auto piece_base = [&](int c, int h) {
+        if constexpr (PLANES) return (const float *)((const char *)g.A + (size_t)c * 128 + (size_t)h * plane_bytes);
+        else return (const float *)(g.A + (2 * c + h) * KC);
+    };
     const unsigned lds_a = (unsigned)(size_t)(strip_lds + RT * wave * 256);
     auto stage = [&](int kc, int buf) {
         const float *ab = (const float *)(g.A + kc * KC);
@@ -301,14 +309,27 @@
             const unsigned da = __builtin_amdgcn_readfirstlane(lds_a + buf * 2 * CHA * 4);
 #pragma unroll
             for (int h = 0; h < 2; ++h) {
-                const float *ab = (const float *)(g.A + (2 * c + h) * KC);
+                const float *ab = piece_base(c, h);
 #pragma unroll
                 for (int j = 0; j < RT; ++j) pd_dma_piece(ab, oa[j], da + h * CHA * 4 + j * 1024);
             }
         };
-        auto block = [&](const unsigned *a, const wv4 &w0, const wv4 &w1, const wv4 &w2, const wv4 &w3) {
+        auto block = [&](const unsigned *a, int blk, const wv4 &w0, const wv4 &w1, const wv4 &w2, const wv4 &w3) {
             uint4 ah[RT], al[RT];
-            if constexpr (M16) {
+            if constexpr (PLANES) {
+                const int sl = 4 * ((4 * blk + kg) ^ pd_strip_swz_planes(l15));
+#pragma unroll
+                for (int st = 0; st < 2; ++st)
+#pragma unroll
+                    for (int mi = 0; mi < RT; ++mi) {
+                        const uint4 h8 = *(const uint4 *)(a + (mi * 32 + st * 16) * KC + sl);
+                        const uint4 l8 = *(const uint4 *)(a + CHA + (mi * 32 + st * 16) * KC + sl);
+                        acc_v4 &c0 = acc4[M16 ? 2 * mi + st : 0][0], &c1 = acc4[M16 ? 2 * mi + st : 0][1];
+                        c0 = mma16(l8, w0, c0); c1 = mma16(l8, w2, c1);
+                        c0 = mma16(h8, w1, c0); c1 = mma16(h8, w3, c1);
+                        c0 = mma16(h8, w0, c0); c1 = mma16(h8, w2, c1);
+                    }
+            } else if constexpr (M16) {
                 const int sz = pd_strip_swz<true>(l15);
 #pragma unroll
                 for (int st = 0; st < 2; ++st)
@@ -349,7 +370,19 @@
 #if PD_STRIP_PIPE
         wv4 raw[2][RT][2];
         const int swz = M16 ? pd_strip_swz<true>(l15) : (l31 >> 1) & 7;
-        auto read_mi = [&](int rb, const unsigned *a, int st, int mi) {
+        const int slp0 = 4 * (kg ^ pd_strip_swz_planes(l15)), slp1 = slp0 ^ 16;
+        auto read_plane = [&](int rb, const unsigned *a, int blk, int st, int mi, int pl) {
+            const unsigned p_ = (unsigned)(size_t)(a + (mi * 32 + st * 16) * KC + (blk ? slp1 : slp0));
+            if (pl == 0) asm volatile("ds_read_b128 %0, %1" : "=&v"(raw[rb][mi][0]) : "v"(p_) : "memory");
+            else asm volatile("ds_read_b128 %0, %1 offset:%2" : "=&v"(raw[rb][mi][1]) : "v"(p_), "n"(CHA * 4) : "memory");
+        };
+        auto read_mi = [&](int rb, const unsigned *a, int blk, int st, int mi) {
+            if constexpr (PLANES) {
+                read_plane(rb, a, blk, st, mi, 0);
+                read_plane(rb, a, blk, st, mi, 1);
+                return;
+            }
+            a += blk * CHA;
             const unsigned p_ = (unsigned)(size_t)(M16 ? a + (mi * 32 + st * 16) * KC + 4 * ((2 * kg) ^ swz) : a + mi * 32 * KC + 4 * ((4 * st + 2 * hi) ^ swz));
             const unsigned q_ = (unsigned)(size_t)(M16 ? a + (mi * 32 + st * 16) * KC + 4 * ((2 * kg + 1) ^ swz) : a + mi * 32 * KC + 4 * ((4 * st + 2 * hi + 1) ^ swz));
             asm volatile("ds_read_b128 %0, %2\n\tds_read_b128 %1, %3" : "=&v"(raw[rb][mi][0]), "=&v"(raw[rb][mi][1]) : "v"(p_), "v"(q_) : "memory");
@@ -362,9 +395,9 @@
         auto dma_piece_at = [&](int p) {
             const unsigned da = __builtin_amdgcn_readfirstlane(lds_a + dma_nb * 2 * CHA * 4);
             const int h = p / RT, j = p % RT;
-            pd_dma_piece((const float *)(g.A + (2 * dma_cn + h) * KC), oa[j], da + h * CHA * 4 + j * 1024);
-        };
-        auto step = [&](int rb, const wv4 &wh, const wv4 &wl, bool has_next, int nrb, const unsigned *na, int nst, int dma_step) {
+            pd_dma_piece(piece_base(dma_cn, h), oa[j], da + h * CHA * 4 + j * 1024);
+        };
+        auto step = [&](int rb, const wv4 &wh, const wv4 &wl, bool has_next, int nrb, const unsigned *na, int nblk, int nst, int dma_step) {
             uint4 ah[RT], al[RT];
 #pragma unroll
             for (int mi = 0; mi < RT; ++mi) {
@@ -388,7 +421,7 @@
                 ah[mi] = make_uint4(__builtin_amdgcn_perm(p.y, p.x, 0x05040100u), __builtin_amdgcn_perm(p.w, p.z, 0x05040100u),
                                     __builtin_amdgcn_perm(q.y, q.x, 0x05040100u), __builtin_amdgcn_perm(q.w, q.z, 0x05040100u));
 #endif
-                if (has_next) read_mi(nrb, na, nst, mi);
+                if (has_next) read_mi(nrb, na, nblk, nst, mi);
                 __builtin_amdgcn_sched_barrier(0);
                 acc[mi][0] = mmaw(ah[mi], wl, acc[mi][0]);
                 __builtin_amdgcn_sched_barrier(0);
@@ -401,9 +434,43 @@
                 __builtin_amdgcn_sched_barrier(0);
             }
         };
-        auto step16 = [&](int rb, int h, const wv4 &w0, const wv4 &w1, const wv4 &w2, const wv4 &w3, bool has_next, int nrb, const unsigned *na, int nst,
+        auto step16 = [&](int rb, int h, const wv4 &w0, const wv4 &w1, const wv4 &w2, const wv4 &w3, bool has_next, int nrb, const unsigned *na, int nblk, int nst,
                           int dma_step) {
             uint4 ah[RT], al[RT];
+            if constexpr (PLANES) {
+#pragma unroll
+                for (int mi = 0; mi < RT; ++mi) {
+                    const wv4 q = raw[rb][mi][1];
+                    const int t = M16 ? 2 * mi + h : 0;
+                    al[mi] = make_uint4(q.x, q.y, q.z, q.w);
+                    if (has_next) read_plane(nrb, na, nblk, nst, mi, 0);
+                    __builtin_amdgcn_sched_barrier(0);
+                    acc4[t][0] = mma16(al[mi], w0, acc4[t][0]);
+                    acc4[t][1] = mma16(al[mi], w2, acc4[t][1]);
+                    __builtin_amdgcn_sched_barrier(0);
+                }
+#pragma unroll
+                for (int mi = 0; mi < RT; ++mi) {
+                    const wv4 p = raw[rb][mi][0];
+                    const int t = M16 ? 2 * mi + h : 0;
+                    ah[mi] = make_uint4(p.x, p.y, p.z, p.w);
+                    if (has_next) read_plane(nrb, na, nblk, nst, mi, 1);
+                    __builtin_amdgcn_sched_barrier(0);
+                    acc4[t][0] = mma16(ah[mi], w1, acc4[t][0]);
+                    acc4[t][1] = mma16(ah[mi], w3, acc4[t][1]);
+                    __builtin_amdgcn_sched_barrier(0);
+                }
+#pragma unroll
+                for (int mi = 0; mi < RT; ++mi) {
+                    const int t = M16 ? 2 * mi + h : 0;
+                    if (dma_step >= 0) dma_piece_at(dma_step * RT + mi);
+                    __builtin_amdgcn_sched_barrier(0);
+                    acc4[t][0] = mma16(ah[mi], w0, acc4[t][0]);
+                    acc4[t][1] = mma16(ah[mi], w2, acc4[t][1]);
+                    __builtin_amdgcn_sched_barrier(0);
+                }
+                return;
+            }
 #pragma unroll
             for (int mi = 0; mi < RT; ++mi) {
                 const wv4 p = raw[rb][mi][0], q = raw[rb][mi][1];
@@ -421,7 +488,7 @@
                 const int t = M16 ? 2 * mi + h : 0;
                 ah[mi] = make_uint4(__builtin_amdgcn_perm(p.y, p.x, 0x05040100u), __builtin_amdgcn_perm(p.w, p.z, 0x05040100u),
                                     __builtin_amdgcn_perm(q.y, q.x, 0x05040100u), __builtin_amdgcn_perm(q.w, q.z, 0x05040100u));
-                if (has_next) read_mi(nrb, na, nst, mi);
+                if (has_next) read_mi(nrb, na, nblk, nst, mi);
                 __builtin_amdgcn_sched_barrier(0);
                 acc4[t][0] = mma16(ah[mi], w1, acc4[t][0]);
                 acc4[t][1] = mma16(ah[mi], w3, acc4[t][1]);
@@ -479,20 +546,20 @@
             dma_cn = cn;
             dma_nb = (c + 1) & 1;
 #pragma unroll
-            for (int mi = 0; mi < RT; ++mi) read_mi(0, a, 0, mi);
+            for (int mi = 0; mi < RT; ++mi) read_mi(0, a, 0, 0, mi);
             wait_reads(0);
             PD_LEG_T0();
-            if constexpr (M16) step16(0, 0, a0, a1, a2, a3, true, 1, a, 1, MODE == 2 ? -1 : 0);
-            else step(0, a0, a1, true, 1, a, 1, MODE == 2 ? -1 : 0);
+            if constexpr (M16) step16(0, 0, a0, a1, a2, a3, true, 1, a, 0, 1, MODE == 2 ? -1 : 0);
+            else step(0, a0, a1, true, 1, a, 0, 1, MODE == 2 ? -1 : 0);
             PD_LEG_ACC(leg_s0);
             wait_reads(1);
             PD_LEG_T0();
-            if constexpr (M16) step16(1, 1, a0, a1, a2, a3, true, 0, a + CHA, 0, MODE == 2 ? -1 : 1);
-            else step(1, a2, a3, true, 0, a + CHA, 0, MODE == 2 ? -1 : 1);
+            if constexpr (M16) step16(1, 1, a0, a1, a2, a3, true, 0, a, 1, 0, MODE == 2 ? -1 : 1);
+            else step(1, a2, a3, true, 0, a, 1, 0, MODE == 2 ? -1 : 1);
             PD_LEG_ACC(leg_s1);
 #else
             if constexpr (MODE != 2) stage64(cn, (c + 1) & 1);
-            block(a, a0, a1, a2, a3);
+            block(a, 0, a0, a1, a2, a3);
 #endif
             if constexpr (MODE != 2) PD_STRIP_WLOAD(a0, a1, a2, a3, 2 * cn);
             PD_LEG_T0();
@@ -501,16 +568,16 @@
 #if PD_STRIP_PIPE
             wait_reads(0);
             PD_LEG_T0();
-            if constexpr (M16) step16(0, 0, b0, b1, b2, b3, true, 1, a + CHA, 1, -1);
-            else step(0, b0, b1, true, 1, a + CHA, 1, -1);
+            if constexpr (M16) step16(0, 0, b0, b1, b2, b3, true, 1, a, 1, 1, -1);
+            else step(0, b0, b1, true, 1, a, 1, 1, -1);
             PD_LEG_ACC(leg_s2);
             wait_reads(1);
             PD_LEG_T0();
-            if constexpr (M16) step16(1, 1, b0, b1, b2, b3, false, 0, a, 0, -1);
-            else step(1, b2, b3, false, 0, a, 0, -1);
+            if constexpr (M16) step16(1, 1, b0, b1, b2, b3, false, 0, a, 0, 0, -1);
+            else step(1, b2, b3, false, 0, a, 0, 0, -1);
             PD_LEG_ACC(leg_s3);
 #else
-            block(a + CHA, b0, b1, b2, b3);
+            block(PLANES ? a : a + CHA, PLANES ? 1 : 0, b0, b1, b2, b3);
 #endif
             if constexpr (MODE != 2) {
                 PD_STRIP_WLOAD(b0, b1, b2, b3, 2 * cn + 1);
@@ -674,6 +741,13 @@
                         if constexpr (EPI == 3 || EPI == 4) o[e] = pd_split_word_as<F16 ? 2 : 1>(t, g.out_scale);
                         else o[e] = __float_as_uint(t);
                     }
+                    if constexpr (PLANES && EPI == 4) {
+                        if (row < g.M) {
+                            unsigned short *ch = (unsigned short *)g.C + (size_t)row * g.Nout + colb;
+                            *(uint2 *)ch = make_uint2(__builtin_amdgcn_perm(o[1], o[0], 0x05040100u), __builtin_amdgcn_perm(o[3], o[2], 0x05040100u));
+                            *(uint2 *)(ch + (size_t)g.M * g.Nout) = make_uint2(__builtin_amdgcn_perm(o[1], o[0], 0x07060302u), __builtin_amdgcn_perm(o[3], o[2], 0x07060302u));
+                        }
+                    } else
                     if (row < g.M) *(uint4 *)((unsigned *)g.C + (size_t)row * g.Nout + colb) = make_uint4(o[0], o[1], o[2], o[3]);
                 }
             }
@@ -716,12 +790,12 @@
 #endif
 #endif
 }
-template <int EPI, int RT, bool F16, int CT = 1, bool K64 = false>
+template <int EPI, int RT, bool F16, int CT = 1, bool K64 = false, bool PLANES = false>
 static inline void pd_gemm_strip(const unsigned *A, int lda, const unsigned *W, int K, const float *bias, void *C, int M, int Nout, hipStream_t s,
                                  float c_scale = 1.0f, float out_scale = 1.0f) {
     VitSplitArgs g{A, W, bias, C, M, Nout, K, lda, c_scale, out_scale};
     constexpr int TM = 32 * RT;
-    hipLaunchKernelGGL((pd_gemm_strip_kernel<EPI, RT, F16, CT, 0, K64>), dim3(((M + TM - 1) / TM) * (Nout / (128 * CT))), dim3(256),
+    hipLaunchKernelGGL((pd_gemm_strip_kernel<EPI, RT, F16, CT, 0, K64, PLANES>), dim3(((M + TM - 1) / TM) * (Nout / (128 * CT))), dim3(256),
                        (pd_gemm_strip_lds<RT, K64>()), s, g);
 }
 
diff --git a/posediffusion_amd/csrc/pd_gemm_stream.h b/posediffusion_amd/csrc/pd_gemm_stream.h
--- a/posediffusion_amd/csrc/pd_gemm_stream.h
+++ b/posediffusion_amd/csrc/pd_gemm_stream.h
@@ -54,6 +54,24 @@
 #pragma unroll
     for (int off = 32; off >= 1; off >>= 1) q += __shfl_xor(q, off, 64);
     const float rstd = 1.0f / sqrtf(q * (1.0f / D) + eps);
+    if constexpr (SPLIT == 3) {
+        static_assert(SPLIT != 3 || PER == 8, "a lane stores 8 halves = 16 bytes per plane");
+        __shared__ __attribute__((aligned(16))) unsigned ln_patch[4][D];
+        unsigned *pw = ln_patch[threadIdx.x >> 6];
+#pragma unroll
+        for (int i = 0; i < PER; ++i) pw[(lane + 64 * i) ^ ((i & 2) << 1)] = pd_split_word_h((v[i] - mean) * rstd * scale);
+        __builtin_amdgcn_fence(__ATOMIC_RELEASE, "wavefront");
+        __builtin_amdgcn_wave_barrier();
+        __builtin_amdgcn_fence(__ATOMIC_ACQUIRE, "wavefront");
+        const int sw = (lane >> 2) & 4;
+        const uint4 a = *(const uint4 *)(pw + ((8 * lane) ^ sw)), b = *(const uint4 *)(pw + ((8 * lane + 4) ^ sw));
+        unsigned short *dst = (unsigned short *)xn + (size_t)row * D + 8 * lane;
+        *(uint4 *)dst = make_uint4(__builtin_amdgcn_perm(a.y, a.x, 0x05040100u), __builtin_amdgcn_perm(a.w, a.z, 0x05040100u),
+                                   __builtin_amdgcn_perm(b.y, b.x, 0x05040100u), __builtin_amdgcn_perm(b.w, b.z, 0x05040100u));
+        *(uint4 *)(dst + (size_t)M * D) = make_uint4(__builtin_amdgcn_perm(a.y, a.x, 0x07060302u), __builtin_amdgcn_perm(a.w, a.z, 0x07060302u),
+                                                     __builtin_amdgcn_perm(b.y, b.x, 0x07060302u), __builtin_amdgcn_perm(b.w, b.z, 0x07060302u));
+        return;
+    }
 #pragma unroll
     for (int i = 0; i < PER; ++i) {
         const float o = (v[i] - mean) * rstd;
diff --git a/posediffusion_amd/csrc/pd_internal.h b/posediffusion_amd/csrc/pd_internal.h
--- a/posediffusion_amd/csrc/pd_internal.h
+++ b/posediffusion_amd/csrc/pd_internal.h
@@ -231,6 +231,7 @@
     int ggs_long_pair_items = 0;
     unsigned int *d_err = nullptr;
     int ggs_prof_on = 0;
+    int den_act_planes = 1;
     int den_fused_attn = 1;
     int den_long_attn = 0;
     int den_split = 0;
@@ -275,6 +276,8 @@
 int pd_denoiser_t_rows(pd_engine *eng, const int64_t *t_seq, int B, int N, hipStream_t s);
 int pd_denoiser_q_sample(pd_engine *eng, const float *x_start, const float *noise, const int64_t *t_seq, int B, int N, float *xt, hipStream_t s);
 void pd_den_first_gemm_t(const PdDenoiserDev *d, const int *t_row, int M, hipStream_t s);
+struct PdLayerDev;
+void pd_den_layer_f16_planes(const PdDenoiserDev *d, const PdLayerDev &L, int B, int N, bool rt3_res, bool rt3_ff1, hipStream_t s);
 int pd_denoiser_prepare(pd_engine *eng, const float *z, int B, int N, hipStream_t s);
 
 int pd_time_table(const pd_weights *w, float *table);
diff --git a/posediffusion_amd/csrc/pd_qkv_attn.h b/posediffusion_amd/csrc/pd_qkv_attn.h
--- a/posediffusion_amd/csrc/pd_qkv_attn.h
+++ b/posediffusion_amd/csrc/pd_qkv_attn.h
@@ -33,10 +33,11 @@
     return (image > stage ? image : stage) + (size_t)3 * 32 * PD_QA_LS * sizeof(float);
 }
 
-template <int BARE, bool DEEP = false>
+template <int BARE, bool DEEP = false, bool PLANES = false>
 __global__ __launch_bounds__(PD_QA_THREADS) void pd_qkv_attn_kernel(PdQkvAttnArgs g) {
     constexpr int KC = 32, RT = 3, TM = PD_QA_ROWS, CHA = TM * KC, LDR = PD_QA_LDR, LS = PD_QA_LS;
     constexpr bool M16 = PD_STRIP_MFMA16 != 0;
+    static_assert(!PLANES || (M16 && BARE == 0), "fp16 planes: the 16x16x32 form only");
     extern __shared__ __attribute__((aligned(1024))) unsigned qa_lds[];
     const int tid = threadIdx.x, lane = tid & 63, l31 = lane & 31, hi = lane >> 5;
     const int wave = __builtin_amdgcn_readfirstlane(tid >> 6);
@@ -66,8 +67,10 @@
     unsigned oa;
     {
         const int r = 8 * wave + prow;
-        oa = (unsigned)(((size_t)min(m0 + r, M - 1) * DM + 4 * (pslot ^ pd_strip_swz<M16>(r))) * sizeof(unsigned));
-    }
+        if constexpr (PLANES) oa = (unsigned)((size_t)min(m0 + r, M - 1) * DM * 2 + 16 * (pslot ^ pd_strip_swz_planes(r)));
+        else oa = (unsigned)(((size_t)min(m0 + r, M - 1) * DM + 4 * (pslot ^ pd_strip_swz<M16>(r))) * sizeof(unsigned));
+    }
+    const size_t plane_bytes = (size_t)M * DM * 2;
     const unsigned lds_a = (unsigned)(size_t)(qa_lds + wave * 256);
     const int third = wave >> 2;
     const int ntile = third * (DM / 32) + head * (DH / 32) + (wave & 3);
@@ -109,11 +112,25 @@
         if (!stages) return;
         const unsigned da = __builtin_amdgcn_readfirstlane(lds_a + buf * 2 * CHA * 4);
 #pragma unroll
-        for (int h = 0; h < 2; ++h) pd_dma_piece((const float *)(g.A + (2 * c + h) * KC), oa, da + h * CHA * 4);
+        for (int h = 0; h < 2; ++h) {
+            if constexpr (PLANES) pd_dma_piece((const float *)((const char *)g.A + (size_t)c * 128 + (size_t)h * plane_bytes), oa, da + h * CHA * 4);
+            else pd_dma_piece((const float *)(g.A + (2 * c + h) * KC), oa, da + h * CHA * 4);
+        }
     };
-    auto block = [&](auto nt_, const unsigned *a, const wv4 &w0, const wv4 &w1, const wv4 &w2, const wv4 &w3) {
+    auto block = [&](auto nt_, const unsigned *a, int blk, const wv4 &w0, const wv4 &w1, const wv4 &w2, const wv4 &w3) {
         constexpr int NT = decltype(nt_)::value;
-        if constexpr (M16) {
+        if constexpr (PLANES) {
+            const int sl = 4 * ((4 * blk + kg) ^ pd_strip_swz_planes(l15));
+#pragma unroll
+            for (int t = 0; t < NT; ++t) {
+                const uint4 h8 = *(const uint4 *)(a + t * 16 * KC + sl);
+                const uint4 l8 = *(const uint4 *)(a + CHA + t * 16 * KC + sl);
+                f32x4 &c0 = acc4[M16 ? t : 0][0], &c1 = acc4[M16 ? t : 0][1];
+                c0 = mma16(l8, w0, c0); c1 = mma16(l8, w2, c1);
+                c0 = mma16(h8, w1, c0); c1 = mma16(h8, w3, c1);
+                c0 = mma16(h8, w0, c0); c1 = mma16(h8, w2, c1);
+            }
+        } else if constexpr (M16) {
             const int sz = pd_strip_swz<true>(l15);
 #pragma unroll
             for (int t = 0; t < NT; ++t) {
@@ -170,8 +187,8 @@
                     stage64(c + 1, 1);
                     PD_QA_WLOAD(c0, c1, c2, c3, 2 * (c + 1));
                     PD_QA_WLOAD(d0, d1, d2, d3, 2 * (c + 1) + 1);
-                    block(nt_, a, a0, a1, a2, a3);
-                    block(nt_, a + CHA, b0, b1, b2, b3);
+                    block(nt_, a, 0, a0, a1, a2, a3);
+                    block(nt_, PLANES ? a : a + CHA, PLANES ? 1 : 0, b0, b1, b2, b3);
                     PD_QA_WAIT(0, c0, c1, c2, c3);
                     PD_QA_WAIT(0, d0, d1, d2, d3);
                     __syncthreads();
@@ -182,8 +199,8 @@
                     stage64(cn, 0);
                     PD_QA_WLOAD(a0, a1, a2, a3, 2 * cn);
                     PD_QA_WLOAD(b0, b1, b2, b3, 2 * cn + 1);
-                    block(nt_, a, c0, c1, c2, c3);
-                    block(nt_, a + CHA, d0, d1, d2, d3);
+                    block(nt_, a, 0, c0, c1, c2, c3);
+                    block(nt_, PLANES ? a : a + CHA, PLANES ? 1 : 0, d0, d1, d2, d3);
                     PD_QA_WAIT(0, a0, a1, a2, a3);
                     PD_QA_WAIT(0, b0, b1, b2, b3);
                     __syncthreads();
@@ -196,22 +213,22 @@
             if constexpr (BARE == 0) {
                 if (c + 1 < nk64) {
                     stage64(cn, (c + 1) & 1);
-                    block(nt_, a, a0, a1, a2, a3);
+                    block(nt_, a, 0, a0, a1, a2, a3);
                     PD_QA_WLOAD(a0, a1, a2, a3, 2 * cn);
                     PD_QA_WAIT_STAGED(stages, b0, b1, b2, b3);
-                    block(nt_, a + CHA, b0, b1, b2, b3);
+                    block(nt_, PLANES ? a : a + CHA, PLANES ? 1 : 0, b0, b1, b2, b3);
                     PD_QA_WLOAD(b0, b1, b2, b3, 2 * cn + 1);
                     PD_QA_WAIT(4, a0, a1, a2, a3);
                 } else {
-                    block(nt_, a, a0, a1, a2, a3);
+                    block(nt_, a, 0, a0, a1, a2, a3);
                     PD_QA_WAIT(0, b0, b1, b2, b3);
-                    block(nt_, a + CHA, b0, b1, b2, b3);
+                    block(nt_, PLANES ? a : a + CHA, PLANES ? 1 : 0, b0, b1, b2, b3);
                 }
             } else {
                 if constexpr (BARE != 2 && BARE != 3) stage64(cn, (c + 1) & 1);
-                if constexpr (BARE != 4) block(nt_, a, a0, a1, a2, a3);
+                if constexpr (BARE != 4) block(nt_, a, 0, a0, a1, a2, a3);
                 if constexpr (BARE != 1 && BARE != 3) PD_QA_WLOAD(a0, a1, a2, a3, 2 * cn);
-                if constexpr (BARE != 4) block(nt_, a + CHA, b0, b1, b2, b3);
+                if constexpr (BARE != 4) block(nt_, PLANES ? a : a + CHA, PLANES ? 1 : 0, b0, b1, b2, b3);
                 if constexpr (BARE != 1 && BARE != 3) PD_QA_WLOAD(b0, b1, b2, b3, 2 * cn + 1);
                 PD_QA_WAIT(0, a0, a1, a2, a3);
                 PD_QA_WAIT(0, b0, b1, b2, b3);
@@ -351,6 +368,33 @@
                     o[1][1] = __builtin_amdgcn_mfma_f32_16x16x4f32(a1[e], v1[e], o[1][1], 0, 0, 0);
                 }
             }
+            if constexpr (PLANES) {
+                unsigned *pw = (unsigned *)img + (size_t)s * N * LDR + 32 * tw;
+#pragma unroll
+                for (int rt = 0; rt < 2; ++rt)
+#pragma unroll
+                    for (int e = 0; e < 4; ++e) {
+                        const int i = 16 * rt + 4 * (lane >> 4) + e;
+                        if (i < N) {
+#pragma unroll
+                            for (int ct = 0; ct < 2; ++ct) pw[i * LDR + 16 * ct + (lane & 15)] = pd_split_word_as<2>(o[rt][ct][e], g.out_scale);
+                        }
+                    }
+                __builtin_amdgcn_fence(__ATOMIC_RELEASE, "wavefront");
+                __builtin_amdgcn_wave_barrier();
+                __builtin_amdgcn_fence(__ATOMIC_ACQUIRE, "wavefront");
+                const int g16 = (lane >> 4) & 1, pass = ((((lane & 15) + 4) >> 3) & 1) ^ g16;
+#pragma unroll
+                for (int q = 0; q < 4; ++q) {
+                    const int i = pass + 2 * (lane >> 5) + 4 * (q & 1) + 8 * g16 + 16 * (q >> 1);
+                    if (i < N) {
+                        const uint4 w4 = *(const uint4 *)(pw + i * LDR + 4 * (lane & 7));
+                        unsigned short *ch = (unsigned short *)g.ctx + (size_t)((seq0 + s) * N + i) * DM + head * DH + 32 * tw + 4 * (lane & 7);
+                        *(uint2 *)ch = make_uint2(__builtin_amdgcn_perm(w4.y, w4.x, 0x05040100u), __builtin_amdgcn_perm(w4.w, w4.z, 0x05040100u));
+                        *(uint2 *)((char *)ch + plane_bytes) = make_uint2(__builtin_amdgcn_perm(w4.y, w4.x, 0x07060302u), __builtin_amdgcn_perm(w4.w, w4.z, 0x07060302u));
+                    }
+                }
+            } else
 #pragma unroll
             for (int rt = 0; rt < 2; ++rt)
 #pragma unroll
@@ -367,11 +411,16 @@
     }
 }
 
+template <bool PLANES = false>
 static inline void pd_qkv_attn(const unsigned *hn, const unsigned *Wh, const float *bias, unsigned *ctx, int B, int N, float c_scale, float out_scale,
                                hipStream_t s) {
     PdQkvAttnArgs g{hn, Wh, bias, ctx, B, N, pd_qkv_attn_group(N), c_scale, out_scale};
     const dim3 grid(pd_qkv_attn_wgs(B, N)), blk(PD_QA_THREADS);
     const size_t lds = pd_qkv_attn_lds(N);
+    if constexpr (PLANES) {
+        hipLaunchKernelGGL((pd_qkv_attn_kernel<0, PD_QA_DEEP_DEFAULT != 0, true>), grid, blk, lds, s, g);
+        return;
+    } else {
 #ifdef PD_DEV_KNOBS
     static const int bare = pd_dev_knob("PD_QA_BARE", 0);
     static const int deep = pd_dev_knob("PD_QA_DEEP", PD_QA_DEEP_DEFAULT);
@@ -386,4 +435,5 @@
     }
 #endif
     hipLaunchKernelGGL((pd_qkv_attn_kernel<0, PD_QA_DEEP_DEFAULT != 0>), grid, blk, lds, s, g);
+    }
 }
```

New measurement: 1128, median of 6. 1.4% higher.
